# nianticlabs/simplerecon

Hardware: AMD Instinct MI355X
Metric: depth frames/sec (640x480, 7 src views, 64 planes) (higher is better)
Workload: dtype f32

## Files before the change

include/simplerecon_hip.h:

```cpp
#ifndef SIMPLERECON_HIP_H_
#define SIMPLERECON_HIP_H_

#include <stddef.h>
#include <stdint.h>

#ifdef __cplusplus
extern "C" {
#endif

#define SR_OK 0
#define SR_ERR_INVALID_ARGUMENT 1
#define SR_ERR_UNSUPPORTED 2
#define SR_ERR_WORKSPACE_TOO_SMALL 3
#define SR_ERR_HIP_BASE 1000

enum {
  SR_OPT_MLP_SPLIT = 0, SR_OPT_WINO_SPLIT, SR_OPT_WINO_XCD, SR_OPT_WINO_NT, SR_OPT_WINO_KSPLIT, SR_OPT_CONV_WINO,
  SR_OPT_CONV_TILE, SR_OPT_CONV_KSPLIT, SR_OPT_PW_NT, SR_OPT_PW_KS, SR_OPT_PT_CFG, SR_OPT_PT_KS, SR_OPT_DOT_LDS,
  SR_OPT_DOT_LDS_G, SR_OPT_DOT_LDS_CULL, SR_OPT_DOT_LDS_CAP, SR_OPT_UPSAMPLE_QUAD, SR_OPT_POOL_STREAM,
  SR_OPT_MLP_TILE,
  SR_OPT_COUNT
};
int sr_option_count(void);
const char* sr_option_name(int id);
int sr_option_id(const char* name);
int sr_option_get(int id, int* value);
int sr_option_set(int id, int value, int* previous );
int sr_option_default(int id, int* value);

int sr_abi_version(void);

const char* sr_target_arch(void);


size_t sr_volume_workspace_bytes(int B, int K, int C, int h, int w);

int sr_volume_prepare(const float* src, const float* K_src, const float* T_src_cur,
                      const float* T_cur_src, int B, int K, int C, int h, int w, void* workspace,
                      size_t workspace_bytes, void* stream);

int sr_dot_volume_sweep(const float* cur, const float* invK_cur, const float* planes, int64_t ps_b,
                        int64_t ps_d, int64_t ps_y, int64_t ps_x, int B, int K, int C, int h, int w,
                        int D, float* out_cv, int64_t cv_sb, int64_t cv_sd, int64_t cv_sp,
                        float* out_lowest, uint8_t* out_mask, void* workspace,
                        size_t workspace_bytes, void* stream);

int sr_conv3x3_wino_io_nhwc_fwd(const void* in, int64_t in_batch_stride, int in_pix_stride, const float* packed_u,
                                const float* bias, const void* residual, int64_t res_batch_stride, int res_pix_stride,
                                void* out, int64_t out_batch_stride, int out_pix_stride, int B, int H, int W, int Cin,
                                int Cout, float leaky_slope, int io_dtype, void* stream);
int sr_pw_conv_io_nhwc_fwd(const void* in, int64_t in_batch_stride, int in_pix_stride, const float* packed_w,
                           const float* bias, const void* residual, int64_t res_batch_stride, int res_pix_stride, void* out,
                           int64_t out_batch_stride, int out_pix_stride, int B, int HW, int Cin, int Cout, float act_code,
                           int io_dtype, void* stream);

size_t sr_pw_conv_tiled_workspace_bytes(int M, int Cin, int Cout);
int sr_pw_conv_tiled_plan(int M, int Cin, int Cout, int can_split, int* cfg, int* ks);
int sr_pw_conv_tiled_nhwc_fwd(const float* in, int in_pix_stride, const float* packed_w, const float* bias,
                              const float* gate, const float* residual, int res_pix_stride, float* out,
                              int out_pix_stride, int M, int HW, int Cin, int Cout, float act_code, void* workspace,
                              size_t workspace_bytes, void* stream);
int sr_pw_conv_supported(int Cin, int Cout);
int sr_pw_conv_plan(int B, int HW, int Cin, int Cout, int* nt, int* ks);
int sr_pw_conv_nhwc_fwd(const float* in, int64_t in_batch_stride, int in_pix_stride, const float* packed_w,
                        const float* bias, const float* gate, const float* residual, int64_t res_batch_stride,
                        int res_pix_stride, float* out, int64_t out_batch_stride, int out_pix_stride, int B, int HW,
                        int Cin, int Cout, float act_code, void* stream);

int sr_backproject_fwd(const float* depth, const float* invK, float* out_points, int B, int h, int w, void* stream);
int sr_project3d_fwd(const float* points, const float* K, const float* T, float* out, int B, int N, float eps,
                     void* stream);
int sr_backproject_bwd(const float* grad_points, const float* invK, float* grad_depth, int B, int h, int w, void* stream);
int sr_project3d_bwd(const float* grad_out, const float* points, const float* K, const float* T, float* grad_points, int B,
                     int N, float eps, void* stream);
int sr_pose_distance_fwd(const float* T, float* out, int n, void* stream);
int sr_camera_rays_fwd(const float* points, const float* T, float* out, int B, int N, int in_camera_frame, void* stream);

int sr_selftest_rcp(const float* x, float* out_fast, float* out_div, int n, void* stream);

int sr_dot_volume_fwd(const float* cur, const float* src, const float* K_src,
                      const float* T_src_cur, const float* invK_cur, const float* planes,
                      int64_t ps_b, int64_t ps_d, int64_t ps_y, int64_t ps_x, int B, int K, int C,
                      int h, int w, int D, float* out_cv, int64_t cv_sb, int64_t cv_sd,
                      int64_t cv_sp, float* out_lowest, uint8_t* out_mask, void* workspace,
                      size_t workspace_bytes, void* stream);

int sr_warp_features_fwd(const float* src, const float* K_src, const float* T_src_cur,
                         const float* invK_cur, const float* planes, int64_t ps_b, int64_t ps_d,
                         int64_t ps_y, int64_t ps_x, int B, int K, int C, int h, int w, int Dp,
                         float* out_world, float* out_depths, float* out_warped, float* out_mask,
                         float* out_pix, void* workspace, size_t workspace_bytes, void* stream);

size_t sr_mlp_volume_workspace_bytes(int B, int K, int C, int h, int w, int hidden);

int sr_mlp_pack_weights(const float* W1, const float* b1, const float* W2, const float* b2,
                        const float* W3, const float* b3, int hidden, int B, int K, int C, int h, int w,
                        void* workspace, size_t workspace_bytes, void* stream);

int sr_mlp_volume_sweep(const float* cur, const float* invK_cur, const float* planes, int64_t ps_b,
                        int64_t ps_d, int64_t ps_y, int64_t ps_x, float leaky_slope, int B, int K,
                        int C, int h, int w, int D, float* out_cv, int64_t cv_sb, int64_t cv_sd,
                        int64_t cv_sp, float* out_lowest, uint8_t* out_mask, void* workspace,
                        size_t workspace_bytes, void* stream);

int sr_mlp_volume_tile_shape(int h, int w, int* th, int* tw);

int sr_mlp_volume_fwd(const float* cur, const float* src, const float* K_src, const float* T_src_cur,
                      const float* T_cur_src, const float* invK_cur, const float* planes, int64_t ps_b,
                      int64_t ps_d, int64_t ps_y, int64_t ps_x, const float* W1, const float* b1,
                      const float* W2, const float* b2, const float* W3, const float* b3, int hidden,
                      float leaky_slope, int B, int K, int C, int h, int w, int D, float* out_cv,
                      int64_t cv_sb, int64_t cv_sd, int64_t cv_sp, float* out_lowest, uint8_t* out_mask,
                      int reserve_cus, void* workspace, size_t workspace_bytes, void* stream);

int sr_mlp_volume_fwd_nhwc(const float* cur, const float* src, const float* K_src, const float* T_src_cur,
                           const float* T_cur_src, const float* invK_cur, const float* planes, int64_t ps_b,
                           int64_t ps_d, int64_t ps_y, int64_t ps_x, const float* W1, const float* b1,
                           const float* W2, const float* b2, const float* W3, const float* b3, int hidden,
                           float leaky_slope, int B, int K, int C, int h, int w, int D, float* out_cv,
                           int64_t cv_sb, int64_t cv_sd, int64_t cv_sp, float* out_lowest, uint8_t* out_mask,
                           int reserve_cus, void* workspace, size_t workspace_bytes, void* stream);


size_t sr_conv_packed_weight_floats(int Cout, int Cin, int ksize);

int sr_conv_pack_weights(const float* weight, int Cout, int Cin, int ksize, float* packed, void* stream);

int sr_conv2d_nhwc_fwd(const float* in, int64_t in_batch_stride, int in_pix_stride,
                       const float* packed_weight, const float* bias, const float* residual,
                       int64_t res_batch_stride, int res_pix_stride, float* out,
                       int64_t out_batch_stride, int out_pix_stride, int B, int H, int W, int Cin,
                       int Cout, int ksize, int stride, float leaky_slope, void* stream);

int sr_conv2d_replicate_nhwc_fwd(const float* in, int64_t in_batch_stride, int in_pix_stride,
                                 const float* packed_weight, const float* bias, const float* residual,
                                 int64_t res_batch_stride, int res_pix_stride, float* out,
                                 int64_t out_batch_stride, int out_pix_stride, int B, int H, int W, int Cin,
                                 int Cout, int ksize, int stride, float leaky_slope, void* stream);

#define SR_ACT_NONE (-1.0f)
#define SR_ACT_SILU (-2.0f)
int sr_conv2d_padded_nhwc_fwd(const float* in, int64_t in_batch_stride, int in_pix_stride,
                              const float* packed_weight, const float* bias, const float* residual,
                              int64_t res_batch_stride, int res_pix_stride, float* out,
                              int64_t out_batch_stride, int out_pix_stride, int B, int H, int W, int Cin,
                              int Cout, int ksize, int stride, int pad_top, int pad_left, int pad_bottom,
                              int pad_right, float leaky_slope, void* stream);

size_t sr_conv_splitk_workspace_bytes(int B, int H, int W, int Cin, int Cout, int ksize, int stride);
int sr_conv2d_splitk_nhwc_fwd(const float* in, int64_t in_batch_stride, int in_pix_stride,
                              const float* packed_weight, const float* bias, const float* residual,
                              int64_t res_batch_stride, int res_pix_stride, float* out,
                              int64_t out_batch_stride, int out_pix_stride, int B, int H, int W, int Cin,
                              int Cout, int ksize, int stride, float leaky_slope, void* workspace,
                              size_t workspace_bytes, void* stream);

size_t sr_wino_packed_weight_floats(int Cout, int Cin);
int sr_wino_pack_weights(const float* weight, int Cout, int Cin, float* packed, void* stream);
int sr_conv_prefers_wino(int B, int H, int W, int Cin, int Cout, int ksize, int stride);
int sr_conv3x3_wino_nhwc_fwd(const float* in, int64_t in_batch_stride, int in_pix_stride,
                             const float* packed_u, const float* bias, const float* residual,
                             int64_t res_batch_stride, int res_pix_stride, float* out,
                             int64_t out_batch_stride, int out_pix_stride, int B, int H, int W, int Cin,
                             int Cout, float leaky_slope, void* stream);

size_t sr_wino4_packed_weight_floats(int Cout, int Cin);
int sr_wino4_pack_weights(const float* weight, int Cout, int Cin, float* packed, void* stream);
int sr_conv_prefers_wino4(int B, int H, int W, int Cin, int Cout, int mode);
int sr_conv3x3_wino4_nhwc_fwd(const float* in, int64_t in_batch_stride, int in_pix_stride, const float* packed_u,
                              const float* bias, const float* residual, int64_t res_batch_stride, int res_pix_stride,
                              float* out, int64_t out_batch_stride, int out_pix_stride, int B, int H, int W, int Cin,
                              int Cout, float leaky_slope, void* stream);

int sr_conv3x3_wino4_variant_nhwc_fwd(const float* in, int64_t in_batch_stride, int in_pix_stride, const float* packed_u,
                                      const float* bias, const float* residual, int64_t res_batch_stride,
                                      int res_pix_stride, float* out, int64_t out_batch_stride, int out_pix_stride, int B,
                                      int H, int W, int Cin, int Cout, float leaky_slope, int variant, void* stream);

int sr_wino_splitk_factor(int B, int H, int W, int Cin, int Cout);
size_t sr_wino_splitk_workspace_bytes(int B, int H, int W, int Cin, int Cout);
int sr_conv3x3_wino_splitk_nhwc_fwd(const float* in, int64_t in_batch_stride, int in_pix_stride,
                                    const float* packed_u, const float* bias, const float* residual,
                                    int64_t res_batch_stride, int res_pix_stride, float* out,
                                    int64_t out_batch_stride, int out_pix_stride, int B, int H, int W, int Cin,
                                    int Cout, float leaky_slope, void* workspace, size_t workspace_bytes,
                                    void* stream);

const char* sr_wino_kernel_name(int B, int H, int W, int Cin, int Cout, int aligned_in, int aligned_out);

const char* sr_conv_kernel_name(int B, int H, int W, int Cin, int Cout, int ksize, int stride, int aligned16);

int sr_upsample2x_nhwc_fwd(const float* in, int64_t in_batch_stride, int in_pix_stride, float* out,
                           int64_t out_batch_stride, int out_pix_stride, int B, int H, int W, int C,
                           void* stream);

int sr_exp_fwd(const float* in, float* out, int64_t n, void* stream);


size_t sr_stem_packed_weight_floats(int Cout);
int sr_stem_pack_weights(const float* weight, int Cout, float* packed, void* stream);

int sr_stem7x7_fwd(const float* in, int64_t in_batch_stride, int64_t in_chan_stride, int64_t in_row_stride,
                   int64_t in_col_stride, const float* packed_weight, const float* scale, const float* shift,
                   float leaky_slope, float* out, int64_t out_batch_stride, int out_pix_stride, int B, int H, int W,
                   int Cout, void* stream);

int sr_maxblurpool_nhwc_fwd(const float* in, int64_t in_batch_stride, int in_pix_stride, float* out,
                            int64_t out_batch_stride, int out_pix_stride, int B, int H, int W, int C, void* stream);

size_t sr_instance_norm_workspace_bytes(int B, int H, int W, int C);
int sr_instance_norm_nhwc_fwd(const float* in, int64_t in_batch_stride, int in_pix_stride, float* out,
                              int64_t out_batch_stride, int out_pix_stride, int B, int H, int W, int C, float eps,
                              float leaky_slope, void* workspace, size_t workspace_bytes, void* stream);

int sr_instance_norm_stats_nhwc(const float* in, int64_t in_batch_stride, int in_pix_stride, int B, int H, int W, int C,
                                float eps, float* stats, void* workspace, size_t workspace_bytes, void* stream);

size_t sr_conv1x1_stats_workspace_bytes(int B, int H, int W, int Cout);
int sr_conv1x1_stats_nhwc_fwd(const float* in, int64_t in_batch_stride, int in_pix_stride, const float* weight,
                              const float* bias, float* out, int64_t out_batch_stride, int out_pix_stride, int B, int H,
                              int W, int Cin, int Cout, float eps, float* stats, void* workspace, size_t workspace_bytes,
                              void* stream);

size_t sr_conv3x3_c16_packed_weight_floats(int Cout, int Cin);
// ... 351 lines not shown
```

simplerecon_amd/_lib.py:

```python
import contextlib
import ctypes as C
import os

import torch

_HERE = os.path.dirname(os.path.abspath(__file__))
LIB_PATH = os.environ.get("SR_HIP_LIBRARY") or os.path.join(_HERE, "libsimplerecon_hip.so")
ABI_VERSION = 3

_lib = None

_p = C.c_void_p
_i = C.c_int
_i64 = C.c_int64
_f = C.c_float
_sz = C.c_size_t

SIGNATURES = {
    "sr_abi_version": (_i, []),
    "sr_option_count": (_i, []),
    "sr_option_name": (C.c_char_p, [_i]),
    "sr_option_id": (_i, [C.c_char_p]),
    "sr_option_get": (_i, [_i, C.POINTER(C.c_int)]),
    "sr_option_set": (_i, [_i, _i, C.POINTER(C.c_int)]),
    "sr_option_default": (_i, [_i, C.POINTER(C.c_int)]),
    "sr_target_arch": (C.c_char_p, []),
    "sr_volume_workspace_bytes": (_sz, [_i, _i, _i, _i, _i]),
    "sr_volume_prepare": (_i, [_p, _p, _p, _p, _i, _i, _i, _i, _i, _p, _sz, _p]),
    "sr_dot_volume_sweep": (_i, [_p, _p, _p, _i64, _i64, _i64, _i64, _i, _i, _i, _i, _i, _i,
                                 _p, _i64, _i64, _i64, _p, _p, _p, _sz, _p]),
    "sr_dot_volume_fwd": (_i, [_p, _p, _p, _p, _p, _p, _i64, _i64, _i64, _i64, _i, _i, _i, _i, _i, _i,
                               _p, _i64, _i64, _i64, _p, _p, _p, _sz, _p]),
    "sr_rgb_stem3x3s2_fwd": (_i, [_p, _i64, _i64, _i64, _i64, _p, _p, _p, _i64, _i, _i, _i, _i, _i, _i, _i, _i, _i, _f, _p]),
    "sr_se_gate2_fwd": (_i, [_p, _i, _i, _p, _p, _p, _p, _p, _p, _i, _i, _i, _p]),
    "sr_conv3x3_wino_io_nhwc_fwd": (_i, [_p, _i64, _i, _p, _p, _p, _i64, _i, _p, _i64, _i, _i, _i, _i, _i, _i, _f, _i, _p]),
    "sr_pw_conv_io_nhwc_fwd": (_i, [_p, _i64, _i, _p, _p, _p, _i64, _i, _p, _i64, _i, _i, _i, _i, _i, _f, _i, _p]),
    "sr_conv16_packed_weight_bytes": (_sz, [_i, _i, _i]),
    "sr_conv16_pack_weights": (_i, [_p, _i, _i, _i, _i, _p, _p]),
    "sr_conv16_supported": (_i, [_i, _i, _i, _i, _i, _i, _i]),
    "sr_conv16_prefers": (_i, [_i, _i, _i, _i, _i, _i, _i]),
    "sr_conv16_nhwc_fwd": (_i, [_p, _i64, _i, _p, _p, _p, _i64, _i, _p, _i64, _i, _i, _i, _i, _i, _i, _i, _i, _f, _i, _i, _p]),
    "sr_conv16_wgrad_supported": (_i, [_i, _i, _i, _i, _i, _i, _i]),
    "sr_conv16_wgrad_prefers": (_i, [_i, _i, _i, _i, _i, _i, _i]),
    "sr_conv16_wgrad_workspace_bytes": (_sz, [_i, _i, _i, _i, _i, _i, _i]),
    "sr_conv16_wgrad_nhwc": (_i, [_p, _i64, _i, _p, _i64, _i, _p, _i, _i, _i, _i, _i, _i, _i, _i, _p, _sz, _p]),
    "sr_act_bwd_bias16_workspace_bytes": (_sz, [_i64, _i]),
    "sr_act_bwd_bias16_nhwc": (_i, [_p, _i, _p, _p, _p, _i64, _i, _f, _i, _p, _sz, _p]),
    "sr_pw_conv_tiled_workspace_bytes": (_sz, [_i, _i, _i]),
    "sr_pw_conv_tiled_plan": (_i, [_i, _i, _i, _i, _p, _p]),
    "sr_pw_conv_tiled_nhwc_fwd": (_i, [_p, _i, _p, _p, _p, _p, _i, _p, _i, _i, _i, _i, _i, _f, _p, _sz, _p]),
    "sr_pw_conv_supported": (_i, [_i, _i]),
    "sr_pw_conv_plan": (_i, [_i, _i, _i, _i, _p, _p]),
    "sr_pw_conv_nhwc_fwd": (_i, [_p, _i64, _i, _p, _p, _p, _p, _i64, _i, _p, _i64, _i, _i, _i, _i, _i, _f, _p]),
    "sr_backproject_fwd": (_i, [_p, _p, _p, _i, _i, _i, _p]),
    "sr_project3d_fwd": (_i, [_p, _p, _p, _p, _i, _i, _f, _p]),
    "sr_backproject_bwd": (_i, [_p, _p, _p, _i, _i, _i, _p]),
    "sr_project3d_bwd": (_i, [_p, _p, _p, _p, _p, _i, _i, _f, _p]),
    "sr_pose_distance_fwd": (_i, [_p, _p, _i, _p]),
    "sr_camera_rays_fwd": (_i, [_p, _p, _p, _i, _i, _i, _p]),
    "sr_selftest_rcp": (_i, [_p, _p, _p, _i, _p]),
    "sr_warp_features_fwd": (_i, [_p, _p, _p, _p, _p, _i64, _i64, _i64, _i64, _i, _i, _i, _i, _i, _i,
                                  _p, _p, _p, _p, _p, _p, _sz, _p]),
    "sr_mlp_volume_workspace_bytes": (_sz, [_i, _i, _i, _i, _i, _i]),
    "sr_mlp_pack_weights": (_i, [_p, _p, _p, _p, _p, _p, _i, _i, _i, _i, _i, _i, _p, _sz, _p]),
    "sr_mlp_volume_sweep": (_i, [_p, _p, _p, _i64, _i64, _i64, _i64, _f, _i, _i, _i, _i, _i, _i,
                                 _p, _i64, _i64, _i64, _p, _p, _p, _sz, _p]),
    "sr_mlp_volume_tile_shape": (_i, [_i, _i, C.POINTER(C.c_int), C.POINTER(C.c_int)]),
    "sr_mlp_volume_fwd": (_i, [_p, _p, _p, _p, _p, _p, _p, _i64, _i64, _i64, _i64, _p, _p, _p, _p, _p, _p, _i,
                               _f, _i, _i, _i, _i, _i, _i, _p, _i64, _i64, _i64, _p, _p, _i, _p, _sz, _p]),
    "sr_mlp_volume_fwd_nhwc": (_i, [_p, _p, _p, _p, _p, _p, _p, _i64, _i64, _i64, _i64, _p, _p, _p, _p, _p, _p, _i,
                                    _f, _i, _i, _i, _i, _i, _i, _p, _i64, _i64, _i64, _p, _p, _i, _p, _sz, _p]),
    "sr_conv_packed_weight_floats": (_sz, [_i, _i, _i]),
    "sr_conv_pack_weights": (_i, [_p, _i, _i, _i, _p, _p]),
    "sr_conv2d_nhwc_fwd": (_i, [_p, _i64, _i, _p, _p, _p, _i64, _i, _p, _i64, _i, _i, _i, _i, _i, _i, _i, _i, _f, _p]),
    "sr_conv2d_replicate_nhwc_fwd": (_i, [_p, _i64, _i, _p, _p, _p, _i64, _i, _p, _i64, _i, _i, _i, _i, _i, _i, _i, _i,
                                          _f, _p]),
    "sr_conv2d_padded_nhwc_fwd": (_i, [_p, _i64, _i, _p, _p, _p, _i64, _i, _p, _i64, _i, _i, _i, _i, _i, _i, _i, _i,
                                       _i, _i, _i, _i, _f, _p]),
    "sr_dwconv3x3_pool_bands": (_i, [_i]),
    "sr_dwconv3x3_nhwc_fwd": (_i, [_p, _i64, _i, _p, _p, _p, _i64, _i, _p, _i, _i, _i, _i, _i, _i, _i, _i, _i, _f,
                                   _p]),
    "sr_add_nhwc_fwd": (_i, [_p, _i64, _i, _p, _i64, _i, _p, _i64, _i, _i, _i, _i, _i, _p]),
    "sr_se_scale_nhwc_fwd": (_i, [_p, _i, _p, _p, _p, _p, _p, _p, _i64, _i, _p, _i64, _i, _p, _i, _i, _i, _i, _i,
                                  _p]),
    "sr_se_gate_fwd": (_i, [_p, _i, _i, _p, _p, _p, _p, _p, _i, _i, _i, _p]),
    "sr_scale_channels_nhwc_fwd": (_i, [_p, _i64, _i, _p, _p, _i64, _i, _i, _i, _i, _i, _p]),
    "sr_dot_volume_bwd_scratch_bytes": (_sz, [_i, _i, _i, _i, _i]),
    "sr_dot_volume_bwd": (_i, [_p, _i64, _i64, _i64, _p, _p, _p, _i64, _i64, _i64, _i64, _i, _i, _i, _i, _i, _i, _p, _p,
                               _p, _sz, _p, _sz, _p]),
    "sr_mlp_volume_bwd_scratch_bytes": (_sz, [_i, _i, _i, _i, _i, _i]),
    "sr_mlp_volume_bwd": (_i, [_p, _i64, _i64, _i64, _p, _p, _p, _i64, _i64, _i64, _i64, _p, _p, _p, _p, _p, _f, _i, _i,
                               _i, _i, _i, _i, _i, _p, _p, _p, _p, _p, _p, _p, _p, _p, _sz, _p, _sz, _p]),
    "sr_conv_wgrad_workspace_bytes": (_sz, [_i, _i, _i, _i, _i, _i, _i]),
    "sr_conv_wgrad_nhwc": (_i, [_p, _i64, _i, _p, _i64, _i, _p, _i, _i, _i, _i, _i, _i, _i, _p, _sz, _p]),
    "sr_bias_grad_nhwc": (_i, [_p, _i64, _i, _p, _i, _i, _i, _i, _p]),
    "sr_act_bwd": (_i, [_p, _p, _p, _i64, _f, _p]),
    "sr_act_bwd_bias_workspace_bytes": (_sz, [_i64, _i]),
    "sr_act_bwd_bias_nhwc": (_i, [_p, _p, _p, _p, _i64, _i, _f, _p, _sz, _p]),
    "sr_zero_stuff2x_nhwc": (_i, [_p, _i64, _i, _p, _i, _i, _i, _i, _i, _i, _p]),
    "sr_upsample2x_bwd_nhwc": (_i, [_p, _i64, _i, _p, _i64, _i, _i, _i, _i, _i, _p]),
    "sr_conv_flip_transpose_weights": (_i, [_p, _i, _i, _i, _p, _p]),
    "sr_mul_fwd": (_i, [_p, _p, _p, _i64, _p]),
    "sr_norm_workspace_bytes": (_sz, [_i, _i, _i, _i]),
    "sr_norm_stats_nhwc": (_i, [_p, _i64, _i, _i, _i, _i, _i, _p, _p, _p, _sz, _p]),
    "sr_norm_act_fwd_nhwc": (_i, [_p, _i64, _i, _p, _p, _f, _p, _p, _f, _i, _p, _i64, _i, _i, _i, _i, _p]),
    "sr_norm_act_bwd_nhwc": (_i, [_p, _i64, _i, _p, _i64, _i, _p, _p, _f, _p, _p, _f, _i, _i, _p, _i64, _i, _p, _p,
                                  _i, _i, _i, _p, _sz, _p]),
    "sr_rowsum_nhwc": (_i, [_p, _i64, _i, _p, _i64, _i, _i, _i, _i, _f, _p, _p, _sz, _p]),
    "sr_maxblurpool_bwd_workspace_bytes": (_sz, [_i, _i, _i, _i]),
    "sr_maxblurpool_bwd_nhwc": (_i, [_p, _i64, _i, _p, _i64, _i, _p, _i64, _i, _i, _i, _i, _i, _p, _sz, _p]),
    "sr_replicate_pad_nhwc_fwd": (_i, [_p, _i64, _i, _p, _i, _i, _i, _i, _i, _p]),
    "sr_replicate_pad_nhwc_bwd": (_i, [_p, _p, _i, _i, _i, _i, _i, _p]),
    "sr_im2col7x7s2_nhwc": (_i, [_p, _i64, _i64, _i64, _i64, _p, _i, _i, _i, _i, _p]),
    "sr_dwconv3x3_bwd_workspace_bytes": (_sz, [_i, _i, _i, _i]),
    "sr_dwconv3x3_bwd_nhwc": (_i, [_p, _i64, _i, _p, _i64, _i, _p, _p, _p, _i, _i, _i, _i, _i, _i, _i, _i, _i, _p, _sz,
                                   _p]),
    "sr_scale_bwd_nhwc": (_i, [_p, _i64, _i, _p, _p, _f, _p, _i, _i, _i, _p]),
    "sr_small_linear_fwd": (_i, [_p, _p, _p, _p, _p, _i, _i, _i, _f, _p]),
    "sr_small_linear_bwd": (_i, [_p, _p, _p, _p, _p, _p, _p, _i, _i, _i, _f, _p]),
    "sr_act_in_bwd": (_i, [_p, _p, _p, _i64, _f, _p]),
    "sr_add_act_fwd": (_i, [_p, _p, _p, _p, _i64, _f, _p]),
    "sr_conv_wgrad_padded_workspace_bytes": (_sz, [_i, _i, _i, _i, _i, _i]),
    "sr_conv_wgrad_padded_nhwc": (_i, [_p, _i64, _i, _p, _i64, _i, _p, _i, _i, _i, _i, _i, _i, _i, _i, _i, _i, _i, _p,
                                       _sz, _p]),
    "sr_conv_splitk_workspace_bytes": (_sz, [_i, _i, _i, _i, _i, _i, _i]),
    "sr_conv2d_splitk_nhwc_fwd": (_i, [_p, _i64, _i, _p, _p, _p, _i64, _i, _p, _i64, _i, _i, _i, _i, _i, _i, _i, _i,
                                       _f, _p, _sz, _p]),
    "sr_wino_packed_weight_floats": (_sz, [_i, _i]),
    "sr_wino_pack_weights": (_i, [_p, _i, _i, _p, _p]),
    "sr_conv_prefers_wino": (_i, [_i, _i, _i, _i, _i, _i, _i]),
    "sr_wino_splitk_factor": (_i, [_i, _i, _i, _i, _i]),
    "sr_wino_splitk_workspace_bytes": (_sz, [_i, _i, _i, _i, _i]),
    "sr_conv3x3_wino_splitk_nhwc_fwd": (_i, [_p, _i64, _i, _p, _p, _p, _i64, _i, _p, _i64, _i, _i, _i, _i, _i, _i, _f,
                                             _p, _sz, _p]),
# ... 47 lines not shown
    "sr_depth_terms_bwd": (_i, [_p, _p, _p, _p, _p, _p, _p, _i, _i, _p, _i, _i, _p, _i, _i, _i, _i, _i, _f, _i, _p, _p,
                                _p, _p, _p, _p]),
    "sr_depth_metrics_workspace_bytes": (_sz, [_i, _i, _i]),
    "sr_depth_metrics": (_i, [_p, _p, _p, _f, _i, _i, _i, _i, _i, _i, _i, _p, _p, _p, _p, _sz, _p]),
    "sr_depth_metrics_gather": (_i, [_p, _i, _i, _i, _i, _i, _i, _p, _p]),
    "sr_nn_grid_plan": (_i, [_i64, _p, _i64, _p, _p, _p]),
    "sr_nn_keys": (_i, [_p, _i64, C.c_double, C.c_double, C.c_double, C.c_double, _i, _i, _i, _p, _p]),
    "sr_nn_build": (_i, [_p, _i64, _p, _p, _i64, _p, _p, _p]),
    "sr_nn_query": (_i, [_p, _i64, _p, _p, _i64, _p, _i64, C.c_double, C.c_double, C.c_double, C.c_double, _i, _i, _i,
                         _p, _p, _p, _p]),
    "sr_sample_surface_workspace_bytes": (_sz, [_i64]),
    "sr_sample_surface_cdf": (_i, [_p, _i64, _p, _i64, _p, _p, _sz, _p]),
    "sr_sample_surface": (_i, [_p, _i64, _p, _i64, _p, _i64, C.c_uint64, _p, _p, _p]),
    "sr_mesh_metrics_workspace_bytes": (_sz, [_i64, _i64]),
    "sr_mesh_metrics": (_i, [_p, _i64, _p, _i64, _f, _p, _p, _sz, _p]),
    "sr_stsdf_touch": (_i, [_p, _i, _i, _i, _p, C.c_double, C.c_double, _p, _p]),
    "sr_stsdf_block_masks": (_i, [_p, _p, _i64, _i64, _p, _p]),
    "sr_stsdf_integrate": (_i, [_p, _i64, _p, _p, _p, _i64, _p, _p, _p, _i, _i, _i, _f, _f, _p]),
    "sr_stsdf_mesh_count": (_i, [_p, _i64, _p, _p, _i64, _p, _p]),
    "sr_stsdf_mesh_emit": (_i, [_p, _i64, _p, _p, _i64, _f, _p, _i64, _i64, _p, _p, _p, _p, _p]),
    "sr_raster_small": (_i, [_p, _i64, _p, _i64, _p, _p, _i, _i, _i, _f, _f, _i, _p, _p, _p]),
    "sr_raster_large_setup": (_i, [_p, _i64, _p, _i64, _p, _p, _i, _i, _i, _f, _f, _i, _i64, _p, _p, _p, _p]),
    "sr_raster_large": (_i, [_p, _p, _i64, _i64, _p, _i, _i, _i, _f, _f, _p, _p]),
    "sr_raster_resolve": (_i, [_p, _i64, _p, _p, _p]),
    "sr_raster_visibility_mask": (_i, [_p, _i, _i64, _i64, _p, _p]),
    "sr_raster_visibility_count": (_i, [_p, _i64, _p, _i, _p, _p]),
    "sr_mesh_vertex_normals": (_i, [_p, _i64, _p, _i64, _p, _p, _p, _p]),
    "sr_raster_shade": (_i, [_p, _i64, _p, _i64, _p, _p, _i, _i, _i, _f, _p, _p, _p, _p, _p, _f, _p, _i, _i, _i, _p, _p,
                             _p, _p]),
    "sr_frames_resize_fits_lds": (_i, [_i, _i, _i, _i]),
    "sr_frames_resize": (_i, [_p, _i, _i, _i, _i, _p, _i, _p, _i, _i, _p, _p, _i, _i, _i, _i, _p, _p]),
    "sr_frames_depth": (_i, [_p, _i, _i, _i, _i, _p, _p, _i, _i, _f, _f, _f, _i, _p, _p, _p, _p]),
    "sr_frames_jitter_scratch_bytes": (_sz, [_i, _i, _i]),
    "sr_frames_jitter_check_params": (_i, [_p, _i]),
    "sr_frames_jitter": (_i, [_p, _i, _i, _i, _p, _p, _i, _i, _p, _sz, _p]),
    "sr_viz_range_workspace_bytes": (_sz, [_i, _i64]),
    "sr_viz_range": (_i, [_p, _p, _i, _i, _i64, _i, _p, _p, _sz, _p]),
    "sr_viz_colormap": (_i, [_p, _p, _i, _i, _i64, _p, _p, _i64, _p, _i64, _f, _f, _f, _f, _f, _p, _p, _p]),
    "sr_viz_unit": (_i, [_p, _i, _i64, _i, _p, _p, _p]),
    "sr_adamw_step": (_i, [_p, _p, _p, _p, _p, _p, _p, _p, _p, _i, _i, _p, _i, _p, _p, _p]),
    "sr_adamw_step_clipped": (_i, [_p, _p, _p, _p, _p, _p, _p, _p, _p, _i, _i, _p, _i, _p, _p, _p, _p]),
    "sr_grad_stats_workspace_bytes": (_sz, [_i, _i]),
    "sr_grad_stats": (_i, [_p, _p, _p, _i, _i, _p, _f, _p, _p, _p, _p, C.c_double, C.c_double, _i, _p, _sz, _p]),
    "sr_grad_scale_inplace": (_i, [_p, _p, _p, _i, _i, _p, _p]),
}


class HipLibraryError(RuntimeError):
    pass


def lib():
    global _lib
    if _lib is None:
        if not os.path.exists(LIB_PATH):
            raise HipLibraryError(
                f"{LIB_PATH} not found: build it with `python -m simplerecon_amd.build` "
                "(hipcc --offload-arch=gfx950).  simplerecon_amd has no CPU/torch fallback.")
        l = C.CDLL(LIB_PATH)
        for name, (res, args) in SIGNATURES.items():
            fn = getattr(l, name)
            fn.restype = res
            fn.argtypes = args
        if l.sr_abi_version() != ABI_VERSION:
            raise HipLibraryError(f"ABI mismatch: library {l.sr_abi_version()} vs binding {ABI_VERSION}")
        _lib = l
    return _lib


ERR_UNSUPPORTED = 2
_ERRORS = {1: "invalid argument", ERR_UNSUPPORTED: "unsupported configuration", 3: "workspace too small"}


def check(rc, what):
    if rc != 0:
        msg = _ERRORS.get(rc, f"hipError {rc - 1000}" if rc >= 1000 else f"error {rc}")
        raise HipLibraryError(f"{what} failed: {msg}")


SPLIT_MODES = {"": 0, "0": 0, "off": 0, "fp32": 0, "bf16": 1, "f16": 2, "fp16": 2}
_SPLIT_NAMES = {0: "", 1: "bf16", 2: "f16"}
SPLIT_OPTION_NAMES = ("SR_MLP_SPLIT", "SR_WINO_SPLIT")
TILE_MODES = {"auto": 0, "flat": 1, "2x32": 2, "4x16": 3, "8x8": 4}
_NAMED_VALUES = {"SR_MLP_SPLIT": SPLIT_MODES, "SR_WINO_SPLIT": SPLIT_MODES, "SR_MLP_TILE": TILE_MODES}
import threading
SPLIT_GUARD = threading.RLock()


OPTION_LISTENERS = []


def _option_id(name):
    oid = lib().sr_option_id(name.encode())
    if oid < 0:
        raise KeyError(f"libsimplerecon_hip.so has no option {name!r}")
    return oid


_OPTION_MIRROR = {}


def get_option(name):
    v = _OPTION_MIRROR.get(name)
    if v is None:
        c = C.c_int(0)
        check(lib().sr_option_get(_option_id(name), C.byref(c)), "sr_option_get")
        v = _OPTION_MIRROR[name] = c.value
    return v


def refresh_options():
    _OPTION_MIRROR.clear()


def set_option(name, value):
    if isinstance(value, str):
        if name not in _NAMED_VALUES:
            raise ValueError(f"option {name} takes an integer, got {value!r}")
        value = _NAMED_VALUES[name].get(value, -1)
    prev = C.c_int(0)
    with SPLIT_GUARD if name in SPLIT_OPTION_NAMES else _NULL_CONTEXT:
        check(lib().sr_option_set(_option_id(name), int(value), C.byref(prev)), "sr_option_set")
        _OPTION_MIRROR[name] = int(value)
        for fn in OPTION_LISTENERS:
            fn(name, int(value))
    return prev.value


@contextlib.contextmanager
def option(name, value):
    prev = set_option(name, value)
    try:
        yield
    finally:
        set_option(name, prev)


def split_mode_name(option_name):
    v = get_option(option_name)
    return _SPLIT_NAMES.get(v, str(v))


def require_device_f32(name, t, allow_none=False):
    if t is None:
        if allow_none:
            return
        raise ValueError(f"{name} is None")
    if not isinstance(t, torch.Tensor):
        raise TypeError(f"{name} must be a torch.Tensor, got {type(t)}")
    if not t.is_cuda:
        raise HipLibraryError(f"{name} lives on {t.device}: the HIP path needs device tensors (no CPU fallback)")
    if t.dtype != torch.float32:
        raise TypeError(f"{name} must be float32 (the reference runs inference in fp32), got {t.dtype}")


def device_f32(name, t, why=None):
    if why is not None and isinstance(t, torch.Tensor) and t.dtype != torch.float32:
        raise TypeError(f"{name} must be float32 ({why}), got {t.dtype}")
    require_device_f32(name, t)
    return t.contiguous()


def data_f32(name, t, role, why=None):
    t = device_f32(name, t, why)
    if torch.is_grad_enabled() and t.requires_grad:
        raise HipLibraryError(f"{name} requires a gradient: {role}")
    return t.detach()
# ... 66 lines not shown
```

simplerecon_amd/csrc/sr_common.h:

```cpp
#pragma once
#include <hip/hip_runtime.h>
#include <stdint.h>

#include "simplerecon_hip.h"

#define SR_GEOM_STRIDE 20

#define SR_WAVE 64

int sr_opt(int id);

int sr_device_cus();

hipError_t sr_allow_lds(const void* kernel, size_t bytes);

int sr_wgrad_reduce_launch(const float* part, float* d_weight, int Cout, int Cin, int taps, int ci_blocks, int per, int blocks,
                           hipStream_t stream);
int sr_bias_partial_reduce_launch(const float* partial, int blocks, int C, float* d_bias, hipStream_t stream);

static inline int sr_hip_rc(hipError_t e) { return e == hipSuccess ? SR_OK : SR_ERR_HIP_BASE + (int)e; }

static inline size_t sr_align_up(size_t v, size_t a) { return (v + a - 1) / a * a; }

struct SrPlanes {
// ... 37 lines not shown
  w_nw = (vx0 & vy0) ? wtop.x : 0.0f;
  w_ne = (vx1 & vy0) ? wtop.y : 0.0f;
  w_sw = (vx0 & vy1) ? wbot.x : 0.0f;
  w_se = (vx1 & vy1) ? wbot.y : 0.0f;
  any_tap = (vx0 | vx1) & (vy0 | vy1);
}
__device__ __forceinline__ void sr_bilinear_taps(float ix, float iy, int h, int w, float& fx0, float& fy0, float& w_nw,
                                                 float& w_ne, float& w_sw, float& w_se) {
  bool any_tap;
  sr_bilinear_taps(ix, iy, h, w, fx0, fy0, w_nw, w_ne, w_sw, w_se, any_tap);
}

struct SrSampleXY {
  float zp, pix_x, pix_y;
  float ix, iy;
  float fx0, fy0;
  float w_nw, w_ne, w_sw, w_se;
  bool any_tap;
};

__device__ __forceinline__ void sr_project_sample_xy(const float* __restrict__ g ,
                                                     float X0, float X1, float X2, int h, int w,
                                                     float inv_w, float inv_h, SrSampleXY& s) {
#pragma clang fp contract(off)
  const float eps = 1e-8f;
  const sr_f2v q01 = sr_f2v{g[0], g[4]} * X0 + sr_f2v{g[1], g[5]} * X1 + sr_f2v{g[2], g[6]} * X2 + sr_f2v{g[3], g[7]};
  const float q2 = g[8] * X0 + g[9] * X1 + g[10] * X2 + g[11];
  s.zp = q2 + eps;
  const float sc = (fabsf(q2) > eps) ? 1.0f / s.zp : 1.0f;
  const sr_f2v pix = q01 * sc;
  s.pix_x = pix.x;
  s.pix_y = pix.y;
  const sr_f2v uv = 2.0f * pix * sr_f2v{inv_w, inv_h} - 1.0f;
  const sr_f2v size = {(float)w, (float)h};
  const sr_f2v ixy = ((uv + 1.0f) * size - 1.0f) / 2.0f;
  s.ix = ixy.x;
  s.iy = ixy.y;
  sr_bilinear_taps(s.ix, s.iy, h, w, s.fx0, s.fy0, s.w_nw, s.w_ne, s.w_sw, s.w_se, s.any_tap);
}

__device__ __forceinline__ void sr_project_sample(const float* __restrict__ g ,
                                                  float X0, float X1, float X2, int h, int w,
                                                  float inv_w, float inv_h, SrSample& s) {
  SrSampleXY c;
  sr_project_sample_xy(g, X0, X1, X2, h, w, inv_w, inv_h, c);
  s.zp = c.zp; s.pix_x = c.pix_x; s.pix_y = c.pix_y;
  s.w_nw = c.w_nw; s.w_ne = c.w_ne; s.w_sw = c.w_sw; s.w_se = c.w_se;
  s.any_tap = c.any_tap;
  const float wm = (float)(w - 1), hm = (float)(h - 1);
  const float fx1 = c.fx0 + 1.0f, fy1 = c.fy0 + 1.0f;
  const int x0 = (int)fminf(fmaxf(c.fx0, 0.0f), wm), x1 = (int)fminf(fmaxf(fx1, 0.0f), wm);
  const int y0 = (int)fminf(fmaxf(c.fy0, 0.0f), hm), y1 = (int)fminf(fmaxf(fy1, 0.0f), hm);
  s.o_nw = y0 * w + x0;
  s.o_ne = y0 * w + x1;
  s.o_sw = y1 * w + x0;
  s.o_se = y1 * w + x1;
}

__device__ __forceinline__ bool sr_in_bounds(const SrSample& s, int h, int w) {
  return (s.pix_x > 2.0f) & (s.pix_x < (float)(w - 2)) & (s.pix_y > 2.0f) & (s.pix_y < (float)(h - 2));
}

#ifdef __HIPCC__
__device__ __forceinline__ float sr_vmax(float a, float b) {
  float r;
  asm("v_max_f32 %0, %1, %2" : "=v"(r) : "v"(a), "v"(b));
  return r;
}
__device__ __forceinline__ float sr_vmin(float a, float b) {
  float r;
  asm("v_min_f32 %0, %1, %2" : "=v"(r) : "v"(a), "v"(b));
  return r;
}
__device__ __forceinline__ float sr_vmax_mfma(float a, float b) {
  float r;
  asm("v_max_f32 %0, %1, %2\n\ts_nop 1" : "=v"(r) : "v"(a), "v"(b));
  return r;
}
__device__ __forceinline__ float sr_activate(float v, float slope) {
  if (slope >= 0.0f) return fmaxf(v, 0.0f) + slope * fminf(v, 0.0f);
  if (slope < -1.5f) return v / (1.0f + __expf(-v));
  return v;
}
__device__ __forceinline__ float sr_uniform(float x) {
  return __builtin_bit_cast(float, __builtin_amdgcn_readfirstlane(__builtin_bit_cast(int, x)));
}
template <int N>
__device__ __forceinline__ void sr_activate_group(float (&v)[N], float slope) {
  if (slope >= 0.0f) {
    if (slope <= 1.0f) {
#pragma unroll
      for (int i = 0; i < N; ++i) v[i] = sr_vmax(v[i], slope * v[i]);
    } else {
#pragma unroll
      for (int i = 0; i < N; ++i) v[i] = sr_vmax(v[i], 0.0f) + slope * sr_vmin(v[i], 0.0f);
    }
  } else if (slope < -1.5f) {
#pragma unroll
    for (int i = 0; i < N; ++i) v[i] = v[i] / (1.0f + __expf(-v[i]));
  }
}
#endif

struct SrDotParams {
  const float* cur;
  const float* src_nhwc;
  const float* invK;
  const float* geom;
  SrPlanes planes;
  SrVolumeOut out;
  int B, K, h, w, D;
  float inv_w, inv_h;
};

static inline float* sr_ws_geom(void* workspace) { return (float*)sr_align_up((size_t)workspace, 256); }
static inline float* sr_ws_src_nhwc(void* workspace, int B, int K) {
  return (float*)((char*)sr_ws_geom(workspace) + sr_align_up((size_t)B * K * SR_GEOM_STRIDE * sizeof(float), 256));
}

static inline size_t sr_ws_nhwc_bytes(int B, int K, int C, int h, int w) {
  return sr_align_up((size_t)B * K * h * w * C * sizeof(float), 256);
}
static inline unsigned long long* sr_ws_keys(void* workspace, int B, int K, int C, int h, int w) {
  return (unsigned long long*)((char*)sr_ws_src_nhwc(workspace, B, K) + sr_ws_nhwc_bytes(B, K, C, h, w));
}

int sr_launch_dot_volume_lds(const SrDotParams& p, unsigned long long* keys, hipStream_t stream);
int sr_launch_geom(const float* K_src, const float* T_src_cur, const float* T_cur_src, float* geom,
                   int n, hipStream_t stream);
int sr_launch_argmax_planes(const float* cv, int64_t sb, int64_t sd, int64_t sp, SrPlanes planes, int B, int h, int w,
                            int D, float* lowest, hipStream_t stream);
int sr_launch_splitk_reduce(const float* part, int ksplit, int64_t part_stride, const float* bias, const float* res,
                            int64_t res_sb, int res_sp, float* out, int64_t out_sb, int out_sp, int B, int HW, int Cout,
                            float slope, hipStream_t stream);
int sr_launch_unpack_nhwc(const float* src_nhwc, float* dst_nchw, int images, int C, int npix, hipStream_t stream);
int sr_launch_pack_nhwc(const float* src_nchw, float* dst_nhwc, int images, int C, int npix,
                        hipStream_t stream);
```

simplerecon_amd/csrc/sr_conv.hip:

```cpp
#include <stdio.h>
#include <stdlib.h>

#include "sr_common.h"
#include "sr_view.h"

#ifndef SR_NB1
#define SR_NB1 6
#endif
#ifndef SR_RES_PF
#define SR_RES_PF 0
#endif

#ifndef SR_CK1
#define SR_CK1 64
#endif
#ifndef SR_CONV_BLOCKS_PER_CU
#define SR_CONV_BLOCKS_PER_CU 2
#endif
__host__ __device__ constexpr int sr_ck(int ks, int stride = 1) { return (ks == 1 && stride == 1) ? SR_CK1 : 16; }

struct SrConvParams {
  const float* in; int64_t in_sb; int in_sp;
  const float* wp;
  const float* bias;
// ... 15 lines not shown
  static constexpr int HH = (TH - 1) * S + KS;
  static constexpr int HW = (CM - 1) * S + KS;
  static constexpr int CK = sr_ck(KS, S);
  static constexpr int ROW = CK + 4;
  static constexpr int Q = CK / 4;
  static constexpr int ELEMS = HH * HW * Q;
  static constexpr int PER_THREAD = (ELEMS + 255) / 256;
  static constexpr int TILE_FLOATS = HH * HW * ROW;
};

template <int KS, int S, int MT, int CM>
__device__ __forceinline__ void sr_conv_stage_setup(const SrConvParams& p, int iy0, int ix0,
                                                    int (&offs)[SrConvGeom<KS, S, MT, CM>::PER_THREAD]) {
  using G = SrConvGeom<KS, S, MT, CM>;
#pragma unroll
  for (int it = 0; it < G::PER_THREAD; ++it) {
    const int e = threadIdx.x + it * 256;
    const int px = e / G::Q, q = e % G::Q;
    const int hy = px / G::HW, hx = px - hy * G::HW;
    int iy = iy0 + hy, ix = ix0 + hx;
    if (p.replicate) {
      iy = min(max(iy, 0), p.H - 1);
      ix = min(max(ix, 0), p.W - 1);
    }
    const bool ok = (e < G::ELEMS) && (iy >= 0) && (iy < p.H) && (ix >= 0) && (ix < p.W);
    offs[it] = ok ? (iy * p.W + ix) * p.in_sp + 4 * q : -1;
  }
}

template <int KS, int S, int MT, int CM, bool VEC4>
__device__ __forceinline__ void sr_conv_stage_load(const SrConvParams& p, const float* __restrict__ in_b, int c0,
                                                   const int (&offs)[SrConvGeom<KS, S, MT, CM>::PER_THREAD],
                                                   float4 (&stg)[SrConvGeom<KS, S, MT, CM>::PER_THREAD]) {
  using G = SrConvGeom<KS, S, MT, CM>;
#pragma unroll
  for (int it = 0; it < G::PER_THREAD; ++it) {
    const int c = c0 + 4 * ((threadIdx.x + it * 256) % G::Q);
    const bool ok = (offs[it] >= 0) && (c < p.Cin);
    const float* src = in_b + (ok ? offs[it] + c0 : 0);
    if (VEC4) {
      const float4 v = *reinterpret_cast<const float4*>(src);
      stg[it] = ok ? v : make_float4(0.f, 0.f, 0.f, 0.f);
    } else {
      float4 v = make_float4(0.f, 0.f, 0.f, 0.f);
      if (ok) {
        v.x = src[0];
        if (c + 1 < p.Cin) v.y = src[1];
        if (c + 2 < p.Cin) v.z = src[2];
        if (c + 3 < p.Cin) v.w = src[3];
      }
      stg[it] = v;
    }
  }
}

template <int KS, int S, int MT, int CM>
__device__ __forceinline__ void sr_conv_stage_store(float* __restrict__ tile,
                                                    const float4 (&stg)[SrConvGeom<KS, S, MT, CM>::PER_THREAD]) {
  using G = SrConvGeom<KS, S, MT, CM>;
#pragma unroll
  for (int it = 0; it < G::PER_THREAD; ++it) {
    const int e = threadIdx.x + it * 256;
    if (e < G::ELEMS) *reinterpret_cast<float4*>(&tile[(e / G::Q) * G::ROW + 4 * (e % G::Q)]) = stg[it];
  }
}

struct SrTileCoord { int b, co0, oy0, ox0, ks; };

template <int TH, int NT, int CM>
__device__ __forceinline__ SrTileCoord sr_conv_tile(const SrConvParams& p, int work) {
  SrTileCoord t;
  t.ks = 0;
  if (p.ksplit > 1) { t.ks = work % p.ksplit; work /= p.ksplit; }
  const int cb = work % p.co_blocks; work /= p.co_blocks;
  const int tx = work % p.tiles_x; work /= p.tiles_x;
  const int ty = work % p.tiles_y;
  t.b = work / p.tiles_y;
  t.co0 = cb * (32 * NT);
  t.oy0 = ty * TH;
  t.ox0 = tx * CM;
  return t;
}

template <int KS, int S, int MT, int NT, int CM, bool VEC4>
__global__ __launch_bounds__(256) void sr_conv_kernel(SrConvParams p) {
  using G = SrConvGeom<KS, S, MT, CM>;
  constexpr int TH = G::TH, HW = G::HW, RM = G::RM;
  constexpr int GPS = G::CK / 8;
  constexpr int STEPS = KS * KS * GPS;
  constexpr int ROW = G::ROW;
  __shared__ __attribute__((aligned(16))) float tiles[2][G::TILE_FLOATS];

  const int lane = threadIdx.x & 63;
  const int wave = threadIdx.x >> 6;
  const int i = lane & 31, kk = lane >> 5;

  int a_off[MT];
#pragma unroll
  for (int m = 0; m < MT; ++m)
    a_off[m] = ((((wave * MT + m) * RM + i / CM) * S) * HW + (i % CM) * S) * ROW + 4 * kk;
  const int64_t rec = (int64_t)2 * p.Co_pad;
  const int chunks = p.G / GPS;

  constexpr int NB = (NT == 1) ? (STEPS % 6 == 0 ? SR_NB1 : STEPS % 4 == 0 ? 4 : STEPS % 3 == 0 ? 3 : 2)
                               : (STEPS % 3 == 0 ? 3 : 2);
  constexpr int PD = NB - 1;
  static_assert(STEPS % NB == 0 && PD < STEPS + 1, "rotating buffers must line up across slabs");
  constexpr bool RES_PF = (MT * NT <= 2) && SR_RES_PF;
  float4 b_f[NB][NT], a_f[2][MT], stg[G::PER_THREAD];
  int offs[G::PER_THREAD];

  int work = blockIdx.x;
  if (work >= p.total_tiles) return;
  SrTileCoord t = sr_conv_tile<TH, NT, CM>(p, work);
  const float4* wp4 = reinterpret_cast<const float4*>(p.wp) + (kk * p.Co_pad + t.co0 + i);
  auto load_b = [&](const float4* base, int ch, int s, float4 (&dst)[NT]) {
    const int tap = s / GPS, g = s % GPS;
    const float4* wrec = base + (int64_t)(tap * p.G + GPS * ch + g) * rec;
#pragma unroll
    for (int n = 0; n < NT; ++n) dst[n] = wrec[32 * n];
  };

  int c_beg = t.ks * chunks / p.ksplit, c_end = (t.ks + 1) * chunks / p.ksplit;
  sr_conv_stage_setup<KS, S, MT, CM>(p, t.oy0 * S - p.pad_y, t.ox0 * S - p.pad_x, offs);
  sr_conv_stage_load<KS, S, MT, CM, VEC4>(p, p.in + (int64_t)t.b * p.in_sb, c_beg * G::CK, offs, stg);
  sr_conv_stage_store<KS, S, MT, CM>(tiles[0], stg);
#pragma unroll
  for (int s = 0; s < PD; ++s) load_b(wp4, c_beg, s, b_f[s]);
  __syncthreads();
  int buf = 0;
  const bool partial = p.ksplit > 1;

  while (true) {
    const int next_work = work + gridDim.x;
    const bool have_next = next_work < p.total_tiles;
    SrTileCoord tn = t;
    if (have_next) tn = sr_conv_tile<TH, NT, CM>(p, next_work);
    const float4* wp4n = reinterpret_cast<const float4*>(p.wp) + (kk * p.Co_pad + tn.co0 + i);
    const int cn_beg = tn.ks * chunks / p.ksplit, cn_end = (tn.ks + 1) * chunks / p.ksplit;

    f32x16 acc[MT][NT];
#pragma unroll
    for (int m = 0; m < MT; ++m)
#pragma unroll
      for (int n = 0; n < NT; ++n)
#pragma unroll
        for (int r = 0; r < 16; ++r) acc[m][n][r] = 0.0f;
    float rpf[RES_PF ? MT : 1][RES_PF ? NT : 1][16];
    const float* __restrict__ resp = (p.res && !partial) ? p.res + (int64_t)t.b * p.res_sb : nullptr;

    for (int ch = c_beg; ch < c_end; ++ch) {
      const float* tile = tiles[buf];
      const bool last = ch + 1 == c_end;
      const bool more = !last || have_next;
      if (more) {
        if (last) sr_conv_stage_setup<KS, S, MT, CM>(p, tn.oy0 * S - p.pad_y, tn.ox0 * S - p.pad_x, offs);
        sr_conv_stage_load<KS, S, MT, CM, VEC4>(p, p.in + (int64_t)(last ? tn.b : t.b) * p.in_sb,
                                            (last ? cn_beg : ch + 1) * G::CK, offs, stg);
      }
      const float4* wnext = last ? wp4n : wp4;
      const int chn = last ? cn_beg : ch + 1;
      if (RES_PF && last) {
#pragma unroll
        for (int m = 0; m < (RES_PF ? MT : 0); ++m) {
          const int oyb = t.oy0 + (wave * MT + m) * RM;
          const int pixb = oyb * p.Wo + t.ox0 + 4 * kk;
#pragma unroll
          for (int n = 0; n < NT; ++n) {
            const int co = t.co0 + 32 * n + i;
            const unsigned rb = (unsigned)(pixb * p.res_sp + co);
#pragma unroll
            for (int r = 0; r < 16; ++r) {
              const int row = (8 * (r >> 2)) / CM, colc = (8 * (r >> 2)) % CM + (r & 3);
              const bool ok = (resp != nullptr) & (co < p.Cout) & (oyb + row < p.Ho) & (t.ox0 + colc + 4 * kk < p.Wo);
              const float v = (resp ? resp : p.in)[ok ? rb + (unsigned)((row * p.Wo + colc) * p.res_sp) : 0u];
              rpf[m][n][r] = ok ? v : 0.0f;
            }
          }
        }
      }
#pragma unroll
      for (int m = 0; m < MT; ++m) a_f[0][m] = *reinterpret_cast<const float4*>(&tile[a_off[m]]);
#pragma unroll
      for (int s = 0; s < STEPS; ++s) {
        const int cb = s % NB, ca = s & 1;
        if (s + PD < STEPS) load_b(wp4, ch, s + PD, b_f[(s + PD) % NB]);
        else if (more) load_b(wnext, chn, s + PD - STEPS, b_f[(s + PD) % NB]);
        if (s + 1 < STEPS) {
          const int tap = (s + 1) / GPS, g = (s + 1) % GPS;
          const int ky = tap / KS, kx = tap - ky * KS;
#pragma unroll
          for (int m = 0; m < MT; ++m)
            a_f[ca ^ 1][m] = *reinterpret_cast<const float4*>(&tile[a_off[m] + (ky * HW + kx) * ROW + 8 * g]);
        }
        __builtin_amdgcn_sched_barrier(0);
#define SR_CONV_KSTEP(E)                                                                                       \
        _Pragma("unroll") for (int m = 0; m < MT; ++m)                                                         \
          _Pragma("unroll") for (int n = 0; n < NT; ++n)                                                       \
            acc[m][n] = __builtin_amdgcn_mfma_f32_32x32x2f32(a_f[ca][m].E, b_f[cb][n].E, acc[m][n], 0, 0, 0);
        SR_CONV_KSTEP(x) SR_CONV_KSTEP(y) SR_CONV_KSTEP(z) SR_CONV_KSTEP(w)
#undef SR_CONV_KSTEP
        __builtin_amdgcn_sched_barrier(0);
      }
      if (more) sr_conv_stage_store<KS, S, MT, CM>(tiles[buf ^ 1], stg);
      __syncthreads();
      buf ^= 1;
    }

    {
      float* __restrict__ outp = partial ? p.part + t.ks * p.part_stride + (int64_t)t.b * p.Ho * p.Wo * p.Cout
                                         : p.out + (int64_t)t.b * p.out_sb;
      const int osp = partial ? p.Cout : p.out_sp, rsp = p.res_sp;
      const float slope = sr_uniform(partial ? SR_ACT_NONE : p.slope);
      const bool no_res = (resp == nullptr);
      const bool full = (t.oy0 + TH <= p.Ho) && (t.ox0 + CM <= p.Wo) && (t.co0 + 32 * NT <= p.Cout);
#pragma unroll
      for (int m = 0; m < MT; ++m) {
        const int oyb = t.oy0 + (wave * MT + m) * RM;
        const int pixb = oyb * p.Wo + t.ox0 + 4 * kk;
#pragma unroll
        for (int n = 0; n < NT; ++n) {
          const int co = t.co0 + 32 * n + i;
          const bool okc = co < p.Cout;
          const float bv = (p.bias && okc && !partial) ? p.bias[co] : 0.0f;
          const unsigned ob = (unsigned)(pixb * osp + co), rb = (unsigned)(pixb * rsp + co);
          float rv[16];
          if (RES_PF) {
#pragma unroll
            for (int r = 0; r < 16; ++r) rv[r] = rpf[RES_PF ? m : 0][RES_PF ? n : 0][r];
          }
          if (full) {
            if (RES_PF) {
            } else if (!no_res) {
#pragma unroll
              for (int r = 0; r < 16; ++r) {
                const int row = (8 * (r >> 2)) / CM, colc = (8 * (r >> 2)) % CM + (r & 3);
                rv[r] = resp[rb + (unsigned)((row * p.Wo + colc) * rsp)];
              }
            } else {
#pragma unroll
              for (int r = 0; r < 16; ++r) rv[r] = 0.0f;
            }
            float o16[16];
#pragma unroll
            for (int r = 0; r < 16; ++r) o16[r] = acc[m][n][r] + bv + rv[r];
            sr_activate_group(o16, slope);
#pragma unroll
            for (int r = 0; r < 16; ++r) {
              const int row = (8 * (r >> 2)) / CM, colc = (8 * (r >> 2)) % CM + (r & 3);
              outp[ob + (unsigned)((row * p.Wo + colc) * osp)] = o16[r];
            }
          } else {
            bool ok[16];
#pragma unroll
            for (int r = 0; r < 16; ++r) {
              const int row = (8 * (r >> 2)) / CM, colc = (8 * (r >> 2)) % CM + (r & 3);
              ok[r] = okc && (oyb + row < p.Ho) && (t.ox0 + colc + 4 * kk < p.Wo);
              if (!RES_PF) rv[r] = (!no_res && ok[r]) ? resp[rb + (unsigned)((row * p.Wo + colc) * rsp)] : 0.0f;
            }
            float o16[16];
#pragma unroll
            for (int r = 0; r < 16; ++r) o16[r] = acc[m][n][r] + bv + rv[r];
            sr_activate_group(o16, slope);
#pragma unroll
            for (int r = 0; r < 16; ++r) {
              const int row = (8 * (r >> 2)) / CM, colc = (8 * (r >> 2)) % CM + (r & 3);
              if (ok[r]) outp[ob + (unsigned)((row * p.Wo + colc) * osp)] = o16[r];
            }
          }
        }
      }
    }
    if (!have_next) break;
    work = next_work;
    t = tn;
    c_beg = cn_beg; c_end = cn_end;
    wp4 = wp4n;
  }
}

__global__ void sr_conv_pack_kernel(const float* __restrict__ w, float* __restrict__ wp, int Co, int Ci, int taps,
                                    int G, int Co_pad) {
  const int64_t total = (int64_t)taps * G * 2 * Co_pad * 4;
  for (int64_t e = blockIdx.x * (int64_t)blockDim.x + threadIdx.x; e < total; e += (int64_t)gridDim.x * blockDim.x) {
    const int el = (int)(e & 3);
    int64_t r = e >> 2;
    const int co = (int)(r % Co_pad); r /= Co_pad;
    const int kk = (int)(r & 1); r >>= 1;
    const int g = (int)(r % G);
    const int tap = (int)(r / G);
    const int ci = 8 * g + 4 * kk + el;
    wp[e] = (co < Co && ci < Ci) ? w[((int64_t)co * Ci + ci) * taps + tap] : 0.0f;
  }
}

__global__ void sr_upsample2x_kernel(const float* __restrict__ in, int64_t in_sb, int in_sp, float* __restrict__ out,
                                     int64_t out_sb, int out_sp, int H, int W, int C, int vec4) {
  const int Ho = 2 * H, Wo = 2 * W;
  const int cq = (C + 3) >> 2;
  const int64_t total = (int64_t)Ho * Wo * cq;
  const int b = blockIdx.y;
  for (int64_t e = blockIdx.x * (int64_t)blockDim.x + threadIdx.x; e < total; e += (int64_t)gridDim.x * blockDim.x) {
    const int q = (int)(e % cq);
    const int64_t opix = e / cq;
    const int oy = (int)(opix / Wo), ox = (int)(opix - (int64_t)oy * Wo);
    const float sy = fmaxf(((float)oy + 0.5f) * 0.5f - 0.5f, 0.0f);
    const float sx = fmaxf(((float)ox + 0.5f) * 0.5f - 0.5f, 0.0f);
    const int y0 = (int)sy, x0 = (int)sx;
    const int y1 = y0 + (y0 < H - 1 ? 1 : 0), x1 = x0 + (x0 < W - 1 ? 1 : 0);
    const float ly = sy - (float)y0, lx = sx - (float)x0;
    const float hy = 1.0f - ly, hx = 1.0f - lx;
    const float* ib = in + (int64_t)b * in_sb + 4 * q;
    const float* p00 = ib + ((int64_t)y0 * W + x0) * in_sp;
    const float* p01 = ib + ((int64_t)y0 * W + x1) * in_sp;
    const float* p10 = ib + ((int64_t)y1 * W + x0) * in_sp;
    const float* p11 = ib + ((int64_t)y1 * W + x1) * in_sp;
    float* o = out + (int64_t)b * out_sb + opix * out_sp + 4 * q;
    const int nc = min(4, C - 4 * q);
    if (vec4 && nc == 4) {
      const float4 a = *reinterpret_cast<const float4*>(p00), bq = *reinterpret_cast<const float4*>(p01);
      const float4 c = *reinterpret_cast<const float4*>(p10), d = *reinterpret_cast<const float4*>(p11);
      float4 r;
      r.x = hy * (hx * a.x + lx * bq.x) + ly * (hx * c.x + lx * d.x);
      r.y = hy * (hx * a.y + lx * bq.y) + ly * (hx * c.y + lx * d.y);
      r.z = hy * (hx * a.z + lx * bq.z) + ly * (hx * c.z + lx * d.z);
      r.w = hy * (hx * a.w + lx * bq.w) + ly * (hx * c.w + lx * d.w);
      *reinterpret_cast<float4*>(o) = r;
    } else {
      for (int k = 0; k < nc; ++k)
        o[k] = hy * (hx * p00[k] + lx * p01[k]) + ly * (hx * p10[k] + lx * p11[k]);
    }
  }
}

__global__ __launch_bounds__(256) void sr_upsample2x_quad_kernel(const float* __restrict__ in, int64_t in_sb, int in_sp,
                                                                 float* __restrict__ out, int64_t out_sb, int out_sp, int B,
                                                                 int H, int W, int cq) {
  const int Ho = 2 * H, Wo = 2 * W;
  const int t = blockIdx.x * blockDim.x + threadIdx.x;
  if (t >= (W + 1) * cq) return;
  const int q = t % cq, bx = t / cq - 1;
  const int xa = min(max(bx, 0), W - 1), xb = min(xa + 1, W - 1);
  float lx[2], hx[2];
#pragma unroll
  for (int r = 0; r < 2; ++r) {
    const float sx = fmaxf(((float)(2 * bx + 1 + r) + 0.5f) * 0.5f - 0.5f, 0.0f);
// ... 2 lines not shown
  }
  for (int row = blockIdx.y; row < B * (H + 1); row += gridDim.y) {
    const int b = row / (H + 1), by = row - b * (H + 1) - 1;
    const int ya = min(max(by, 0), H - 1), yb = min(ya + 1, H - 1);
    const float* ib = in + (int64_t)b * in_sb + 4 * q;
    const float4 a = *reinterpret_cast<const float4*>(ib + ((int64_t)ya * W + xa) * in_sp);
    const float4 bq = *reinterpret_cast<const float4*>(ib + ((int64_t)ya * W + xb) * in_sp);
    const float4 c = *reinterpret_cast<const float4*>(ib + ((int64_t)yb * W + xa) * in_sp);
    const float4 d = *reinterpret_cast<const float4*>(ib + ((int64_t)yb * W + xb) * in_sp);
    float* ob = out + (int64_t)b * out_sb + 4 * q;
#pragma unroll
    for (int ry = 0; ry < 2; ++ry) {
      const int oy = 2 * by + 1 + ry;
      if (oy < 0 || oy >= Ho) continue;
      const float sy = fmaxf(((float)oy + 0.5f) * 0.5f - 0.5f, 0.0f);
      const float ly = sy - (float)ya, hy = 1.0f - ly;
#pragma unroll
      for (int rx = 0; rx < 2; ++rx) {
        const int ox = 2 * bx + 1 + rx;
        if (ox < 0 || ox >= Wo) continue;
        float4 r;
        r.x = hy * (hx[rx] * a.x + lx[rx] * bq.x) + ly * (hx[rx] * c.x + lx[rx] * d.x);
        r.y = hy * (hx[rx] * a.y + lx[rx] * bq.y) + ly * (hx[rx] * c.y + lx[rx] * d.y);
        r.z = hy * (hx[rx] * a.z + lx[rx] * bq.z) + ly * (hx[rx] * c.z + lx[rx] * d.z);
        r.w = hy * (hx[rx] * a.w + lx[rx] * bq.w) + ly * (hx[rx] * c.w + lx[rx] * d.w);
        *reinterpret_cast<float4*>(ob + ((int64_t)oy * Wo + ox) * out_sp) = r;
      }
    }
  }
}

__global__ __launch_bounds__(256) void sr_exp_kernel(const float* __restrict__ in, float* __restrict__ out, int64_t n) {
  for (int64_t i = (int64_t)blockIdx.x * blockDim.x + threadIdx.x; i < n; i += (int64_t)gridDim.x * blockDim.x)
    out[i] = expf(in[i]);
}


extern "C" int sr_exp_fwd(const float* in, float* out, int64_t n, void* stream_) {
  if (n < 0) return SR_ERR_INVALID_ARGUMENT;
  if (n == 0) return SR_OK;
  if (!in || !out) return SR_ERR_INVALID_ARGUMENT;
  const int64_t blocks = (n + 255) / 256 < 2048 ? (n + 255) / 256 : 2048;
  hipLaunchKernelGGL(sr_exp_kernel, dim3((unsigned)blocks), dim3(256), 0, (hipStream_t)stream_, in, out, n);
  return sr_hip_rc(hipGetLastError());
}

extern "C" size_t sr_conv_packed_weight_floats(int Cout, int Cin, int ksize) {
  if (Cout <= 0 || Cin <= 0 || (ksize != 1 && ksize != 3)) return 0;
  const int ck = sr_ck(ksize);
  const size_t G = (size_t)((Cin + ck - 1) / ck) * (ck / 8), Co_pad = (size_t)((Cout + 31) / 32) * 32;
  return (size_t)ksize * ksize * G * 2 * Co_pad * 4;
}

extern "C" int sr_conv_pack_weights(const float* weight, int Cout, int Cin, int ksize, float* packed, void* stream_) {
  if (!weight || !packed || Cout <= 0 || Cin <= 0) return SR_ERR_INVALID_ARGUMENT;
  if (ksize != 1 && ksize != 3) return SR_ERR_UNSUPPORTED;
  const int ck = sr_ck(ksize);
  const int G = ((Cin + ck - 1) / ck) * (ck / 8), Co_pad = ((Cout + 31) / 32) * 32;
  hipLaunchKernelGGL(sr_conv_pack_kernel, dim3(256), dim3(256), 0, (hipStream_t)stream_, weight, packed, Cout, Cin,
                     ksize * ksize, G, Co_pad);
  return sr_hip_rc(hipGetLastError());
}

template <int KS, int S, int MT, int CM>
static int sr_conv_launch(SrConvParams& p, int B, int nt, hipStream_t stream) {
  using G = SrConvGeom<KS, S, MT, CM>;
  p.tiles_x = (p.Wo + CM - 1) / CM;
  p.tiles_y = (p.Ho + G::TH - 1) / G::TH;
  p.co_blocks = (p.Co_pad + 32 * nt - 1) / (32 * nt);
  p.total_tiles = p.tiles_x * p.tiles_y * p.co_blocks * B;
  if (p.ksplit > 1) {
    const int chunks = p.G / (G::CK / 8);
    int ks = (2 * sr_device_cus()) / p.total_tiles;
    if (KS == 3 && 2 * p.total_tiles > sr_device_cus()) ks = 1;
    if (ks > chunks / 2) ks = chunks / 2;
    if (ks > p.ksplit) ks = p.ksplit;
    p.ksplit = ks < 2 ? 1 : ks;
    p.total_tiles *= p.ksplit;
  }
  int blocks = sr_device_cus() * (KS == 1 ? SR_CONV_BLOCKS_PER_CU : 2);
  if (blocks > p.total_tiles) blocks = p.total_tiles;
  dim3 grid(blocks), block(256);
  const bool v4 = p.vec4 && (p.Cin % 4 == 0);
  if (nt == 2 && v4) hipLaunchKernelGGL((sr_conv_kernel<KS, S, MT, 2, CM, true>), grid, block, 0, stream, p);
  else if (nt == 2) hipLaunchKernelGGL((sr_conv_kernel<KS, S, MT, 2, CM, false>), grid, block, 0, stream, p);
  else if (v4) hipLaunchKernelGGL((sr_conv_kernel<KS, S, MT, 1, CM, true>), grid, block, 0, stream, p);
  else hipLaunchKernelGGL((sr_conv_kernel<KS, S, MT, 1, CM, false>), grid, block, 0, stream, p);
  return sr_hip_rc(hipGetLastError());
}

struct SrConvCfg { int shape, nt; };
static SrConvCfg sr_conv_pick(const SrConvParams& p, int B, int stride, int ksize) {
  const int cus = sr_device_cus();
  const double stage_w = ksize == 1 ? 0.6 : 0.0;
  const int th[3] = {8, 4, 16}, tw[3] = {32, 32, 8}, mt[3] = {2, 1, 1};
  SrConvCfg best = {1, 1};
  double best_cost = -1;
  for (int c = 0; c < 3; ++c) {
    if (stride == 2 && c == 0) continue;
    for (int nt = 2; nt >= 1; --nt) {
      if (nt == 2 && p.Co_pad % 64 != 0) continue;
      const long tiles = (long)((p.Wo + tw[c] - 1) / tw[c]) * ((p.Ho + th[c] - 1) / th[c]) *
                         ((p.Co_pad + 32 * nt - 1) / (32 * nt)) * B;
      double rounds = (double)((tiles + cus - 1) / cus);
      if (ksize == 1 && mt[c] * nt == 1 && tiles > cus && tiles <= 2 * cus)
        rounds = 1.0 + 0.35 * (double)(tiles - cus) / cus;
      const double cost = rounds * (mt[c] * nt + 0.12 + 0.04 * nt + stage_w * mt[c]);
      if (best_cost < 0 || cost < best_cost) { best = {c, nt}; best_cost = cost; }
    }
  }
  return best;
}

static SrConvCfg sr_conv_cfg(const SrConvParams& p, int B, int stride, int ksize) {
  SrConvCfg cfg = sr_conv_pick(p, B, stride, ksize);
  const int v = sr_opt(SR_OPT_CONV_TILE);
  if (v > 0) {
    const int shape = v % 10, nt = v / 10;
    if (shape >= 0 && shape <= 2 && !(stride == 2 && shape == 0)) cfg.shape = shape;
    if (nt == 1 || (nt == 2 && p.Co_pad % 64 == 0)) cfg.nt = nt;
  }
  return cfg;
}

#define SR_CONV_KSPLIT_MAX 8
static bool sr_conv_splitk_eligible(const float* out, int64_t out_sb, int out_sp, const float* bias, const float* res,
                                    int64_t res_sb, int res_sp, int Cin, int Cout, int ksize, int stride) {
  const int on = sr_opt(SR_OPT_CONV_KSPLIT);
  const bool pw = ksize == 1 && stride == 1 && Cin >= 4 * SR_CK1;
  const bool s2 = ksize == 3 && stride == 2 && Cin >= 8 * sr_ck(3);
  if (!on || !(pw || s2) || Cout % 4 != 0) return false;
  if (!sr_rows_aligned(out, out_sb, out_sp, 15, 4) || (bias && !sr_ptr_aligned(bias, 15))) return false;
  return !res || sr_rows_aligned(res, res_sb, res_sp, 15, 4);
}

static int sr_conv2d_dispatch(const float* in, int64_t in_batch_stride, int in_pix_stride,
                             const float* packed_weight, const float* bias, const float* residual,
                             int64_t res_batch_stride, int res_pix_stride, float* out, int64_t out_batch_stride,
                             int out_pix_stride, int B, int H, int W, int Cin, int Cout, int ksize, int stride,
                             float leaky_slope, int replicate, void* stream_, const int* pads = nullptr,
                             void* workspace = nullptr, size_t workspace_bytes = 0) {
  if (B < 0 || H <= 0 || W <= 0 || Cin <= 0 || Cout <= 0) return SR_ERR_INVALID_ARGUMENT;
  if (B == 0) return SR_OK;
  if (!in || !packed_weight || !out) return SR_ERR_INVALID_ARGUMENT;
  if ((ksize != 1 && ksize != 3) || (stride != 1 && stride != 2)) return SR_ERR_UNSUPPORTED;
  const int pad = ksize / 2;
  const int pt = pads ? pads[0] : pad, pl = pads ? pads[1] : pad, pb = pads ? pads[2] : pad, pr = pads ? pads[3] : pad;
  if (pt < 0 || pl < 0 || pb < 0 || pr < 0 || pt >= ksize || pl >= ksize || pb >= ksize || pr >= ksize ||
      H + pt + pb < ksize || W + pl + pr < ksize)
    return SR_ERR_INVALID_ARGUMENT;
  SrConvParams p;
  p.in = in; p.in_sb = in_batch_stride; p.in_sp = in_pix_stride;
  p.wp = packed_weight; p.bias = bias;
  p.res = residual; p.res_sb = res_batch_stride; p.res_sp = res_pix_stride;
  p.out = out; p.out_sb = out_batch_stride; p.out_sp = out_pix_stride;
  p.H = H; p.W = W; p.Cin = Cin; p.Cout = Cout;
  p.Ho = (H + pt + pb - ksize) / stride + 1;
  p.Wo = (W + pl + pr - ksize) / stride + 1;
  p.pad_y = pt; p.pad_x = pl;
  p.Co_pad = ((Cout + 31) / 32) * 32;
  p.G = ((Cin + sr_ck(ksize) - 1) / sr_ck(ksize)) * (sr_ck(ksize) / 8);
  p.slope = leaky_slope;
  p.replicate = replicate;
  p.ksplit = 1; p.part = nullptr; p.part_stride = 0;
  if (workspace && sr_conv_splitk_eligible(out, out_batch_stride, out_pix_stride, bias, residual, res_batch_stride,
                                           res_pix_stride, Cin, Cout, ksize, stride)) {
    p.part_stride = (int64_t)B * p.Ho * p.Wo * Cout;
    const size_t fit = workspace_bytes / ((size_t)p.part_stride * sizeof(float));
    p.ksplit = fit < 2 ? 1 : (fit < SR_CONV_KSPLIT_MAX ? (int)fit : SR_CONV_KSPLIT_MAX);
    p.part = (float*)workspace;
  }
  p.vec4 = sr_rows_aligned(in, in_batch_stride, in_pix_stride, 15, 4);
  hipStream_t stream = (hipStream_t)stream_;
  const SrConvCfg cfg = sr_conv_cfg(p, B, stride, ksize);
  const int c = cfg.shape, nt = cfg.nt;
  int rc;
  if (ksize == 3 && stride == 1) {
    if (c == 0) rc = sr_conv_launch<3, 1, 2, 32>(p, B, nt, stream);
    else if (c == 1) rc = sr_conv_launch<3, 1, 1, 32>(p, B, nt, stream);
    else rc = sr_conv_launch<3, 1, 1, 8>(p, B, nt, stream);
  } else if (ksize == 3 && stride == 2) {
    if (c == 1) rc = sr_conv_launch<3, 2, 1, 32>(p, B, nt, stream);
    else rc = sr_conv_launch<3, 2, 1, 8>(p, B, nt, stream);
  } else if (ksize == 1 && stride == 1) {
    if (c == 0) rc = sr_conv_launch<1, 1, 2, 32>(p, B, nt, stream);
    else if (c == 1) rc = sr_conv_launch<1, 1, 1, 32>(p, B, nt, stream);
    else rc = sr_conv_launch<1, 1, 1, 8>(p, B, nt, stream);
  } else {
    if (c == 1) rc = sr_conv_launch<1, 2, 1, 32>(p, B, nt, stream);
    else rc = sr_conv_launch<1, 2, 1, 8>(p, B, nt, stream);
  }
  if (rc == SR_OK && p.ksplit > 1)
    rc = sr_launch_splitk_reduce(p.part, p.ksplit, p.part_stride, bias, residual, res_batch_stride, res_pix_stride, out,
                                 out_batch_stride, out_pix_stride, B, p.Ho * p.Wo, Cout, leaky_slope, stream);
  return rc;
}

extern "C" int sr_conv2d_nhwc_fwd(const float* in, int64_t in_batch_stride, int in_pix_stride,
                                  const float* packed_weight, const float* bias, const float* residual,
                                  int64_t res_batch_stride, int res_pix_stride, float* out,
                                  int64_t out_batch_stride, int out_pix_stride, int B, int H, int W, int Cin,
                                  int Cout, int ksize, int stride, float leaky_slope, void* stream_) {
  return sr_conv2d_dispatch(in, in_batch_stride, in_pix_stride, packed_weight, bias, residual, res_batch_stride,
                            res_pix_stride, out, out_batch_stride, out_pix_stride, B, H, W, Cin, Cout, ksize, stride,
                            leaky_slope, 0, stream_);
}

extern "C" int sr_conv2d_replicate_nhwc_fwd(const float* in, int64_t in_batch_stride, int in_pix_stride,
                                            const float* packed_weight, const float* bias, const float* residual,
                                            int64_t res_batch_stride, int res_pix_stride, float* out,
                                            int64_t out_batch_stride, int out_pix_stride, int B, int H, int W,
                                            int Cin, int Cout, int ksize, int stride, float leaky_slope,
                                            void* stream_) {
  return sr_conv2d_dispatch(in, in_batch_stride, in_pix_stride, packed_weight, bias, residual, res_batch_stride,
                            res_pix_stride, out, out_batch_stride, out_pix_stride, B, H, W, Cin, Cout, ksize, stride,
                            leaky_slope, 1, stream_);
}

extern "C" int sr_conv2d_padded_nhwc_fwd(const float* in, int64_t in_batch_stride, int in_pix_stride,
                                         const float* packed_weight, const float* bias, const float* residual,
                                         int64_t res_batch_stride, int res_pix_stride, float* out,
                                         int64_t out_batch_stride, int out_pix_stride, int B, int H, int W, int Cin,
                                         int Cout, int ksize, int stride, int pad_top, int pad_left, int pad_bottom,
                                         int pad_right, float leaky_slope, void* stream_) {
  const int pads[4] = {pad_top, pad_left, pad_bottom, pad_right};
  return sr_conv2d_dispatch(in, in_batch_stride, in_pix_stride, packed_weight, bias, residual, res_batch_stride,
                            res_pix_stride, out, out_batch_stride, out_pix_stride, B, H, W, Cin, Cout, ksize, stride,
                            leaky_slope, 0, stream_, pads);
}

extern "C" size_t sr_conv_splitk_workspace_bytes(int B, int H, int W, int Cin, int Cout, int ksize, int stride) {
  if (B <= 0 || H <= 0 || W <= 0 || Cout % 4 != 0) return 0;
  const bool pw = ksize == 1 && stride == 1 && Cin >= 4 * SR_CK1;
  const bool s2 = ksize == 3 && stride == 2 && Cin >= 8 * sr_ck(3);
  if (!pw && !s2) return 0;
  const int64_t px = s2 ? (int64_t)B * ((H - 1) / 2 + 1) * ((W - 1) / 2 + 1) : (int64_t)B * H * W;
  const int64_t tiles = ((px + 127) / 128) * ((Cout + 31) / 32);
  if (s2 ? 2 * tiles > sr_device_cus() : tiles >= 2 * sr_device_cus()) return 0;
  return (size_t)SR_CONV_KSPLIT_MAX * px * Cout * sizeof(float);
}

extern "C" int sr_conv2d_splitk_nhwc_fwd(const float* in, int64_t in_batch_stride, int in_pix_stride,
                                         const float* packed_weight, const float* bias, const float* residual,
                                         int64_t res_batch_stride, int res_pix_stride, float* out,
                                         int64_t out_batch_stride, int out_pix_stride, int B, int H, int W, int Cin,
                                         int Cout, int ksize, int stride, float leaky_slope, void* workspace,
                                         size_t workspace_bytes, void* stream_) {
  return sr_conv2d_dispatch(in, in_batch_stride, in_pix_stride, packed_weight, bias, residual, res_batch_stride,
                            res_pix_stride, out, out_batch_stride, out_pix_stride, B, H, W, Cin, Cout, ksize, stride,
                            leaky_slope, 0, stream_, nullptr, workspace, workspace_bytes);
}

extern "C" const char* sr_conv_kernel_name(int B, int H, int W, int Cin, int Cout, int ksize, int stride,
                                           int aligned16) {
  static thread_local char buf[96];
  SrConvParams p;
  const int pad = ksize / 2;
  p.Ho = (H + 2 * pad - ksize) / stride + 1;
  p.Wo = (W + 2 * pad - ksize) / stride + 1;
  p.Co_pad = ((Cout + 31) / 32) * 32;
  const SrConvCfg cfg = sr_conv_cfg(p, B, stride, ksize);
  const int mt = cfg.shape == 0 ? 2 : 1, cm = cfg.shape == 2 ? 8 : 32, nt = cfg.nt;
  snprintf(buf, sizeof(buf), "sr_conv_kernel<%d, %d, %d, %d, %d, %s>", ksize, stride, mt, nt, cm,
           (aligned16 && Cin % 4 == 0) ? "true" : "false");
  return buf;
}

extern "C" int sr_upsample2x_nhwc_fwd(const float* in, int64_t in_batch_stride, int in_pix_stride, float* out,
                                      int64_t out_batch_stride, int out_pix_stride, int B, int H, int W, int C,
                                      void* stream_) {
  if (B < 0 || H <= 0 || W <= 0 || C <= 0) return SR_ERR_INVALID_ARGUMENT;
  if (B == 0) return SR_OK;
  if (!in || !out) return SR_ERR_INVALID_ARGUMENT;
  const int vec4 = sr_rows_aligned(in, in_batch_stride, in_pix_stride, 15, 4) &&
                   sr_rows_aligned(out, out_batch_stride, out_pix_stride, 15, 4);
  if (vec4 && C % 4 == 0 && sr_opt(SR_OPT_UPSAMPLE_QUAD)) {
    const int cq = C / 4;
    const int64_t rows = (int64_t)B * (H + 1);
    hipLaunchKernelGGL(sr_upsample2x_quad_kernel, dim3(((W + 1) * cq + 255) / 256, (unsigned)(rows < 65535 ? rows : 65535)),
                       dim3(256), 0, (hipStream_t)stream_, in, in_batch_stride, in_pix_stride, out, out_batch_stride,
                       out_pix_stride, B, H, W, cq);
    return sr_hip_rc(hipGetLastError());
  }
  const int64_t total = (int64_t)4 * H * W * ((C + 3) / 4);
  const int blocks = (int)((total + 255) / 256 < 4096 ? (total + 255) / 256 : 4096);
  hipLaunchKernelGGL(sr_upsample2x_kernel, dim3(blocks, B), dim3(256), 0, (hipStream_t)stream_, in, in_batch_stride,
                     in_pix_stride, out, out_batch_stride, out_pix_stride, H, W, C, vec4);
  return sr_hip_rc(hipGetLastError());
}
```

simplerecon_amd/csrc/sr_mbconv.hip:

```cpp
#include "sr_common.h"

namespace {

constexpr int DW_CH = 64;
constexpr int DW_XL = 16;

struct SrDwParams {
  const float* in; int64_t in_sb; int in_sp;
  const float* w;
  const float* bias;
  float* out; int64_t out_sb; int out_sp;
  float* pool;
  int H, W, C, Ho, Wo, stride, pad_y, pad_x, rows, bands;
  float slope;
};

__device__ __forceinline__ float4 f4fma(float4 a, float4 b, float4 c) {
  return make_float4(fmaf(a.x, b.x, c.x), fmaf(a.y, b.y, c.y), fmaf(a.z, b.z, c.z), fmaf(a.w, b.w, c.w));
}

__global__ __launch_bounds__(256) void sr_dwconv3x3_kernel(SrDwParams p) {
  __shared__ float4 red[DW_XL][DW_CH / 4];
  const int c4 = threadIdx.x & 15, xl = threadIdx.x >> 4;
  const int c = blockIdx.x * DW_CH + 4 * c4;
  const int band = blockIdx.y, b = blockIdx.z;
  const bool live = c < p.C;
  float4 wt[9], bv = make_float4(0.f, 0.f, 0.f, 0.f), sum = make_float4(0.f, 0.f, 0.f, 0.f);
#pragma unroll
  for (int t = 0; t < 9; ++t)
    wt[t] = live ? *reinterpret_cast<const float4*>(p.w + (int64_t)t * p.C + c) : make_float4(0.f, 0.f, 0.f, 0.f);
  if (live && p.bias) bv = *reinterpret_cast<const float4*>(p.bias + c);
  const float* __restrict__ inb = p.in + (int64_t)b * p.in_sb + c;
  float* __restrict__ outb = p.out + (int64_t)b * p.out_sb + c;
  const int oy0 = band * p.rows;
  const int npx = (min(p.Ho, oy0 + p.rows) - oy0) * p.Wo;
  if (live) {
    for (int q0 = xl; q0 < npx; q0 += 2 * DW_XL) {
      float4 v[2][9];
      int opix[2];
#pragma unroll
      for (int u = 0; u < 2; ++u) {
        const int q = q0 + u * DW_XL;
        const bool have = q < npx;
        const int oy = oy0 + (have ? q / p.Wo : 0), ox = have ? q % p.Wo : 0;
        opix[u] = have ? oy * p.Wo + ox : -1;
        const int iy0 = oy * p.stride - p.pad_y, ix0 = ox * p.stride - p.pad_x;
#pragma unroll
        for (int ky = 0; ky < 3; ++ky) {
#pragma unroll
          for (int kx = 0; kx < 3; ++kx) {
            const int iy = iy0 + ky, ix = ix0 + kx;
            const bool ok = have && (iy >= 0) && (iy < p.H) && (ix >= 0) && (ix < p.W);
            const float4 t = *reinterpret_cast<const float4*>(inb + (int64_t)(ok ? iy * p.W + ix : 0) * p.in_sp);
            v[u][ky * 3 + kx] = ok ? t : make_float4(0.f, 0.f, 0.f, 0.f);
          }
        }
      }
#pragma unroll
      for (int u = 0; u < 2; ++u) {
        if (opix[u] < 0) continue;
        float4 acc = bv;
#pragma unroll
        for (int t = 0; t < 9; ++t) acc = f4fma(v[u][t], wt[t], acc);
        {
          float a4[4] = {acc.x, acc.y, acc.z, acc.w};
          sr_activate_group(a4, sr_uniform(p.slope));
          acc = make_float4(a4[0], a4[1], a4[2], a4[3]);
        }
        *reinterpret_cast<float4*>(outb + (int64_t)opix[u] * p.out_sp) = acc;
        sum.x += acc.x; sum.y += acc.y; sum.z += acc.z; sum.w += acc.w;
      }
    }
  }
  if (p.pool) {
    red[xl][c4] = sum;
    __syncthreads();
    for (int s = DW_XL / 2; s > 0; s >>= 1) {
      if (xl < s) {
        const float4 a = red[xl][c4], o = red[xl + s][c4];
        red[xl][c4] = make_float4(a.x + o.x, a.y + o.y, a.z + o.z, a.w + o.w);
      }
      __syncthreads();
    }
    if (xl == 0 && live)
      *reinterpret_cast<float4*>(p.pool + ((int64_t)b * p.bands + band) * p.C + c) = red[0][c4];
  }
}

struct SrSeParams {
  const float* pool; int bands; float inv_count;
  const float* w1; const float* b1;
  const float* w2; const float* b2;
  float* gate;
  int C, rd;
};

__global__ __launch_bounds__(256) void sr_se_gate_kernel(SrSeParams p) {
  extern __shared__ float sm[];
  float* mean = sm;
  float* hid = sm + p.C;
  const int b = blockIdx.x;
  for (int c = threadIdx.x; c < p.C; c += 256) {
    float s = 0.f;
    for (int k = 0; k < p.bands; ++k) s += p.pool[((int64_t)b * p.bands + k) * p.C + c];
    mean[c] = s * p.inv_count;
  }
  __syncthreads();
  const int lane = threadIdx.x & 63, wave = threadIdx.x >> 6;
  for (int j = wave; j < p.rd; j += 4) {
    float s = 0.f;
    for (int c = lane; c < p.C; c += 64) s = fmaf(p.w1[(int64_t)j * p.C + c], mean[c], s);
#pragma unroll
    for (int o = 32; o > 0; o >>= 1) s += __shfl_xor(s, o);
    if (lane == 0) hid[j] = sr_activate(s + (p.b1 ? p.b1[j] : 0.f), SR_ACT_SILU);
  }
  __syncthreads();
  for (int c = threadIdx.x; c < p.C; c += 256) {
    float s = p.b2 ? p.b2[c] : 0.f;
    for (int j = 0; j < p.rd; ++j) s = fmaf(p.w2[(int64_t)c * p.rd + j], hid[j], s);
    p.gate[(int64_t)b * p.C + c] = 1.0f / (1.0f + __expf(-s));
  }
}

__global__ __launch_bounds__(256) void sr_se_hidden_kernel(SrSeParams p, float* __restrict__ hidden) {
  extern __shared__ float mean[];
  const int lane = threadIdx.x & 63, wave = threadIdx.x >> 6;
  const int j = blockIdx.x * 4 + wave, b = blockIdx.y;
  const float* __restrict__ pool = p.pool + (int64_t)b * p.bands * p.C;
  for (int c = threadIdx.x; c < p.C; c += 256) {
    float m = 0.f;
    for (int k0 = 0; k0 < p.bands; k0 += 16) {
      float v[16];
#pragma unroll
      for (int k = 0; k < 16; ++k) v[k] = (k0 + k < p.bands) ? pool[(int64_t)(k0 + k) * p.C + c] : 0.f;
#pragma unroll
      for (int k = 0; k < 16; ++k) m += v[k];
    }
    mean[c] = m * p.inv_count;
  }
  __syncthreads();
  if (j >= p.rd) return;
  const float* __restrict__ w = p.w1 + (int64_t)j * p.C;
  float s = 0.f;
  for (int c0 = 0; c0 < p.C; c0 += 64 * 8) {
    float v[8];
#pragma unroll
    for (int u = 0; u < 8; ++u) { const int c = c0 + 64 * u + lane; v[u] = c < p.C ? w[c] : 0.f; }
#pragma unroll
    for (int u = 0; u < 8; ++u) { const int c = c0 + 64 * u + lane; s = fmaf(v[u], c < p.C ? mean[c] : 0.f, s); }
  }
#pragma unroll
  for (int o = 32; o > 0; o >>= 1) s += __shfl_xor(s, o);
  if (lane == 0) hidden[(int64_t)b * p.rd + j] = sr_activate(s + (p.b1 ? p.b1[j] : 0.f), SR_ACT_SILU);
// ... 43 lines not shown
#pragma unroll
    for (int u = 0; u < 8; ++u) {
      const int px = px0 + 16 * u;
      v[u] = px < HW ? *reinterpret_cast<const float4*>(inb + (int64_t)px * in_sp) : make_float4(0.f, 0.f, 0.f, 0.f);
    }
#pragma unroll
    for (int u = 0; u < 8; ++u) {
      const int px = px0 + 16 * u;
      if (px < HW)
        *reinterpret_cast<float4*>(outb + (int64_t)px * out_sp) =
            make_float4(v[u].x * gv.x, v[u].y * gv.y, v[u].z * gv.z, v[u].w * gv.w);
    }
  }
}

__global__ __launch_bounds__(256) void sr_scale_channels_kernel(const float* __restrict__ in, int64_t in_sb, int in_sp,
                                                                const float* __restrict__ gate,
                                                                float* __restrict__ out, int64_t out_sb, int out_sp,
                                                                int HW, int C4) {
  const int b = blockIdx.y;
  const int64_t n = (int64_t)HW * C4;
  for (int64_t e = blockIdx.x * 256 + threadIdx.x; e < n; e += (int64_t)gridDim.x * 256) {
    const int px = (int)(e / C4), c4 = (int)(e - (int64_t)px * C4);
    const float4 g = *reinterpret_cast<const float4*>(gate + ((int64_t)b * C4 + c4) * 4);
    float4 v = *reinterpret_cast<const float4*>(in + (int64_t)b * in_sb + (int64_t)px * in_sp + 4 * c4);
    v.x *= g.x; v.y *= g.y; v.z *= g.z; v.w *= g.w;
    *reinterpret_cast<float4*>(out + (int64_t)b * out_sb + (int64_t)px * out_sp + 4 * c4) = v;
  }
}

__global__ __launch_bounds__(256) void sr_add_kernel(const float* __restrict__ a, int64_t a_sb, int a_sp,
                                                     const float* __restrict__ b_, int64_t b_sb, int b_sp,
                                                     float* __restrict__ out, int64_t out_sb, int out_sp, int HW,
                                                     int C4) {
  const int b = blockIdx.y;
  const int64_t n = (int64_t)HW * C4;
  for (int64_t e = blockIdx.x * 256 + threadIdx.x; e < n; e += (int64_t)gridDim.x * 256) {
    const int px = (int)(e / C4), c4 = (int)(e - (int64_t)px * C4);
    const float4 u = *reinterpret_cast<const float4*>(a + (int64_t)b * a_sb + (int64_t)px * a_sp + 4 * c4);
    const float4 v = *reinterpret_cast<const float4*>(b_ + (int64_t)b * b_sb + (int64_t)px * b_sp + 4 * c4);
    *reinterpret_cast<float4*>(out + (int64_t)b * out_sb + (int64_t)px * out_sp + 4 * c4) =
        make_float4(u.x + v.x, u.y + v.y, u.z + v.z, u.w + v.w);
  }
}

template <int COUT>
__global__ __launch_bounds__(256) void sr_rgb_stem3x3s2_kernel(const float* __restrict__ img, int64_t sb, int64_t sc, int64_t sy,
                                                               int64_t sx, const float* __restrict__ w ,
                                                               const float* __restrict__ bias, float* __restrict__ out,
                                                               int64_t out_sb, int out_sp, int H, int W, int Ho, int Wo,
                                                               int pad_y, int pad_x, float slope) {
  const int b = blockIdx.y;
  const int64_t npix = (int64_t)Ho * Wo;
  for (int64_t pix = blockIdx.x * (int64_t)blockDim.x + threadIdx.x; pix < npix; pix += (int64_t)gridDim.x * blockDim.x) {
    const int oy = (int)(pix / Wo), ox = (int)(pix - (int64_t)oy * Wo);
    float acc[COUT];
#pragma unroll
    for (int c = 0; c < COUT; ++c) acc[c] = bias ? bias[c] : 0.0f;
#pragma unroll
    for (int ky = 0; ky < 3; ++ky) {
      const int iy = 2 * oy - pad_y + ky;
#pragma unroll
      for (int kx = 0; kx < 3; ++kx) {
        const int ix = 2 * ox - pad_x + kx;
        const bool ok = (iy >= 0) & (iy < H) & (ix >= 0) & (ix < W);
        const float* q = img + b * sb + (ok ? iy * sy + ix * sx : 0);
#pragma unroll
        for (int ci = 0; ci < 3; ++ci) {
          const float v = ok ? q[ci * sc] : 0.0f;
          const float* wr = w + ((ky * 3 + kx) * 3 + ci) * COUT;
#pragma unroll
          for (int c = 0; c < COUT; ++c) acc[c] = fmaf(v, wr[c], acc[c]);
        }
      }
    }
    sr_activate_group(acc, sr_uniform(slope));
    float* o = out + b * out_sb + pix * out_sp;
#pragma unroll
    for (int c = 0; c < COUT; c += 4) *reinterpret_cast<float4*>(o + c) = make_float4(acc[c], acc[c + 1], acc[c + 2], acc[c + 3]);
  }
}

inline bool aligned16(const void* ptr) { return (((uintptr_t)ptr) & 15) == 0; }

}

extern "C" int sr_dwconv3x3_pool_bands(int Ho) {
  if (Ho <= 0) return 0;
  const int rows = Ho > 64 ? 4 : 2;
  return (Ho + rows - 1) / rows;
}

extern "C" int sr_dwconv3x3_nhwc_fwd(const float* in, int64_t in_batch_stride, int in_pix_stride, const float* weight9c,
                                     const float* bias, float* out, int64_t out_batch_stride, int out_pix_stride,
                                     float* pool_partial, int B, int H, int W, int C, int stride, int pad_top,
                                     int pad_left, int pad_bottom, int pad_right, float leaky_slope, void* stream_) {
  if (B < 0 || H <= 0 || W <= 0 || C <= 0) return SR_ERR_INVALID_ARGUMENT;
  if (stride != 1 && stride != 2) return SR_ERR_UNSUPPORTED;
  if (pad_top < 0 || pad_left < 0 || pad_bottom < 0 || pad_right < 0 || pad_top > 2 || pad_left > 2 ||
      pad_bottom > 2 || pad_right > 2 || H + pad_top + pad_bottom < 3 || W + pad_left + pad_right < 3)
    return SR_ERR_INVALID_ARGUMENT;
  if (B == 0) return SR_OK;
  if (!in || !weight9c || !out) return SR_ERR_INVALID_ARGUMENT;
  if (C % 4 != 0 || in_pix_stride % 4 != 0 || out_pix_stride % 4 != 0 || in_batch_stride % 4 != 0 ||
      out_batch_stride % 4 != 0 || !aligned16(in) || !aligned16(out) || !aligned16(weight9c) ||
      (bias && !aligned16(bias)) || (pool_partial && !aligned16(pool_partial)))
    return SR_ERR_UNSUPPORTED;
  SrDwParams p;
  p.in = in; p.in_sb = in_batch_stride; p.in_sp = in_pix_stride;
  p.w = weight9c; p.bias = bias;
  p.out = out; p.out_sb = out_batch_stride; p.out_sp = out_pix_stride;
  p.pool = pool_partial;
  p.H = H; p.W = W; p.C = C; p.stride = stride; p.pad_y = pad_top; p.pad_x = pad_left;
  p.Ho = (H + pad_top + pad_bottom - 3) / stride + 1;
  p.Wo = (W + pad_left + pad_right - 3) / stride + 1;
  p.bands = sr_dwconv3x3_pool_bands(p.Ho);
  p.rows = (p.Ho + p.bands - 1) / p.bands;
  p.slope = leaky_slope;
  if ((int64_t)H * W * in_pix_stride >= (1ll << 31) || (int64_t)p.Ho * p.Wo * out_pix_stride >= (1ll << 31))
    return SR_ERR_UNSUPPORTED;
  dim3 grid((C + DW_CH - 1) / DW_CH, p.bands, B);
  hipLaunchKernelGGL(sr_dwconv3x3_kernel, grid, dim3(256), 0, (hipStream_t)stream_, p);
  return sr_hip_rc(hipGetLastError());
}

extern "C" int sr_se_gate_fwd(const float* pool_partial, int bands, int pixels, const float* w_reduce,
                              const float* b_reduce, const float* w_expand, const float* b_expand, float* gate, int B,
                              int C, int rd, void* stream_) {
  if (B < 0 || C <= 0 || rd <= 0 || bands <= 0 || pixels <= 0) return SR_ERR_INVALID_ARGUMENT;
  if (B == 0) return SR_OK;
  if (!pool_partial || !w_reduce || !w_expand || !gate) return SR_ERR_INVALID_ARGUMENT;
  const size_t lds = (size_t)(C + rd) * sizeof(float);
  if (lds > 64 * 1024) return SR_ERR_UNSUPPORTED;
  SrSeParams p;
  p.pool = pool_partial; p.bands = bands; p.inv_count = 1.0f / (float)pixels;
  p.w1 = w_reduce; p.b1 = b_reduce; p.w2 = w_expand; p.b2 = b_expand; p.gate = gate; p.C = C; p.rd = rd;
  hipLaunchKernelGGL(sr_se_gate_kernel, dim3(B), dim3(256), lds, (hipStream_t)stream_, p);
  return sr_hip_rc(hipGetLastError());
}

extern "C" int sr_scale_channels_nhwc_fwd(const float* in, int64_t in_batch_stride, int in_pix_stride,
                                          const float* gate, float* out, int64_t out_batch_stride, int out_pix_stride,
                                          int B, int H, int W, int C, void* stream_) {
  if (B < 0 || H <= 0 || W <= 0 || C <= 0) return SR_ERR_INVALID_ARGUMENT;
  if (B == 0) return SR_OK;
  if (!in || !gate || !out) return SR_ERR_INVALID_ARGUMENT;
  if (C % 4 != 0 || in_pix_stride % 4 != 0 || out_pix_stride % 4 != 0 || in_batch_stride % 4 != 0 ||
      out_batch_stride % 4 != 0 || !aligned16(in) || !aligned16(out) || !aligned16(gate))
    return SR_ERR_UNSUPPORTED;
  const int64_t n = (int64_t)H * W * (C / 4);
  const int blocks = (int)((n + 256 * 4 - 1) / (256 * 4));
  dim3 grid(blocks < 1 ? 1 : (blocks > 2048 ? 2048 : blocks), B);
  hipLaunchKernelGGL(sr_scale_channels_kernel, grid, dim3(256), 0, (hipStream_t)stream_, in, in_batch_stride,
                     in_pix_stride, gate, out, out_batch_stride, out_pix_stride, H * W, C / 4);
  return sr_hip_rc(hipGetLastError());
}

extern "C" int sr_add_nhwc_fwd(const float* a, int64_t a_batch_stride, int a_pix_stride, const float* b,
                               int64_t b_batch_stride, int b_pix_stride, float* out, int64_t out_batch_stride,
                               int out_pix_stride, int B, int H, int W, int C, void* stream_) {
  if (B < 0 || H <= 0 || W <= 0 || C <= 0) return SR_ERR_INVALID_ARGUMENT;
  if (B == 0) return SR_OK;
  if (!a || !b || !out) return SR_ERR_INVALID_ARGUMENT;
  if (C % 4 != 0 || a_pix_stride % 4 != 0 || b_pix_stride % 4 != 0 || out_pix_stride % 4 != 0 ||
      a_batch_stride % 4 != 0 || b_batch_stride % 4 != 0 || out_batch_stride % 4 != 0 || !aligned16(a) ||
      !aligned16(b) || !aligned16(out))
    return SR_ERR_UNSUPPORTED;
  const int64_t n = (int64_t)H * W * (C / 4);
  const int blocks = (int)((n + 256 * 4 - 1) / (256 * 4));
  dim3 grid(blocks < 1 ? 1 : (blocks > 2048 ? 2048 : blocks), B);
  hipLaunchKernelGGL(sr_add_kernel, grid, dim3(256), 0, (hipStream_t)stream_, a, a_batch_stride, a_pix_stride, b,
                     b_batch_stride, b_pix_stride, out, out_batch_stride, out_pix_stride, H * W, C / 4);
  return sr_hip_rc(hipGetLastError());
}

extern "C" int sr_rgb_stem3x3s2_fwd(const float* image, int64_t sb, int64_t sc, int64_t sy, int64_t sx, const float* weight27c,
                                    const float* bias, float* out, int64_t out_batch_stride, int out_pix_stride, int B, int H,
                                    int W, int Cout, int pad_top, int pad_left, int Ho, int Wo, float act_code, void* stream_) {
  if (B < 0 || H <= 0 || W <= 0 || Ho <= 0 || Wo <= 0 || pad_top < 0 || pad_left < 0) return SR_ERR_INVALID_ARGUMENT;
  if (B == 0) return SR_OK;
  if (!image || !weight27c || !out) return SR_ERR_INVALID_ARGUMENT;
  if (Cout != 24 || out_pix_stride % 4 != 0 || out_batch_stride % 4 != 0 || !aligned16(out)) return SR_ERR_UNSUPPORTED;
  if (2 * (Ho - 1) - pad_top >= H || 2 * (Wo - 1) - pad_left >= W) return SR_ERR_INVALID_ARGUMENT;
  const int64_t npix = (int64_t)Ho * Wo;
  const int blocks = (int)((npix + 255) / 256 < 4096 ? (npix + 255) / 256 : 4096);
  hipLaunchKernelGGL((sr_rgb_stem3x3s2_kernel<24>), dim3(blocks, B), dim3(256), 0, (hipStream_t)stream_, image, sb, sc, sy, sx,
                     weight27c, bias, out, out_batch_stride, out_pix_stride, H, W, Ho, Wo, pad_top, pad_left, act_code);
  return sr_hip_rc(hipGetLastError());
}

extern "C" int sr_se_gate2_fwd(const float* pool_partial, int bands, int pixels, const float* w_reduce,
                               const float* b_reduce, const float* w_expand, const float* b_expand, float* hidden,
                               float* gate, int B, int C, int rd, void* stream_) {
  if (B < 0 || C <= 0 || rd <= 0 || bands <= 0 || pixels <= 0) return SR_ERR_INVALID_ARGUMENT;
  if (B == 0) return SR_OK;
  if (!pool_partial || !w_reduce || !w_expand || !hidden || !gate) return SR_ERR_INVALID_ARGUMENT;
  if (rd > 256 || C > 16384) return SR_ERR_UNSUPPORTED;
  SrSeParams p;
  p.pool = pool_partial; p.bands = bands; p.inv_count = 1.0f / (float)pixels;
  p.w1 = w_reduce; p.b1 = b_reduce; p.w2 = w_expand; p.b2 = b_expand; p.gate = gate; p.C = C; p.rd = rd;
  hipStream_t stream = (hipStream_t)stream_;
  hipLaunchKernelGGL(sr_se_hidden_kernel, dim3((rd + 3) / 4, B), dim3(256), (size_t)C * sizeof(float), stream, p, hidden);
  hipLaunchKernelGGL(sr_se_scale_kernel, dim3((C + DW_CH - 1) / DW_CH, B), dim3(256), 0, stream, p, (const float*)hidden,
                     (const float*)nullptr, (int64_t)0, 0, (float*)nullptr, (int64_t)0, 0, 0);
  return sr_hip_rc(hipGetLastError());
// ... 24 lines not shown
```

simplerecon_amd/csrc/sr_options.hip:

```cpp
#include <atomic>
#include <map>
#include <mutex>
#include <utility>
#include <stdlib.h>
#include <string.h>

#include "sr_common.h"

namespace {

struct OptDef { const char* name; int dflt; int kind; };
const OptDef kDefs[SR_OPT_COUNT] = {
    {"SR_MLP_SPLIT", 0, 1},       {"SR_WINO_SPLIT", 0, 1},     {"SR_WINO_XCD", 1, 0},        {"SR_WINO_NT", 0, 0},
    {"SR_WINO_KSPLIT", 0, 0},     {"SR_CONV_WINO", 1, 0},      {"SR_CONV_TILE", 0, 0},       {"SR_CONV_KSPLIT", 1, 0},
    {"SR_PW_NT", 0, 0},           {"SR_PW_KS", 0, 0},          {"SR_PT_CFG", -1, 0},         {"SR_PT_KS", 0, 0},
    {"SR_DOT_LDS", 1, 0},         {"SR_DOT_LDS_G", 0, 0},      {"SR_DOT_LDS_CULL", 1, 0},    {"SR_DOT_LDS_CAP", 634, 0},
    {"SR_UPSAMPLE_QUAD", 1, 0},   {"SR_POOL_STREAM", 1, 0},    {"SR_MLP_TILE", 0, 2},
};
std::atomic<int> g_val[SR_OPT_COUNT];
std::once_flag g_once;

int parse(const OptDef& d, const char* e) {
  if (d.kind == 1) {
    if (!e || !*e || !strcmp(e, "0") || !strcmp(e, "off") || !strcmp(e, "fp32")) return 0;
    if (!strcmp(e, "bf16")) return 1;
    if (!strcmp(e, "f16") || !strcmp(e, "fp16")) return 2;
    return -1;
  }
  if (d.kind == 2) {
    static const char* const names[] = {"auto", "flat", "2x32", "4x16", "8x8"};
    if (!e || !*e) return d.dflt;
    for (int i = 0; i < 5; ++i)
      if (!strcmp(e, names[i])) return i;
    return -1;
  }
  return (e && *e) ? atoi(e) : d.dflt;
}

void init() {
  for (int i = 0; i < SR_OPT_COUNT; ++i) {
    const char* e = getenv(kDefs[i].name);
    g_val[i].store(e ? parse(kDefs[i], e) : kDefs[i].dflt, std::memory_order_relaxed);
  }
}

}

int sr_opt(int id) {
  std::call_once(g_once, init);
  return g_val[id].load(std::memory_order_relaxed);
}

extern "C" int sr_option_count(void) { return SR_OPT_COUNT; }

extern "C" const char* sr_option_name(int id) { return (id >= 0 && id < SR_OPT_COUNT) ? kDefs[id].name : nullptr; }

extern "C" int sr_option_id(const char* name) {
  if (!name) return -1;
  for (int i = 0; i < SR_OPT_COUNT; ++i)
    if (!strcmp(kDefs[i].name, name)) return i;
  return -1;
}

extern "C" int sr_option_get(int id, int* value) {
  if (id < 0 || id >= SR_OPT_COUNT || !value) return SR_ERR_INVALID_ARGUMENT;
  *value = sr_opt(id);
  return SR_OK;
}

extern "C" int sr_option_set(int id, int value, int* previous) {
  if (id < 0 || id >= SR_OPT_COUNT) return SR_ERR_INVALID_ARGUMENT;
  std::call_once(g_once, init);
  const int old = g_val[id].exchange(value, std::memory_order_relaxed);
  if (previous) *previous = old;
  return SR_OK;
}

extern "C" int sr_option_default(int id, int* value) {
  if (id < 0 || id >= SR_OPT_COUNT || !value) return SR_ERR_INVALID_ARGUMENT;
  *value = kDefs[id].dflt;
  return SR_OK;
}

int sr_device_cus() {
  constexpr int kMaxDevices = 64;
  static std::atomic<int> cus[kMaxDevices];
  int dev = 0;
  if (hipGetDevice(&dev) != hipSuccess || dev < 0 || dev >= kMaxDevices) return 256;
  int v = cus[dev].load(std::memory_order_relaxed);
  if (v == 0) {
    if (hipDeviceGetAttribute(&v, hipDeviceAttributeMultiprocessorCount, dev) != hipSuccess || v <= 0) v = 256;
    cus[dev].store(v, std::memory_order_relaxed);
  }
  return v;
}

hipError_t sr_allow_lds(const void* kernel, size_t bytes) {
  static std::mutex mu;
  static std::map<std::pair<const void*, int>, size_t> granted;
  int dev = 0;
  if (hipError_t e = hipGetDevice(&dev)) return e;
  std::lock_guard<std::mutex> lock(mu);
  size_t& have = granted[{kernel, dev}];
  if (bytes <= have) return hipSuccess;
  if (hipError_t e = hipFuncSetAttribute(kernel, hipFuncAttributeMaxDynamicSharedMemorySize, (int)bytes)) return e;
  have = bytes;
  return hipSuccess;
}
```

simplerecon_amd/csrc/sr_pw.hip:

```cpp
#include <stdlib.h>

#include "sr_buffer.h"
#include "sr_view.h"

namespace {

template <int IO>
__device__ __forceinline__ float pw_load_elem(__amdgpu_buffer_rsrc_t r, unsigned voff, unsigned soff) {
  if (IO == 0) return __builtin_bit_cast(float, __builtin_amdgcn_raw_buffer_load_b32(r, (int)voff, (int)soff, 0));
  return sr_widen<IO>(__builtin_amdgcn_raw_buffer_load_b16(r, (int)voff, (int)soff, 0));
}
template <int IO>
__device__ __forceinline__ void pw_store_elem(float v, __amdgpu_buffer_rsrc_t r, unsigned voff, unsigned soff) {
  if (IO == 0) __builtin_amdgcn_raw_buffer_store_b32(__builtin_bit_cast(unsigned, v), r, (int)voff, (int)soff, 0);
  else __builtin_amdgcn_raw_buffer_store_b16(sr_narrow<IO>(v), r, (int)voff, (int)soff, 0);
}
struct SrPwParams {
  const float* in; int64_t in_sb; int in_sp;
  const float* wp;
  const float* bias;
  const float* gate;
  const float* res; int64_t res_sb; int res_sp;
  float* out; int64_t out_sb; int out_sp;
  int B, HW, Cin, Cout, Co_pad, G, G8;
// ... 115 lines not shown
      float rv[16];
#pragma unroll
      for (int r = 0; r < 16; ++r) {
        const int dr = (r & 3) + 8 * (r >> 2);
        const bool ok = full || (okc && row0 + 4 * kk + dr < p.HW);
        rv[r] = pw_load_elem<IO>(rs_res, ok ? r_base : SR_OOB, (unsigned)dr * (unsigned)p.res_sp * ES);
      }
#pragma unroll
      for (int r = 0; r < 16; ++r) v[r] += rv[r];
    }
    sr_activate_group(v, slope);
#pragma unroll
    for (int r = 0; r < 16; ++r) {
      const int dr = (r & 3) + 8 * (r >> 2);
      const bool ok = full || (okc && row0 + 4 * kk + dr < p.HW);
      pw_store_elem<IO>(v[r], rs_out, ok ? o_base : SR_OOB, (unsigned)dr * (unsigned)p.out_sp * ES);
    }
  }
}

struct PwPlan { int nt, ks; };

PwPlan pw_plan(int B, int HW, int Cin, int Cout) {
  const int f_nt = sr_opt(SR_OPT_PW_NT), f_ks = sr_opt(SR_OPT_PW_KS);
  const long mt = (long)B * ((HW + 31) / 32);
  const int n32 = (Cout + 31) / 32;
  const int g8 = (Cin + 7) / 8;
  const long want = (long)sr_device_cus() * 4 * 3 / 2;
  PwPlan best = {1, 1};
  double best_cost = -1.0;
  const int nts[4] = {4, 2, 1, 5};
  for (int a = 0; a < 4; ++a) {
    const int nt = nts[a];
    if (nt == 5 && n32 % 5 != 0) continue;
    if (f_nt > 0 && nt != f_nt) continue;
    for (int ks = 1; ks <= 4; ks *= 2) {
      if (f_ks > 0 && ks != f_ks) continue;
      if (ks > 1 && g8 / ks < 8) continue;
      if (ks > 1 && nt > 2) continue;
      if (nt == 5 && ks > 1) continue;
      const int nblocks = (n32 + nt - 1) / nt;
      const long waves = mt * nblocks * ks;
      const double pad = (double)(nblocks * nt) / n32;
      const double fill = waves >= want ? 1.0 : (double)want / (double)waves;
      const double cost = pad * fill * (1.0 + 0.25 / nt) * (1.0 + (ks > 1 ? 1.5 * ks / g8 : 0.0));
      if (best_cost < 0 || cost < best_cost) { best = {nt, ks}; best_cost = cost; }
    }
  }
  return best;
}

template <int NT, int KS>
int pw_launch(const SrPwParams& p, hipStream_t stream, int io) {
  const int mt_per_wg = 4 / KS;
  const long wgs = ((long)p.total_mt + mt_per_wg - 1) / mt_per_wg * p.n_blocks;
  const size_t lds = KS > 1 ? (size_t)mt_per_wg * (KS - 1) * NT * 16 * 64 * sizeof(float) : 0;
  if (io == 1) hipLaunchKernelGGL((sr_pw_kernel<NT, KS, false, 1>), dim3((unsigned)wgs), dim3(256), lds, stream, p);
  else if (io == 2) hipLaunchKernelGGL((sr_pw_kernel<NT, KS, false, 2>), dim3((unsigned)wgs), dim3(256), lds, stream, p);
  else if (p.gate) hipLaunchKernelGGL((sr_pw_kernel<NT, KS, true>), dim3((unsigned)wgs), dim3(256), lds, stream, p);
  else hipLaunchKernelGGL((sr_pw_kernel<NT, KS, false>), dim3((unsigned)wgs), dim3(256), lds, stream, p);
  return sr_hip_rc(hipGetLastError());
}

}

extern "C" int sr_pw_conv_supported(int Cin, int Cout) { return (Cin > 0 && Cout > 0 && Cin % 4 == 0) ? 1 : 0; }

extern "C" int sr_pw_conv_plan(int B, int HW, int Cin, int Cout, int* nt, int* ks) {
  if (B <= 0 || HW <= 0 || Cin <= 0 || Cout <= 0) return SR_ERR_INVALID_ARGUMENT;
  const PwPlan pl = pw_plan(B, HW, Cin, Cout);
  if (nt) *nt = pl.nt;
  if (ks) *ks = pl.ks;
  return SR_OK;
}

static int pw_run(const float* in, int64_t in_batch_stride, int in_pix_stride, const float* packed_w,
                  const float* bias, const float* gate, const float* residual, int64_t res_batch_stride,
                  int res_pix_stride, float* out, int64_t out_batch_stride, int out_pix_stride, int B,
                  int HW, int Cin, int Cout, float act_code, void* stream_, int io) {
  if (B < 0 || HW <= 0 || Cin <= 0 || Cout <= 0 || io < 0 || io > 2) return SR_ERR_INVALID_ARGUMENT;
  if (B == 0) return SR_OK;
  if (!in || !packed_w || !out) return SR_ERR_INVALID_ARGUMENT;
  if (io && gate) return SR_ERR_UNSUPPORTED;
  if (Cin % 4 != 0 || !sr_rows_aligned(in, in_batch_stride, in_pix_stride, io ? 7 : 15, 4) || (gate && !sr_ptr_aligned(gate, 15)))
    return SR_ERR_UNSUPPORTED;
  if (!sr_view_fits32(HW, in_pix_stride, Cin, 4) || !sr_view_fits32(HW, out_pix_stride, Cout, 4) ||
      (residual && !sr_view_fits32(HW, res_pix_stride, Cout, 4)))
    return SR_ERR_UNSUPPORTED;
  SrPwParams p;
  p.in = in; p.in_sb = in_batch_stride; p.in_sp = in_pix_stride;
  p.wp = packed_w; p.bias = bias; p.gate = gate;
  p.res = residual; p.res_sb = res_batch_stride; p.res_sp = res_pix_stride;
  p.out = out; p.out_sb = out_batch_stride; p.out_sp = out_pix_stride;
  p.B = B; p.HW = HW; p.Cin = Cin; p.Cout = Cout;
  p.Co_pad = ((Cout + 31) / 32) * 32;
  p.G = ((Cin + 63) / 64) * 8;
  p.G8 = (Cin + 7) / 8;
  p.m_tiles = (HW + 31) / 32;
  p.total_mt = B * p.m_tiles;
  p.slope = act_code;
  const PwPlan pl = pw_plan(B, HW, Cin, Cout);
  p.n_blocks = (p.Co_pad / 32 + pl.nt - 1) / pl.nt;
  hipStream_t stream = (hipStream_t)stream_;
  switch (pl.nt * 10 + pl.ks) {
    case 11: return pw_launch<1, 1>(p, stream, io);
    case 12: return pw_launch<1, 2>(p, stream, io);
    case 14: return pw_launch<1, 4>(p, stream, io);
    case 21: return pw_launch<2, 1>(p, stream, io);
    case 22: return pw_launch<2, 2>(p, stream, io);
    case 24: return pw_launch<2, 4>(p, stream, io);
    case 41: return pw_launch<4, 1>(p, stream, io);
    case 51: return pw_launch<5, 1>(p, stream, io);
    default: return SR_ERR_UNSUPPORTED;
  }
}

extern "C" int sr_pw_conv_nhwc_fwd(const float* in, int64_t in_batch_stride, int in_pix_stride, const float* packed_w,
                                   const float* bias, const float* gate, const float* residual, int64_t res_batch_stride,
                                   int res_pix_stride, float* out, int64_t out_batch_stride, int out_pix_stride, int B,
                                   int HW, int Cin, int Cout, float act_code, void* stream_) {
  return pw_run(in, in_batch_stride, in_pix_stride, packed_w, bias, gate, residual, res_batch_stride, res_pix_stride, out,
                out_batch_stride, out_pix_stride, B, HW, Cin, Cout, act_code, stream_, 0);
}

extern "C" int sr_pw_conv_io_nhwc_fwd(const void* in, int64_t in_batch_stride, int in_pix_stride, const float* packed_w,
                                      const float* bias, const void* residual, int64_t res_batch_stride, int res_pix_stride,
                                      void* out, int64_t out_batch_stride, int out_pix_stride, int B, int HW, int Cin, int Cout,
                                      float act_code, int io_dtype, void* stream_) {
  return pw_run((const float*)in, in_batch_stride, in_pix_stride, packed_w, bias, nullptr, (const float*)residual,
                res_batch_stride, res_pix_stride, (float*)out, out_batch_stride, out_pix_stride, B, HW, Cin, Cout, act_code,
                stream_, io_dtype);
}
```

simplerecon_amd/csrc/sr_pw_tiled.hip:

```cpp
#include <stdlib.h>

#include "sr_buffer.h"
#include "sr_view.h"

namespace {

constexpr int PT_KS = 32;
constexpr int PT_AROW = PT_KS + 4;

struct SrPtParams {
  const float* in; int in_sp;
  const float* wp;
  const float* bias; const float* gate;
  const float* res; int res_sp;
  float* out; int out_sp;
  int64_t part_stride;
  int M, HW, Cin, Cout, Co_pad, G;
  int slabs, slabs_per_part, ksplit, tiles_n;
  float slope;
};

template <int WM, int WN, int NTW, bool GATE>
__global__ __launch_bounds__(256, 2) void sr_pw_tiled_kernel(SrPtParams p) {
  constexpr int BM = 32 * WM, BN = 32 * WN * NTW;
// ... 99 lines not shown
    const float bv = (!partial && p.bias && okc) ? p.bias[col] : 0.0f;
    float v[16];
#pragma unroll
    for (int r = 0; r < 16; ++r) v[r] = acc[n][r] + bv;
    if (!partial && p.res) {
      float rv[16];
#pragma unroll
      for (int r = 0; r < 16; ++r) {
        const int m = rbase + (r & 3) + 8 * (r >> 2);
        rv[r] = (okc && m < p.M) ? p.res[(int64_t)m * p.res_sp + col] : 0.0f;
      }
#pragma unroll
      for (int r = 0; r < 16; ++r) v[r] += rv[r];
    }
    sr_activate_group(v, slope);
#pragma unroll
    for (int r = 0; r < 16; ++r) {
      const int m = rbase + (r & 3) + 8 * (r >> 2);
      if (okc && m < p.M) outp[(int64_t)m * p.out_sp + col] = v[r];
    }
  }
}

struct PtPlan { int cfg, ks; };
constexpr int PT_BM[4] = {64, 128, 128, 64}, PT_BN[4] = {128, 160, 64, 64};

PtPlan pt_plan(int M, int Cin, int Cout, bool can_split) {
  const int f_cfg = sr_opt(SR_OPT_PT_CFG), f_ks = sr_opt(SR_OPT_PT_KS);
  const int slabs = (Cin + PT_KS - 1) / PT_KS;
  const long want = (long)sr_device_cus() * 3 / 2;
  PtPlan best = {0, 1};
  double best_cost = -1.0;
  for (int cfg = 0; cfg < 4; ++cfg) {
    if (f_cfg >= 0 && cfg != f_cfg) continue;
    const long tm = (M + PT_BM[cfg] - 1) / PT_BM[cfg], tn = (Cout + PT_BN[cfg] - 1) / PT_BN[cfg];
    const double pad = (double)(tm * PT_BM[cfg]) * (double)(tn * PT_BN[cfg]) / ((double)M * Cout);
    for (int ks = 1; ks <= 8; ks *= 2) {
      if (f_ks > 0 && ks != f_ks) continue;
      if (ks > 1 && (!can_split || slabs / ks < 4)) continue;
      const long wgs = tm * tn * ks;
      const double fill = wgs >= want ? 1.0 : (double)want / (double)wgs;
      const double reuse = 1.0 + 24.0 / (PT_BM[cfg] * PT_BN[cfg] / (double)(PT_BM[cfg] + PT_BN[cfg]));
      const double cost = pad * fill * reuse * (1.0 + (ks > 1 ? 0.10 + 2.0 * ks / slabs : 0.0));
      if (best_cost < 0 || cost < best_cost) { best = {cfg, ks}; best_cost = cost; }
    }
  }
  return best;
}

template <int WM, int WN, int NTW>
int pt_launch(const SrPtParams& p, int tiles_m, hipStream_t stream) {
  constexpr int BM = 32 * WM, BN = 32 * WN * NTW;
  const size_t lds = (size_t)2 * (BM * PT_AROW + (PT_KS / 8) * 2 * BN * 4) * sizeof(float);
  const dim3 grid((unsigned)(tiles_m * p.tiles_n), (unsigned)p.ksplit);
  auto kernel = p.gate ? sr_pw_tiled_kernel<WM, WN, NTW, true> : sr_pw_tiled_kernel<WM, WN, NTW, false>;
  if (hipError_t e = sr_allow_lds((const void*)kernel, lds)) return sr_hip_rc(e);
  hipLaunchKernelGGL(kernel, grid, dim3(256), lds, stream, p);
  return sr_hip_rc(hipGetLastError());
}

}

extern "C" size_t sr_pw_conv_tiled_workspace_bytes(int M, int Cin, int Cout) {
  if (M <= 0 || Cin <= 0 || Cout <= 0 || Cout % 4 != 0) return 0;
  const PtPlan pl = pt_plan(M, Cin, Cout, true);
  return pl.ks > 1 ? (size_t)pl.ks * M * Cout * sizeof(float) : 0;
}

extern "C" int sr_pw_conv_tiled_plan(int M, int Cin, int Cout, int can_split, int* cfg, int* ks) {
  if (M <= 0 || Cin <= 0 || Cout <= 0) return SR_ERR_INVALID_ARGUMENT;
  const PtPlan pl = pt_plan(M, Cin, Cout, can_split != 0 && Cout % 4 == 0);
  if (cfg) *cfg = pl.cfg;
  if (ks) *ks = pl.ks;
  return SR_OK;
}

extern "C" int sr_pw_conv_tiled_nhwc_fwd(const float* in, int in_pix_stride, const float* packed_w, const float* bias,
                                         const float* gate, const float* residual, int res_pix_stride, float* out,
                                         int out_pix_stride, int M, int HW, int Cin, int Cout, float act_code,
                                         void* workspace, size_t workspace_bytes, void* stream_) {
  if (M < 0 || HW <= 0 || Cin <= 0 || Cout <= 0) return SR_ERR_INVALID_ARGUMENT;
  if (M == 0) return SR_OK;
  if (!in || !packed_w || !out) return SR_ERR_INVALID_ARGUMENT;
  if (Cin % 4 != 0 || !sr_rows_aligned(in, 0, in_pix_stride, 15, 4) || (gate && !sr_ptr_aligned(gate, 15)))
    return SR_ERR_UNSUPPORTED;
  const bool can_split = workspace && sr_ptr_aligned(workspace, 15) && Cout % 4 == 0 &&
                         (!residual || sr_rows_aligned(residual, 0, res_pix_stride, 15, 4)) &&
                         sr_rows_aligned(out, 0, out_pix_stride, 15, 4) && (!bias || sr_ptr_aligned(bias, 15));
  PtPlan pl = pt_plan(M, Cin, Cout, can_split);
  if (pl.ks > 1 && workspace_bytes < (size_t)pl.ks * M * Cout * sizeof(float)) pl = pt_plan(M, Cin, Cout, false);
  SrPtParams p;
  p.in = in; p.in_sp = in_pix_stride; p.wp = packed_w; p.bias = bias; p.gate = gate;
  p.res = residual; p.res_sp = res_pix_stride;
  p.M = M; p.HW = HW; p.Cin = Cin; p.Cout = Cout;
  p.Co_pad = ((Cout + 31) / 32) * 32;
  p.G = ((Cin + 63) / 64) * 8;
  p.slabs = (Cin + PT_KS - 1) / PT_KS;
  p.ksplit = pl.ks;
  p.slabs_per_part = (p.slabs + pl.ks - 1) / pl.ks;
  p.slope = act_code;
  p.part_stride = (int64_t)M * Cout;
  if (pl.ks > 1) { p.out = (float*)workspace; p.out_sp = Cout; }
  else { p.out = out; p.out_sp = out_pix_stride; }
  const int tiles_m = (M + PT_BM[pl.cfg] - 1) / PT_BM[pl.cfg];
  p.tiles_n = (Cout + PT_BN[pl.cfg] - 1) / PT_BN[pl.cfg];
  hipStream_t stream = (hipStream_t)stream_;
  int rc;
  switch (pl.cfg) {
    case 0: rc = pt_launch<2, 2, 2>(p, tiles_m, stream); break;
    case 1: rc = pt_launch<4, 1, 5>(p, tiles_m, stream); break;
    case 2: rc = pt_launch<4, 1, 2>(p, tiles_m, stream); break;
    default: rc = pt_launch<2, 2, 1>(p, tiles_m, stream); break;
  }
  if (rc == SR_OK && pl.ks > 1)
    rc = sr_launch_splitk_reduce((const float*)workspace, pl.ks, p.part_stride, bias, residual, (int64_t)0, res_pix_stride,
                                 out, (int64_t)0, out_pix_stride, 1, M, Cout, act_code, stream);
  return rc;
}
```

simplerecon_amd/csrc/sr_wino.hip:

```cpp
#include <type_traits>

#include "sr_view.h"
#include "sr_wino.h"

__global__ void sr_wino_pack_kernel(const float* __restrict__ w, float* __restrict__ wu, int Co, int Ci, int G,
                                    int Co_pad) {
  const int64_t total = (int64_t)16 * G * 2 * Co_pad * 4;
  for (int64_t e = blockIdx.x * (int64_t)blockDim.x + threadIdx.x; e < total; e += (int64_t)gridDim.x * blockDim.x) {
    const int el = (int)(e & 3);
    int64_t r = e >> 2;
    const int co = (int)(r % Co_pad); r /= Co_pad;
    const int kk = (int)(r & 1); r >>= 1;
    const int g8 = (int)(r % G);
    const int xi = (int)(r / G);
    const int ci = 8 * g8 + 4 * kk + el;
    float v = 0.0f;
    if (co < Co && ci < Ci) {
      const float* g = w + ((int64_t)co * Ci + ci) * 9;
      const int ur = xi >> 2, uc = xi & 3;
      float rowv[3];
#pragma unroll
      for (int c = 0; c < 3; ++c) {
        const float g0 = g[c], g1 = g[3 + c], g2 = g[6 + c];
        rowv[c] = ur == 0 ? g0 : (ur == 1 ? (g0 + g1 + g2) * 0.5f : (ur == 2 ? (g0 - g1 + g2) * 0.5f : g2));
      }
      v = uc == 0 ? rowv[0]
                  : (uc == 1 ? (rowv[0] + rowv[1] + rowv[2]) * 0.5f
                             : (uc == 2 ? (rowv[0] - rowv[1] + rowv[2]) * 0.5f : rowv[2]));
    }
    wu[e] = v;
  }
}

template <int NT, bool VEC4, bool VOUT, int IO = 0>
__global__ __launch_bounds__(256, NT == 1 ? SR_WINO_NT1_WAVES : SR_WINO_WAVES) void sr_wino_kernel(SrWinoParams p) {
  static_assert(IO == 0 || (VEC4 && VOUT), "16-bit I/O exists for the vector staging / epilogue instantiation only");
  constexpr unsigned ES = SR_IO_ES(IO);
  extern __shared__ __attribute__((aligned(16))) float lds[];
  float* O = lds;
  float* rawA = lds + WN_V_FLOATS(NT);
  float* rawB = lds + WN_O_FLOATS(NT);
  const int tid = threadIdx.x;
  const int lane = tid & 63, wave = __builtin_amdgcn_readfirstlane(tid >> 6);
  const int i = lane & 31, kk = lane >> 5;
  const int chunks = (p.G >> 1) / p.ksplit;
  const int64_t rec = (int64_t)2 * p.Co_pad;
  constexpr int STEPS = 8;
  static_assert(8 % SR_WINO_NB == 0 && SR_WINO_PD < SR_WINO_NB, "the register rotation must line up across slabs");
  constexpr int NB = SR_WINO_NB, PD = SR_WINO_PD;

  const int t_ra = wave == 0 ? 0 : (wave == 2 ? 2 : 1), t_rb = wave == 0 ? 2 : (wave == 1 ? 2 : (wave == 2 ? 1 : 3));
  const float t_sign = wave == 1 ? 1.0f : -1.0f;
  const int rv_base = ((2 * (i >> 3)) * WN_PW + 2 * (i & 7)) * WN_ROW + 4 * kk;
  int rv_a = rv_base + t_ra * WN_PW * WN_ROW, rv_b = rv_base + t_rb * WN_PW * WN_ROW;
#define SR_WN_PIN(...) asm volatile("" : __VA_ARGS__)

#ifdef SR_WINO_TRACE
  int tr_region = -1;
  if (tid == 0) {
    p.trace[((size_t)blockIdx.x * SR_TR_REGIONS) * SR_TR_EVENTS + 15] =
        ((unsigned long long)__builtin_amdgcn_s_getreg(20 | (0 << 6) | (3 << 11)) << 32) |
        (unsigned long long)__builtin_amdgcn_s_getreg(4 | (0 << 6) | (31 << 11));
  }
#endif
  struct Region { int b, oy0, ox0, co0, ks; };
  const int xcd_g = (int)gridDim.x;
  auto decode = [&](int wk) {
    if (p.xcd_order && (xcd_g & 7) == 0) {
      const int r0 = wk / xcd_g * xcd_g;
      if (r0 + xcd_g <= p.total) { const int bb = wk - r0; wk = r0 + (bb & 7) * (xcd_g >> 3) + (bb >> 3); }
    }
    Region r;
    r.ks = wk % p.ksplit; wk /= p.ksplit;
    const int cb = wk % p.co_blocks; wk /= p.co_blocks;
    const int rx = wk % p.regions_x; wk /= p.regions_x;
    const int ry = wk % p.regions_y;
    r.b = wk / p.regions_y;
    r.oy0 = ry * (2 * WN_TR); r.ox0 = rx * (2 * WN_TC); r.co0 = cb * (32 * NT);
    return r;
  };
  int offs[WN_STAGE_PER_THREAD];
  unsigned s_org = 0;
  const float* in_b = p.in;
  __amdgpu_buffer_rsrc_t rs_in = sr_rsrc(p.in, 0);
  const int64_t in_img_bytes = ((int64_t)(p.H * p.W - 1) * p.in_sp + p.Cin) * ES;
  const int c_quad = 4 * (tid & 3);
  auto aim = [&](const Region& r) {
    in_b = reinterpret_cast<const float*>(reinterpret_cast<const char*>(p.in) + (int64_t)r.b * p.in_sb * ES);
    if (VEC4) {
      rs_in = sr_rsrc(in_b, in_img_bytes);
      const bool interior = (r.oy0 >= 1) & (r.oy0 + 2 * WN_TR + 1 <= p.H) & (r.ox0 >= 1) & (r.ox0 + 2 * WN_TC + 1 <= p.W);
      if (interior) {
        s_org = (unsigned)(((r.oy0 - 1) * p.W + (r.ox0 - 1)) * p.in_sp) * ES;
#pragma unroll
        for (int it = 0; it < WN_STAGE_PER_THREAD; ++it) {
          const int e = tid + it * 256;
          const int px = e >> 2;
          const int py = px / WN_PW, pxx = px - py * WN_PW;
          offs[it] = (it < WN_STAGE_PER_THREAD - 1 || e < WN_STAGE_ELEMS) ? (int)(((py * p.W + pxx) * p.in_sp + c_quad) * ES)
                                                                          : (int)SR_OOB;
        }
      } else {
        s_org = 0;
#pragma unroll
        for (int it = 0; it < WN_STAGE_PER_THREAD; ++it) {
          const int e = tid + it * 256;
          const int px = e >> 2;
          const int py = px / WN_PW, pxx = px - py * WN_PW;
          const int iy = r.oy0 - 1 + py, ix = r.ox0 - 1 + pxx;
          const bool ok = (e < WN_STAGE_ELEMS) & (iy >= 0) & (iy < p.H) & (ix >= 0) & (ix < p.W);
          offs[it] = ok ? (int)(((iy * p.W + ix) * p.in_sp + c_quad) * ES) : (int)SR_OOB;
        }
      }
    } else {
#pragma unroll
      for (int it = 0; it < WN_STAGE_PER_THREAD; ++it) {
        const int e = tid + it * 256;
        const int px = e >> 2, q = e & 3;
        const int py = px / WN_PW, pxx = px - py * WN_PW;
// ... 186 lines not shown
      constexpr int TILE_ROWS_PER_UNIT = (256 / CG) / 8;
      const int cg = tid % CG;
      const int tile0 = tid / CG;
      const int tr0 = tile0 >> 3, tc0 = tile0 & 7;
      const __amdgpu_buffer_rsrc_t rs_out = sr_rsrc(outp, ((int64_t)(p.H * p.W - 1) * out_sp + p.Cout) * ES);
      const __amdgpu_buffer_rsrc_t rs_res =
          sr_rsrc(resp ? (const void*)resp : (const void*)p.wu,
                  resp ? ((int64_t)(p.H * p.W - 1) * p.res_sp + p.Cout) * ES : (int64_t)0);
      const __amdgpu_buffer_rsrc_t rs_bias = sr_rsrc(bias_p ? (const void*)bias_p : (const void*)p.wu,
                                                     bias_p ? (int64_t)p.Cout * 4 : (int64_t)0);
      const bool okc = co0 + 4 * cg < p.Cout;
      const bool full = (oy0 + 2 * WN_TR <= p.H) & (ox0 + 2 * WN_TC <= p.W) & (co0 + CO <= p.Cout);
      const unsigned pix0 = (unsigned)((2 * tr0) * p.W + 2 * tc0);
      const unsigned v_out = (pix0 * out_sp + 4u * cg) * ES, v_res = (pix0 * (unsigned)p.res_sp + 4u * cg) * ES;
      const unsigned s_out0 = ((unsigned)(oy0 * p.W + ox0) * out_sp + (unsigned)co0) * ES;
      const unsigned s_res0 = ((unsigned)(oy0 * p.W + ox0) * (unsigned)p.res_sp + (unsigned)co0) * ES;
      auto d_pix = [&](int it, int q) {
        return (unsigned)((2 * TILE_ROWS_PER_UNIT * it + (q >> 1)) * p.W + (q & 1));
      };
      int o_wr = (wave * 2 * 32 + 4 * kk) * CO + i, o_rd = tile0 * CO + 4 * cg;
      asm volatile("" : "+v"(o_wr), "+v"(o_rd));
      float neg1s = -1.0f;
      asm volatile("" : "+s"(neg1s));
      const wn_f2 neg1 = {neg1s, neg1s};
      unsigned rsp4 = (unsigned)p.res_sp * ES, osp4 = out_sp * ES;
      SR_WN_PIN("+s"(rsp4), "+s"(osp4));
      const bool fast_leaky = slope >= 0.0f && slope <= 1.0f;
      const wn_f2 slope2 = {slope, slope};
      auto epilogue = [&](auto full_tag, auto res_tag) {
        constexpr bool FULL = decltype(full_tag)::value, RES = decltype(res_tag)::value;
        unsigned okm = 0;
        if (!FULL) {
#pragma unroll
          for (int it = 0; it < UNITS; ++it)
#pragma unroll
            for (int q = 0; q < 4; ++q) {
              const int oy = oy0 + 2 * (tr0 + TILE_ROWS_PER_UNIT * it) + (q >> 1), ox = ox0 + 2 * tc0 + (q & 1);
              okm |= (unsigned)(okc & (oy < p.H) & (ox < p.W)) << (4 * it + q);
            }
        }
        auto lane_off = [&](unsigned v, int it, int q) { return (FULL || ((okm >> (4 * it + q)) & 1u)) ? v : SR_OOB; };
        float4 rv[UNITS][4];
        if (RES) {
#pragma unroll
          for (int it = 0; it < UNITS; ++it)
#pragma unroll
            for (int q = 0; q < 4; ++q)
              rv[it][q] = wn_io_load<IO>(rs_res, lane_off(v_res, it, q), s_res0 + d_pix(it, q) * rsp4);
        }
        const float4 bv = wn_io_load<0>(rs_bias, (FULL || okc) ? 16u * cg : SR_OOB, (unsigned)co0 * 4u);
        SR_TR(10);
#pragma unroll
        for (int n = 0; n < NT; ++n) {
#pragma unroll
          for (int r = 0; r < 16; r += 2) {
            const wn_f2 m0 = {acc[0][n][r], acc[0][n][r + 1]}, m1 = {acc[1][n][r], acc[1][n][r + 1]};
            const wn_f2 m2 = {acc[2][n][r], acc[2][n][r + 1]}, m3 = {acc[3][n][r], acc[3][n][r + 1]};
            const wn_f2 c0 = (m0 + m1) + m2;
            const wn_f2 c1 = __builtin_elementwise_fma(neg1, m3, __builtin_elementwise_fma(neg1, m2, m1));
            float* o0 = &O[o_wr + ((r & 3) + 8 * (r >> 2)) * CO + 32 * n];
            float* o1 = o0 + 32 * CO;
            o0[0] = c0.x; o0[CO] = c0.y;
            o1[0] = c1.x; o1[CO] = c1.y;
          }
        }
        SR_TR(11);
        __syncthreads();
        SR_TR(13);
        __builtin_amdgcn_sched_barrier(0);
#pragma unroll
        for (int it = 0; it < UNITS; ++it) {
          float4 t[4][2];
#pragma unroll
          for (int ur = 0; ur < 4; ++ur)
#pragma unroll
            for (int bb = 0; bb < 2; ++bb)
              t[ur][bb] = *reinterpret_cast<const float4*>(&O[o_rd + ((ur * 2 + bb) * 32 + (256 / CG) * it) * CO]);
          const float4 y[4] = {f4add(f4add(t[0][0], t[1][0]), t[2][0]), f4add(f4add(t[0][1], t[1][1]), t[2][1]),
                               f4sub(f4sub(t[1][0], t[2][0]), t[3][0]), f4sub(f4sub(t[1][1], t[2][1]), t[3][1])};
          float o16[16];
#pragma unroll
          for (int q = 0; q < 4; ++q) {
            float4 v = f4add(y[q], bv);
            if (RES) v = f4add(v, rv[it][q]);
            if (fast_leaky) {
              const wn_f2 lo = wn_f2{v.x, v.y} * slope2, hi = wn_f2{v.z, v.w} * slope2;
              v = make_float4(sr_vmax(v.x, lo.x), sr_vmax(v.y, lo.y), sr_vmax(v.z, hi.x), sr_vmax(v.w, hi.y));
            }
            o16[4 * q + 0] = v.x; o16[4 * q + 1] = v.y; o16[4 * q + 2] = v.z; o16[4 * q + 3] = v.w;
          }
          if (!fast_leaky) sr_activate_group(o16, slope);
#pragma unroll
          for (int q = 0; q < 4; ++q) {
            sr_io_store<IO>(sr_f4{o16[4 * q], o16[4 * q + 1], o16[4 * q + 2], o16[4 * q + 3]}, rs_out,
                            lane_off(v_out, it, q), s_out0 + d_pix(it, q) * osp4);
          }
        }
      };
      if (full) { if (resp) epilogue(std::true_type{}, std::true_type{}); else epilogue(std::true_type{}, std::false_type{}); }
      else { if (resp) epilogue(std::false_type{}, std::true_type{}); else epilogue(std::false_type{}, std::false_type{}); }
#ifdef SR_WINO_TRACE
      if (tr_region > 0) SR_TR(15);
#endif
      __syncthreads();
      SR_TR(14);
    } else {
      constexpr int UNITS = 32 * CO / 256;
      float rv[UNITS][4];
      bool ok[UNITS][4];
      unsigned opix[UNITS][4];
      const int co = tid & (CO - 1);
      const int cog = co0 + co;
      const bool okc = cog < p.Cout;
#pragma unroll
      for (int it = 0; it < UNITS; ++it) {
        const int tile = tid / CO + (256 / CO) * it;
        const int tr = tile >> 3, tc = tile & 7;
#pragma unroll
        for (int q = 0; q < 4; ++q) {
          const int oy = oy0 + 2 * tr + (q >> 1), ox = ox0 + 2 * tc + (q & 1);
          ok[it][q] = okc & (oy < p.H) & (ox < p.W);
          opix[it][q] = (unsigned)(oy * p.W + ox);
          const bool ld = ok[it][q] & (resp != nullptr);
          const float v = (resp ? resp : p.in)[ld ? opix[it][q] * (unsigned)p.res_sp + cog : 0u];
          rv[it][q] = ld ? v : 0.0f;
        }
      }
#pragma unroll
      for (int n = 0; n < NT; ++n)
#pragma unroll
        for (int r = 0; r < 16; ++r) {
          const int tile = (r & 3) + 8 * (r >> 2) + 4 * kk;
          const float m0 = acc[0][n][r], m1 = acc[1][n][r], m2 = acc[2][n][r], m3 = acc[3][n][r];
          O[((wave * 2 + 0) * 32 + tile) * CO + 32 * n + i] = (m0 + m1) + m2;
          O[((wave * 2 + 1) * 32 + tile) * CO + 32 * n + i] = (m1 - m2) - m3;
        }
      __syncthreads();
      const float bv = (bias_p && okc) ? bias_p[cog] : 0.0f;
#pragma unroll
      for (int it = 0; it < UNITS; ++it) {
        const int tile = tid / CO + (256 / CO) * it;
        float t[4][2];
#pragma unroll
        for (int ur = 0; ur < 4; ++ur)
#pragma unroll
          for (int bb = 0; bb < 2; ++bb) t[ur][bb] = O[((ur * 2 + bb) * 32 + tile) * CO + co];
        const float y[4] = {(t[0][0] + t[1][0]) + t[2][0], (t[0][1] + t[1][1]) + t[2][1],
                            (t[1][0] - t[2][0]) - t[3][0], (t[1][1] - t[2][1]) - t[3][1]};
        float o4[4];
#pragma unroll
        for (int q = 0; q < 4; ++q) o4[q] = y[q] + bv + rv[it][q];
        sr_activate_group(o4, slope);
#pragma unroll
        for (int q = 0; q < 4; ++q)
          if (ok[it][q]) outp[opix[it][q] * out_sp + cog] = o4[q];
      }
      __syncthreads();
    }
    reg = has_next ? nxt : decode(work + (int)gridDim.x < p.total ? work + (int)gridDim.x : work);
  }
}

__global__ __launch_bounds__(256) void sr_wino_reduce_kernel(const float* __restrict__ part, int ksplit,
                                                             int64_t part_stride, const float* __restrict__ bias,
                                                             const float* __restrict__ res, int64_t res_sb, int res_sp,
                                                             float* __restrict__ out, int64_t out_sb, int out_sp,
                                                             int HW, int C4, float slope) {
  const int b = blockIdx.y;
  const int64_t total = (int64_t)HW * C4;
  for (int64_t idx = (int64_t)blockIdx.x * blockDim.x + threadIdx.x; idx < total; idx += (int64_t)gridDim.x * blockDim.x) {
    const int c4 = (int)(idx % C4);
    const int64_t px = idx / C4;
    const float* q = part + ((int64_t)b * HW + px) * (4 * C4) + 4 * c4;
    float4 v = *reinterpret_cast<const float4*>(q);
// ... 42 lines not shown
  const long regions = (long)((H + 7) / 8) * ((W + 15) / 16);
  const double util = (double)H * W / (double)(regions * 128);
  return (util >= 0.4 && Cin >= 16) ? 1 : 0;
}

struct SrWinoPlan { int nt, ks; };
static SrWinoPlan sr_wino_plan(int B, int H, int W, int Cin, int Cout, bool allow_split) {
  const int co_pad = ((Cout + 31) / 32) * 32;
  const int slabs = (Cin + 15) / 16;
  const int forced_nt = sr_opt(SR_OPT_WINO_NT), forced_ks = sr_opt(SR_OPT_WINO_KSPLIT);
  const long regions = (long)((H + 2 * WN_TR - 1) / (2 * WN_TR)) * ((W + 2 * WN_TC - 1) / (2 * WN_TC)) * B;
  const long cus = sr_device_cus(), slots = 2 * cus;
  SrWinoPlan best = {co_pad % 64 == 0 ? 2 : 1, 1};
  double best_cost = -1.0;
  for (int nt = 2; nt >= 1; --nt) {
    if (nt == 2 && co_pad % 64 != 0) continue;
    if ((forced_nt == 1 || forced_nt == 2) && nt != forced_nt && !(forced_nt == 2 && co_pad % 64 != 0)) continue;
    for (int ks = 1; ks <= 8; ks *= 2) {
      if (ks > 1 && (!allow_split || slabs % ks != 0 || slabs / ks < 4 || Cout % 4 != 0)) continue;
      if (forced_ks > 0 && ks != forced_ks && allow_split && slabs % forced_ks == 0 && slabs / forced_ks >= 1) continue;
      const long items = regions * (co_pad / (32 * nt)) * ks;
      const double f = ((double)slabs / ks + 2.0) / ((double)slabs + 2.0);
      const double t_lat = nt == 2 ? 1.0 : 0.6, t_thr = nt == 2 ? 0.82 : 0.46;
      const long n1 = (items + slots - 1) / slots, n2 = items / slots + (items % slots > cus ? 1 : 0);
      double cost = ((double)n2 * 2.0 * t_thr + (double)(n1 - n2) * t_lat) * f;
      if (ks > 1) cost += 2.7 / ((double)slabs + 2.0);
      if (nt == 1 || ks > 1) cost *= 1.03;
      if (best_cost < 0 || cost < best_cost) { best = {nt, ks}; best_cost = cost; }
    }
  }
  return best;
}

extern "C" int sr_wino_splitk_factor(int B, int H, int W, int Cin, int Cout) {
  if (B <= 0 || H <= 0 || W <= 0 || Cin <= 0 || Cout <= 0) return 1;
  return sr_wino_plan(B, H, W, Cin, Cout, true).ks;
}

extern "C" size_t sr_wino_splitk_workspace_bytes(int B, int H, int W, int Cin, int Cout) {
  const int ks = sr_wino_splitk_factor(B, H, W, Cin, Cout);
  return ks > 1 ? (size_t)ks * B * H * W * Cout * sizeof(float) : 0;
}

extern "C" const char* sr_wino_kernel_name(int B, int H, int W, int Cin, int Cout, int aligned_in, int aligned_out) {
  static thread_local char buf[64];
  const int vin = aligned_in != 0, vout = vin && aligned_out;
  snprintf(buf, sizeof(buf), "sr_wino_kernel<%d, %s, %s>", sr_wino_plan(B, H, W, Cin, Cout, vout != 0).nt,
           vin ? "true" : "false", vout ? "true" : "false");
  return buf;
}

static int sr_wino_run(const float* in, int64_t in_batch_stride, int in_pix_stride, const float* packed_u,
                       const float* bias, const float* residual, int64_t res_batch_stride, int res_pix_stride,
                       float* out, int64_t out_batch_stride, int out_pix_stride, int B, int H, int W, int Cin, int Cout,
                       float leaky_slope, void* workspace, size_t workspace_bytes, void* stream_, int io = 0) {
  if (io < 0 || io > 2) return SR_ERR_INVALID_ARGUMENT;
  const uintptr_t amask = io ? 7 : 15;
  if (B < 0 || H <= 0 || W <= 0 || Cin <= 0 || Cout <= 0) return SR_ERR_INVALID_ARGUMENT;
  if (B == 0) return SR_OK;
  if (!in || !packed_u || !out) return SR_ERR_INVALID_ARGUMENT;
  SrWinoParams p;
  p.in = in; p.in_sb = in_batch_stride; p.in_sp = in_pix_stride;
  p.wu = packed_u; p.bias = bias;
  p.res = residual; p.res_sb = res_batch_stride; p.res_sp = res_pix_stride;
  p.out = out; p.out_sb = out_batch_stride; p.out_sp = out_pix_stride;
  p.H = H; p.W = W; p.Cin = Cin; p.Cout = Cout;
  p.Co_pad = ((Cout + 31) / 32) * 32;
  p.G = ((Cin + 15) / 16) * 2;
  p.regions_x = (W + 2 * WN_TC - 1) / (2 * WN_TC);
  p.regions_y = (H + 2 * WN_TR - 1) / (2 * WN_TR);
  p.slope = leaky_slope;
  p.vec4 = sr_rows_aligned(in, in_batch_stride, in_pix_stride, amask, 4) && (Cin % 4 == 0);
  const bool vout = p.vec4 && (Cout % 4 == 0) && sr_rows_aligned(out, out_batch_stride, out_pix_stride, amask, 4) &&
                    (!bias || sr_ptr_aligned(bias, 15)) &&
                    (!residual || sr_rows_aligned(residual, res_batch_stride, res_pix_stride, amask, 4));
  if (io && !vout) return SR_ERR_UNSUPPORTED;
  const int split = sr_wino_split_mode();
  if (split < 0) return SR_ERR_INVALID_ARGUMENT;
  if (split && (io || !vout)) return SR_ERR_UNSUPPORTED;
  const int64_t HW = (int64_t)H * W;
  if (p.vec4 && !sr_view_fits32(HW, in_pix_stride, Cin, 4)) return SR_ERR_UNSUPPORTED;
  if (vout && (!sr_view_fits32(HW, out_pix_stride, Cout, 4) || (residual && !sr_view_fits32(HW, res_pix_stride, Cout, 4))))
    return SR_ERR_UNSUPPORTED;
  const bool can_split = !io && vout && workspace && sr_ptr_aligned(workspace, 15);
  SrWinoPlan plan = sr_wino_plan(B, H, W, Cin, Cout, can_split);
  if (plan.ks > 1 && workspace_bytes < (size_t)plan.ks * B * H * W * Cout * sizeof(float))
    plan = sr_wino_plan(B, H, W, Cin, Cout, false);
  const int nt = plan.nt;
  p.ksplit = plan.ks;
  p.part = (float*)workspace;
  p.part_stride = (int64_t)B * H * W * Cout;
  p.co_blocks = p.Co_pad / (32 * nt);
  p.total = p.regions_x * p.regions_y * p.co_blocks * B * p.ksplit;
  p.xcd_order = sr_opt(SR_OPT_WINO_XCD);
  hipStream_t stream = (hipStream_t)stream_;
  int blocks = sr_device_cus() * (nt == 1 ? SR_WINO_NT1_WAVES : SR_WINO_WAVES);
  if (blocks > p.total) blocks = p.total;
  const size_t lds = (size_t)WN_LDS_FLOATS(nt) * sizeof(float);
#ifdef SR_WINO_TRACE
  static unsigned long long* trace_buf = nullptr;
  static int launches = 0;
  const size_t trace_n = (size_t)blocks * SR_TR_REGIONS * SR_TR_EVENTS;
  if (!trace_buf) (void)hipMalloc((void**)&trace_buf, (size_t)1024 * SR_TR_REGIONS * SR_TR_EVENTS * 8);
  (void)hipMemsetAsync(trace_buf, 0, trace_n * 8, stream);
  p.trace = trace_buf;
#endif
#define SR_WINO_LAUNCH_IO(NTV, IOV)                                                                              \
  {                                                                                                               \
    if (hipError_t e = sr_allow_lds((const void*)sr_wino_kernel<NTV, true, true, IOV>, lds)) return sr_hip_rc(e); \
    hipLaunchKernelGGL((sr_wino_kernel<NTV, true, true, IOV>), dim3(blocks), dim3(256), lds, stream, p);          \
  }
#define SR_WINO_LAUNCH(NTV, V4, VO)                                                                               \
  {                                                                                                               \
    if (hipError_t e = sr_allow_lds((const void*)sr_wino_kernel<NTV, V4, VO>, lds)) return sr_hip_rc(e);          \
    hipLaunchKernelGGL((sr_wino_kernel<NTV, V4, VO>), dim3(blocks), dim3(256), lds, stream, p);                   \
  }
  if (split) { const int rc = sr_wino_split_launch(p, nt, blocks, split, stream); if (rc) return rc; }
  else if (io == 1 && nt == 2) SR_WINO_LAUNCH_IO(2, 1)
  else if (io == 1) SR_WINO_LAUNCH_IO(1, 1)
  else if (io == 2 && nt == 2) SR_WINO_LAUNCH_IO(2, 2)
  else if (io == 2) SR_WINO_LAUNCH_IO(1, 2)
  else if (nt == 2 && vout) SR_WINO_LAUNCH(2, true, true)
  else if (nt == 2 && p.vec4) SR_WINO_LAUNCH(2, true, false)
  else if (nt == 2) SR_WINO_LAUNCH(2, false, false)
  else if (vout) SR_WINO_LAUNCH(1, true, true)
  else if (p.vec4) SR_WINO_LAUNCH(1, true, false)
  else SR_WINO_LAUNCH(1, false, false)
#undef SR_WINO_LAUNCH
#undef SR_WINO_LAUNCH_IO
#ifdef SR_WINO_TRACE
  {
    const char* path = getenv("SR_WINO_TRACE_FILE");
    const char* at = getenv("SR_WINO_TRACE_LAUNCH");
    if (path && ++launches == (at ? atoi(at) : 10)) {
      (void)hipStreamSynchronize(stream);
      unsigned long long* host = (unsigned long long*)malloc(trace_n * 8);
      (void)hipMemcpy(host, trace_buf, trace_n * 8, hipMemcpyDeviceToHost);
      FILE* f = fopen(path, "wb");
      if (f) { int hdr[4] = {blocks, SR_TR_REGIONS, SR_TR_EVENTS, p.G / 2}; fwrite(hdr, 4, 4, f); fwrite(host, 8, trace_n, f); fclose(f); }
      free(host);
    }
  }
#endif
  int rc = sr_hip_rc(hipGetLastError());
  if (rc == SR_OK && p.ksplit > 1) {
    rc = sr_launch_splitk_reduce(p.part, p.ksplit, p.part_stride, bias, residual, res_batch_stride, res_pix_stride, out,
                                 out_batch_stride, out_pix_stride, B, H * W, Cout, leaky_slope, stream);
  }
  return rc;
}

extern "C" int sr_conv3x3_wino_nhwc_fwd(const float* in, int64_t in_batch_stride, int in_pix_stride,
                                        const float* packed_u, const float* bias, const float* residual,
                                        int64_t res_batch_stride, int res_pix_stride, float* out,
                                        int64_t out_batch_stride, int out_pix_stride, int B, int H, int W, int Cin,
                                        int Cout, float leaky_slope, void* stream_) {
  return sr_wino_run(in, in_batch_stride, in_pix_stride, packed_u, bias, residual, res_batch_stride, res_pix_stride, out,
                     out_batch_stride, out_pix_stride, B, H, W, Cin, Cout, leaky_slope, nullptr, 0, stream_);
}

extern "C" int sr_conv3x3_wino_io_nhwc_fwd(const void* in, int64_t in_batch_stride, int in_pix_stride, const float* packed_u,
                                           const float* bias, const void* residual, int64_t res_batch_stride,
                                           int res_pix_stride, void* out, int64_t out_batch_stride, int out_pix_stride, int B,
                                           int H, int W, int Cin, int Cout, float leaky_slope, int io_dtype, void* stream_) {
  return sr_wino_run((const float*)in, in_batch_stride, in_pix_stride, packed_u, bias, (const float*)residual,
                     res_batch_stride, res_pix_stride, (float*)out, out_batch_stride, out_pix_stride, B, H, W, Cin, Cout,
                     leaky_slope, nullptr, 0, stream_, io_dtype);
}

extern "C" int sr_conv3x3_wino_splitk_nhwc_fwd(const float* in, int64_t in_batch_stride, int in_pix_stride,
                                               const float* packed_u, const float* bias, const float* residual,
                                               int64_t res_batch_stride, int res_pix_stride, float* out,
                                               int64_t out_batch_stride, int out_pix_stride, int B, int H, int W,
                                               int Cin, int Cout, float leaky_slope, void* workspace,
                                               size_t workspace_bytes, void* stream_) {
  return sr_wino_run(in, in_batch_stride, in_pix_stride, packed_u, bias, residual, res_batch_stride, res_pix_stride, out,
                     out_batch_stride, out_pix_stride, B, H, W, Cin, Cout, leaky_slope, workspace, workspace_bytes,
                     stream_);
}
```

simplerecon_amd/csrc/sr_wino4.hip:

```cpp
#include <stdio.h>
#include <stdlib.h>

#include "sr_buffer.h"
#include "sr_view.h"

namespace {

constexpr int W4_PS = 18;
constexpr int W4_RS = 20;
constexpr int W4_RAW_FLOATS = W4_PS * W4_PS * W4_RS;
constexpr int W4_V_FLOATS = 36 * 16 * 16;
constexpr int W4_LDS_BYTES = (W4_RAW_FLOATS + W4_V_FLOATS) * 4;
constexpr int W4_STAGE = 6;
#ifndef SR_W4_NA
#define SR_W4_NA 3
#define SR_W4_PD 2
#endif
constexpr int W4_NA = SR_W4_NA, W4_PD = SR_W4_PD;
#ifndef SR_W4_PRIO
#define SR_W4_PRIO 2
#endif
__device__ __forceinline__ void w4_prio_other() { if (SR_W4_PRIO) __builtin_amdgcn_s_setprio(SR_W4_PRIO); }
__device__ __forceinline__ void w4_prio_mfma() { if (SR_W4_PRIO) __builtin_amdgcn_s_setprio(0); }

// ... 804 lines not shown
  (void)hipGetLastError();
  return SR_ERR_UNSUPPORTED;
}

}

extern "C" size_t sr_wino4_packed_weight_floats(int Cout, int Cin) {
  if (Cout <= 0 || Cin <= 0) return 0;
  const size_t S = (size_t)(Cin + 15) / 16, Co_pad = (size_t)((Cout + 63) / 64) * 64;
  return 36 * S * 4 * Co_pad * 4;
}

extern "C" int sr_wino4_pack_weights(const float* weight, int Cout, int Cin, float* packed, void* stream_) {
  if (!weight || !packed || Cout <= 0 || Cin <= 0) return SR_ERR_INVALID_ARGUMENT;
  const int S = (Cin + 15) / 16, Co_pad = ((Cout + 63) / 64) * 64;
  hipLaunchKernelGGL(sr_wino4_pack_kernel, dim3(512), dim3(256), 0, (hipStream_t)stream_, weight, packed, Cout, Cin, S, Co_pad);
  return sr_hip_rc(hipGetLastError());
}

extern "C" int sr_conv_prefers_wino4(int B, int H, int W, int Cin, int Cout, int mode) {
  if (mode == 0 || B <= 0 || H <= 0 || W <= 0 || Cin <= 0 || Cout <= 0 || Cin % 4 != 0 || Cout % 4 != 0) return 0;
  if (mode == 2) return 1;
  const long regions = (long)((H + 15) / 16) * ((W + 15) / 16);
  const double util = (double)H * W / (double)(regions * 256);
  const int co_blocks = (Cout + 63) / 64;
  const double co_util = (double)Cout / (double)(co_blocks * 64);
  const long items = regions * B * co_blocks;
  const long cus = sr_device_cus();
  if (co_util < 0.99 || Cin < 16) return 0;
  if (items >= 2 * cus) {
    const long rounds = (items + cus - 1) / cus;
    const double fill = (double)items / (double)(rounds * cus);
    if (util < 0.9 || fill < 0.8) return 0;
    return 3;
  }
  if (items * 10 >= cus * 6 && items <= cus && util >= 0.75) return 3;
  return 0;
}

#ifdef SR_W4_TRACE
static unsigned long long* w4_trace_buf = nullptr;
static int w4_trace_launches = 0;
static void w4_trace_begin(SrWino4Params& p, hipStream_t stream) {
  const size_t trace_n = (size_t)16 * 2 * W4_TR_N;
  if (!w4_trace_buf) (void)hipMalloc((void**)&w4_trace_buf, trace_n * 8);
  (void)hipMemsetAsync(w4_trace_buf, 0, trace_n * 8, stream);
  p.trace = w4_trace_buf;
}
static void w4_trace_end(int blocks, hipStream_t stream) {
  const size_t trace_n = (size_t)16 * 2 * W4_TR_N;
  const char* at = getenv("SR_W4_TRACE_LAUNCH");
  if (++w4_trace_launches != (at ? atoi(at) : 10)) return;
  (void)hipStreamSynchronize(stream);
  unsigned long long* host = (unsigned long long*)malloc(trace_n * 8);
  (void)hipMemcpy(host, w4_trace_buf, trace_n * 8, hipMemcpyDeviceToHost);
  for (int b = 0; b < 16 && b < blocks; b += 5)
    for (int g = 0; g < 2; ++g) {
      fprintf(stderr, "W4TRACE block %d group %d:", b, g);
      unsigned long long t0 = host[((size_t)b * 2 + 0) * W4_TR_N] & 0xffffffffffffffull, prev = 0;
      for (int i = 0; i < W4_TR_N; ++i) {
        const unsigned long long v = host[((size_t)b * 2 + g) * W4_TR_N + i];
        if (!v) break;
        const unsigned long long t = (v & 0xffffffffffffffull) - t0;
        fprintf(stderr, " %d@%llu(+%llu)", (int)(v >> 56), t, t - prev);
        prev = t;
      }
      fprintf(stderr, "\n");
    }
  {
    const unsigned long long* t = host + (W4_TR_N - 4);
    if (t[3] > t[1]) fprintf(stderr, "W4CLOCK %.3f GHz over %.1f us\n", 0.1 * (double)(t[2] - t[0]) / (double)(t[3] - t[1]),
                             (double)(t[3] - t[1]) * 0.01);
  }
  free(host);
}
#endif

static int w4_run(const float* in, int64_t in_batch_stride, int in_pix_stride, const float* packed_u, const float* bias,
                  const float* residual, int64_t res_batch_stride, int res_pix_stride, float* out, int64_t out_batch_stride,
                  int out_pix_stride, int B, int H, int W, int Cin, int Cout, float leaky_slope, int variant, void* stream_) {
  if (B < 0 || H <= 0 || W <= 0 || Cin <= 0 || Cout <= 0) return SR_ERR_INVALID_ARGUMENT;
  if (B == 0) return SR_OK;
  if (!in || !packed_u || !out) return SR_ERR_INVALID_ARGUMENT;
  if (Cin % 4 != 0 || Cout % 4 != 0 || !sr_rows_aligned(in, in_batch_stride, in_pix_stride, 15, 4) ||
      !sr_rows_aligned(out, out_batch_stride, out_pix_stride, 15, 4) || (bias && !sr_ptr_aligned(bias, 15)) ||
      (residual && !sr_rows_aligned(residual, res_batch_stride, res_pix_stride, 15, 4)))
    return SR_ERR_UNSUPPORTED;
  const int64_t lim = (int64_t)1 << 31;
  const int64_t HW = (int64_t)H * W;
  if (!sr_view_fits32(HW, in_pix_stride, Cin, 4) || !sr_view_fits32(HW, out_pix_stride, Cout, 4) ||
      (residual && !sr_view_fits32(HW, res_pix_stride, Cout, 4)))
    return SR_ERR_UNSUPPORTED;
  SrWino4Params p;
  p.in = in; p.in_sb = in_batch_stride; p.in_sp = in_pix_stride;
  p.wu = packed_u; p.bias = bias;
  p.res = residual; p.res_sb = res_batch_stride; p.res_sp = res_pix_stride;
  p.out = out; p.out_sb = out_batch_stride; p.out_sp = out_pix_stride;
  p.B = B; p.H = H; p.W = W; p.Cin = Cin; p.Cout = Cout;
  p.Co_pad = ((Cout + 63) / 64) * 64;
  p.S = (Cin + 15) / 16;
  if ((int64_t)36 * p.S * 4 * p.Co_pad * 16 >= lim) return SR_ERR_UNSUPPORTED;
  p.regions_x = (W + 15) / 16;
  p.regions_y = (H + 15) / 16;
  p.co_blocks = p.Co_pad / 64;
  const int64_t total = (int64_t)p.regions_x * p.regions_y * p.co_blocks * B;
  if (total >= lim) return SR_ERR_UNSUPPORTED;
  p.total = (int)total;
  p.slope = leaky_slope;
  if (variant == 3) {
    int blocks = sr_device_cus();
    if (blocks > p.total) blocks = p.total;
    const bool generic_act = !((leaky_slope >= 0.0f && leaky_slope <= 1.0f) || (leaky_slope < 0.0f && leaky_slope > -1.5f));
    auto kernel = generic_act ? (residual ? sr_wino4ws_kernel<true, true> : sr_wino4ws_kernel<true, false>)
                              : (residual ? sr_wino4ws_kernel<false, true> : sr_wino4ws_kernel<false, false>);
    if (int rc = w4_allow_lds((const void*)kernel, W4_WS_LDS_BYTES)) return rc;
#ifdef SR_W4_TRACE
    w4_trace_begin(p, (hipStream_t)stream_);
#endif
    hipLaunchKernelGGL(kernel, dim3(blocks), dim3(512), W4_WS_LDS_BYTES, (hipStream_t)stream_, p);
#ifdef SR_W4_TRACE
    w4_trace_end(blocks, (hipStream_t)stream_);
#endif
    return sr_hip_rc(hipGetLastError());
  }
  if (variant != 2) {
    int blocks = 2 * sr_device_cus();
    if (blocks > p.total) blocks = p.total;
    if (int rc = w4_allow_lds((const void*)sr_wino4_kernel, W4_LDS_BYTES)) return rc;
    hipLaunchKernelGGL(sr_wino4_kernel, dim3(blocks), dim3(256), W4_LDS_BYTES, (hipStream_t)stream_, p);
    return sr_hip_rc(hipGetLastError());
  }
  int blocks = sr_device_cus();
  if (blocks > (p.total + 1) / 2) blocks = (p.total + 1) / 2;
#ifdef SR_W4_TRACE
  w4_trace_begin(p, (hipStream_t)stream_);
#endif
  if (int rc = w4_allow_lds((const void*)sr_wino4pp_kernel, 2 * W4_LDS_BYTES)) return rc;
  hipLaunchKernelGGL(sr_wino4pp_kernel, dim3(blocks), dim3(512), 2 * W4_LDS_BYTES, (hipStream_t)stream_, p);
#ifdef SR_W4_TRACE
  w4_trace_end(blocks, (hipStream_t)stream_);
#endif
  return sr_hip_rc(hipGetLastError());
}

extern "C" int sr_conv3x3_wino4_nhwc_fwd(const float* in, int64_t in_batch_stride, int in_pix_stride, const float* packed_u,
                                         const float* bias, const float* residual, int64_t res_batch_stride,
                                         int res_pix_stride, float* out, int64_t out_batch_stride, int out_pix_stride, int B,
                                         int H, int W, int Cin, int Cout, float leaky_slope, void* stream_) {
  return w4_run(in, in_batch_stride, in_pix_stride, packed_u, bias, residual, res_batch_stride, res_pix_stride, out,
                out_batch_stride, out_pix_stride, B, H, W, Cin, Cout, leaky_slope, 0, stream_);
}

extern "C" int sr_conv3x3_wino4_variant_nhwc_fwd(const float* in, int64_t in_batch_stride, int in_pix_stride,
                                                 const float* packed_u, const float* bias, const float* residual,
                                                 int64_t res_batch_stride, int res_pix_stride, float* out,
                                                 int64_t out_batch_stride, int out_pix_stride, int B, int H, int W, int Cin,
                                                 int Cout, float leaky_slope, int variant, void* stream_) {
  if (variant < 0 || variant > 3) return SR_ERR_INVALID_ARGUMENT;
  return w4_run(in, in_batch_stride, in_pix_stride, packed_u, bias, residual, res_batch_stride, res_pix_stride, out,
                out_batch_stride, out_pix_stride, B, H, W, Cin, Cout, leaky_slope, variant, stream_);
}
```

simplerecon_amd/image_encoder.py:

```python
from typing import List

import torch
from torch import nn

from . import ops
from . import train_ops as T


def _tf_pads(x, conv):
    pads = ops.tf_same_pads(x.shape[2], x.shape[3], conv.kernel_size[0], conv.stride[0])
    return None if pads == (1, 1, 1, 1) else pads

BN_EPS = 1e-3
STEM_CHANNELS = 24
STAGES = (("cn", 2, 1, 1, 24, 0.0), ("er", 4, 2, 4, 48, 0.0), ("er", 4, 2, 4, 64, 0.0),
          ("ir", 6, 2, 4, 128, 0.25), ("ir", 9, 1, 6, 160, 0.25), ("ir", 15, 2, 6, 256, 0.25))
FEATURE_STAGES = (0, 1, 2, 4, 5)


def _conv(cin, cout, k, stride=1, groups=1, bias=False):
    return nn.Conv2d(cin, cout, k, stride=stride, padding=k // 2, groups=groups, bias=bias)


def _bn(c):
    return nn.BatchNorm2d(c, eps=BN_EPS)


class ConvBnAct(nn.Module):

    def __init__(self, cin, cout, stride):
        super().__init__()
        self.conv, self.bn1 = _conv(cin, cout, 3, stride), _bn(cout)
        self.has_skip = stride == 1 and cin == cout

    def forward(self, x):
        y = ops.conv2d(x, self.conv, bn=self.bn1, act="silu", tf_same=True)
        return ops.add_(y, x) if self.has_skip else y

    def forward_train(self, x):
        y = T.batch_norm_act(T.conv(x, self.conv, pads=_tf_pads(x, self.conv)), self.bn1, act=T.ACT_SILU)
        return T.add(y, x) if self.has_skip else y


class EdgeResidual(nn.Module):

    def __init__(self, cin, cout, stride, expansion):
        super().__init__()
        mid = cin * expansion
        self.conv_exp, self.bn1 = _conv(cin, mid, 3, stride), _bn(mid)
        self.se = nn.Identity()
        self.conv_pwl, self.bn2 = _conv(mid, cout, 1), _bn(cout)
        self.has_skip = stride == 1 and cin == cout

    def forward(self, x):
        t = ops.conv2d(x, self.conv_exp, bn=self.bn1, act="silu", tf_same=True)
        return ops.conv2d(t, self.conv_pwl, bn=self.bn2, residual=x if self.has_skip else None)

    def forward_train(self, x):
        t = T.batch_norm_act(T.conv(x, self.conv_exp, pads=_tf_pads(x, self.conv_exp)), self.bn1, act=T.ACT_SILU)
        y = T.batch_norm_act(T.conv(t, self.conv_pwl), self.bn2)
        return T.add(y, x) if self.has_skip else y


class SqueezeExcite(nn.Module):
    def __init__(self, channels, reduced):
        super().__init__()
        self.conv_reduce = nn.Conv2d(channels, reduced, 1, bias=True)
        self.conv_expand = nn.Conv2d(reduced, channels, 1, bias=True)


class InvertedResidual(nn.Module):

    def __init__(self, cin, cout, stride, expansion, se_ratio):
        super().__init__()
        mid = cin * expansion
        self.conv_pw, self.bn1 = _conv(cin, mid, 1), _bn(mid)
        self.conv_dw, self.bn2 = _conv(mid, mid, 3, stride, groups=mid), _bn(mid)
        self.se = SqueezeExcite(mid, int(round(cin * se_ratio)))
        self.conv_pwl, self.bn3 = _conv(mid, cout, 1), _bn(cout)
        self.has_skip = stride == 1 and cin == cout

    def forward(self, x):
        t = ops.conv2d(x, self.conv_pw, bn=self.bn1, act="silu")
        d, pool = ops.dwconv3x3(t, self.conv_dw, bn=self.bn2, act="silu", tf_same=True, want_pool=True)
        gate = ops.se_gates(pool, d.shape[2] * d.shape[3], self.se.conv_reduce, self.se.conv_expand)
        return ops.conv2d(d, self.conv_pwl, bn=self.bn3, residual=x if self.has_skip else None, gate=gate)

    def forward_train(self, x):
        t = T.batch_norm_act(T.conv(x, self.conv_pw), self.bn1, act=T.ACT_SILU)
        pads = ops.tf_same_pads(t.shape[2], t.shape[3], 3, self.conv_dw.stride[0])
        d = T.batch_norm_act(T.dwconv3x3(t, self.conv_dw, pads), self.bn2, act=T.ACT_SILU)
        d = T.squeeze_excite(d, self.se.conv_reduce, self.se.conv_expand)
        y = T.batch_norm_act(T.conv(d, self.conv_pwl), self.bn3)
        return T.add(y, x) if self.has_skip else y


class _FeatureInfo:
    def __init__(self, chans, reductions):
        self._chans, self._red = list(chans), list(reductions)

    def channels(self):
        return list(self._chans)

    def reduction(self):
        return list(self._red)


class EfficientNetV2SFeatures(nn.Module):

    def __init__(self):
        super().__init__()
        self.conv_stem, self.bn1 = _conv(3, STEM_CHANNELS, 3, 2), _bn(STEM_CHANNELS)
        stages, cin = [], STEM_CHANNELS
        for kind, repeats, stride, expansion, cout, se_ratio in STAGES:
            blocks = []
            for i in range(repeats):
                s = stride if i == 0 else 1
                if kind == "cn":
                    blocks.append(ConvBnAct(cin, cout, s))
                elif kind == "er":
# ... 35 lines not shown
```

simplerecon_amd/ops.py:

```python
import ctypes as C
import contextlib
import os
import weakref

import torch
from torch import nn

from . import _lib

PROFILE = None

_PACKED = weakref.WeakKeyDictionary()
_NO_ENTRIES = {}
_FORGET_EPOCH = 0


def _cached(mod, tag, key, build, *args):
    e = _PACKED.get(mod, _NO_ENTRIES).get(tag)
    if e is not None and e[0] == key:
        if e[2] is not None:
            _await_pack(e)
        return e[1]
    payload = build(*args)
    fence = None
# ... 136 lines not shown


def _check_conv(conv):
    k = conv.kernel_size[0]
    if conv.kernel_size[0] != conv.kernel_size[1] or k not in (1, 3) or conv.groups != 1 \
            or conv.dilation != (1, 1) or tuple(conv.padding) != (k // 2,) * 2 \
            or conv.padding_mode not in ("zeros", "replicate"):
        raise _lib.HipLibraryError(f"unsupported Conv2d configuration for the HIP path: {conv}")


def _pack_folded(kind, conv, bn):
    _lib.require_device_f32("conv weight", conv.weight)
    _check_conv(conv)
    w, bias = _effective_weight(conv, bn)
    return _pack(kind, w), bias


def packed_weight(conv: nn.Conv2d, bn=None):
    return _cached(conv, "direct", _state_key(conv, bn), _pack_folded, "conv", conv, bn)


USE_PW_1X1 = True
PW_TILED = os.environ.get("SR_PW_TILED", "auto")
PW_TILED_MIN_ROWS = 100000


def _pack_linear(lin):
    return _pack("conv", lin.weight.detach().reshape(lin.out_features, lin.in_features, 1, 1).contiguous())


def linear(x, lin: nn.Linear, leaky=None):
    _lib.require_device_f32("linear input", x)
    _lib.refuse_autograd(x, lin.weight)
    cin, cout = lin.in_features, lin.out_features
    if x.shape[-1] != cin:
        raise ValueError(f"linear expects {cin} input features, got {x.shape[-1]}")
    x2 = x.reshape(-1, cin).contiguous()
    m = x2.shape[0]
    out = torch.empty((m, cout), dtype=torch.float32, device=x.device)
    if m == 0:
        return out.view(*x.shape[:-1], cout)
    wp = _cached(lin, "linear", _state_key(lin, None), _pack_linear, lin)
    bias = lin.bias.detach() if lin.bias is not None else None
    _lib.call("sr_conv2d_nhwc_fwd", x.device, x2, m * cin, cin, wp, bias, None, 0, 0, out, m * cout, cout, 1, 1, m, cin, cout,
              1, 1, -1.0 if leaky is None else float(leaky))
    return out.view(*x.shape[:-1], cout)


def wino_split_mode():
    return _lib.split_mode_name("SR_WINO_SPLIT")


def packed_wino_weight(conv: nn.Conv2d, bn=None):
    key = (_state_key(conv, bn), wino_split_mode())
    return _cached(conv, "wino", key, _pack_folded, "wino", conv, bn)


WINO4_MODE = int(os.environ.get("SR_CONV_WINO4", "1"))
WINO4_VARIANT = int(os.environ.get("SR_WINO4_VARIANT", "0"))


def packed_wino4_weight(conv: nn.Conv2d, bn=None):
    return _cached(conv, "wino4", _state_key(conv, bn), _pack_folded, "wino4", conv, bn)


_SHAPE_QUERIES = {}


def _drop_shape_queries(*_):
    _SHAPE_QUERIES.clear()


_lib.OPTION_LISTENERS.append(_drop_shape_queries)


def _shape_query(lib, name, *shape, dev=None):
    key = (name, shape, dev)
    v = _SHAPE_QUERIES.get(key)
    if v is None:
        v = _SHAPE_QUERIES[key] = getattr(lib, name)(*shape)
    return v


def conv2d(x, conv: nn.Conv2d, residual=None, leaky=None, out=None, bn=None, act=None, tf_same=False, gate=None):
    _lib.refuse_autograd(x, conv.weight)
    x = as_nhwc(x, "conv input")
    b, ci, h, w = x.shape
    if ci != conv.in_channels:
        raise ValueError(f"conv expects {conv.in_channels} input channels, got {ci}")
    k, s = conv.kernel_size[0], conv.stride[0]
    if conv.stride[0] != conv.stride[1] or s not in (1, 2):
        raise _lib.HipLibraryError(f"unsupported stride {conv.stride}")
    pads = tf_same_pads(h, w, k, s) if tf_same else (k // 2,) * 4
    ho, wo = (h + pads[0] + pads[2] - k) // s + 1, (w + pads[1] + pads[3] - k) // s + 1
    co = conv.out_channels
    if out is None:
        out = empty_nhwc(b, co, ho, wo, x.device)
    else:
        if tuple(out.shape) != (b, co, ho, wo) or not _is_nhwc_view(out):
            raise ValueError(f"`out` must be a channels-last view of shape {(b, co, ho, wo)}")
        _lib.require_device_f32("out", out)
    lib = _lib.lib()
    replicate = conv.padding_mode == "replicate"
    padded = pads != (k // 2,) * 4
    if padded and replicate:
        raise _lib.HipLibraryError("explicit padding is implemented for zero padding only")
    use_wino = (not replicate) and (not padded) and bool(_shape_query(lib, "sr_conv_prefers_wino", b, h, w, ci, co, k, s, dev=x.device.index))
    if residual is not None:
        residual = as_nhwc(residual, "residual")
        if tuple(residual.shape) != (b, co, ho, wo):
            raise ValueError(f"residual shape {tuple(residual.shape)} != output shape {(b, co, ho, wo)}")
    if b == 0:
        return out
    isb, isp = _strides(x)
    osb, osp = _strides(out)
    rsb, rsp = _strides(residual) if residual is not None else (0, 0)
    split = use_wino and wino_split_mode()
    if split and not (ci % 4 == 0 and co % 4 == 0 and _aligned16(x, isb, isp) and _aligned16(out, osb, osp)
                      and _aligned16(residual, rsb, rsp)):
        use_wino = split = False
    if gate is not None:
        _lib.require_device_f32("gate", gate)
        if k != 1 or s != 1 or tuple(gate.shape) != (b, ci) or not gate.is_contiguous():
            raise ValueError(f"`gate` needs a 1x1 / stride-1 conv and a contiguous [{b}, {ci}] tensor")
    slope = _act_code(leaky, act)
    strides = (isb, isp, osb, osp, rsb, rsp)
    if k == 1 and s == 1 and not padded and not replicate and (USE_PW_1X1 or gate is not None) and ci % 4 == 0 \
            and _aligned16(x, isb, isp):
        shape = (b, ci, h, w, co, k, s, ho, wo, residual is not None)
        if _conv_pointwise(lib, x, *packed_weight(conv, bn), residual, out, gate, strides, shape, slope) == 0:
            return out
    if gate is not None:
        raise _lib.HipLibraryError("a gated 1x1 convolution needs Cin % 4 == 0 and 16-byte aligned input rows")
    if k == 1 and s == 1 and (w % 32 != 0 or h % 4 != 0) and (isp, isb) == (ci, h * w * ci) \
            and (osp, osb) == (co, h * w * co) and (residual is None or (rsp, rsb) == (co, h * w * co)):
        m = b * h * w
        fw = 32 if m % 32 == 0 else 8 if m % 8 == 0 else 0
        if fw:
            b, h, w, ho, wo = 1, m // fw, fw, m // fw, fw
            strides = (m * ci, isp, m * co, osp, m * co if residual is not None else 0, rsp)
    shape = (b, ci, h, w, co, k, s, ho, wo, residual is not None)
    w4_form = _shape_query(lib, "sr_conv_prefers_wino4", b, h, w, ci, co, WINO4_MODE, dev=x.device.index) \
        if (use_wino and WINO4_MODE and not split) else 0
    if w4_form and _conv_wino4(lib, x, *packed_wino4_weight(conv, bn), residual, out, strides, shape, slope,
                               WINO4_VARIANT or w4_form) == 0:
        return out
    if use_wino:
        _lib.SPLIT_GUARD.acquire()
        try:
            if _conv_wino(lib, x, *packed_wino_weight(conv, bn), residual, out, strides, shape, slope) == 0:
                return out
        finally:
            _lib.SPLIT_GUARD.release()
        wp, bias = packed_weight(conv, bn)
        isb, isp, osb, osp, rsb, rsp = strides
        _lib.call("sr_conv2d_nhwc_fwd", x.device, x, isb, isp, wp, bias, residual, rsb, rsp, out, osb, osp, b, h, w, ci, co,
                  k, s, slope)
        return out
    _conv_direct(lib, x, *packed_weight(conv, bn), residual, out, strides, shape, slope, pads if padded else None, replicate)
    return out


def _aligned16(t, sb, sp):
    return t is None or (t.data_ptr() % 16 == 0 and sp % 4 == 0 and sb % 4 == 0)


def _timed(device, record, fn, *args):
    prof = PROFILE
    with _lib.on_device(device):
        if prof is None:
            return fn(*args)
        ev0, ev1 = torch.cuda.Event(enable_timing=True), torch.cuda.Event(enable_timing=True)
        ev0.record()
        rc = fn(*args)
        ev1.record()
        if rc == 0:
            name, flops, shape, executed = record()
            prof.append((name, flops, ev0, ev1, shape, executed))
    return rc


def _launch(x, shape, entry, fallback, describe, fn, *args):
    if PROFILE is None:
        with _lib.on_device(x.device):
            rc = fn(*args)
    else:
        def record():
            b, ci, h, w, co, k, s, ho, wo, _ = shape
            name, executed = describe()
            return name, 2.0 * b * ho * wo * co * ci * k * k, shape, executed
        rc = _timed(x.device, record, fn, *args)
    if rc != 0 and (rc != _lib.ERR_UNSUPPORTED or not fallback):
        _lib.check(rc, entry)
    return rc


def _conv_pointwise(lib, x, wp, bias, residual, out, gate, strides, shape, slope):
    isb, isp, osb, osp, rsb, rsp = strides
    b, ci, h, w, co = shape[:5]
    m = b * h * w
    dense = b == 1 or (isb == h * w * isp and osb == h * w * osp and (residual is None or rsb == h * w * rsp))
    gflag = "true" if gate is not None else "false"
    if dense and (PW_TILED == "1" or (PW_TILED == "auto" and m >= PW_TILED_MIN_ROWS)):
        nbytes = _shape_query(lib, "sr_pw_conv_tiled_workspace_bytes", m, ci, co, dev=x.device.index)
        ws = _workspace(x.device, "pw_splitk", nbytes) if nbytes else None

        def describe():
            a_, b_ = C.c_int(0), C.c_int(0)
            can_split = ws is not None and ws.data_ptr() % 16 == 0 and co % 4 == 0 and _aligned16(out, 0, osp) and \
                _aligned16(residual, 0, rsp) and (bias is None or bias.data_ptr() % 16 == 0)
            lib.sr_pw_conv_tiled_plan(m, ci, co, int(can_split), C.byref(a_), C.byref(b_))
            if b_.value > 1 and nbytes < b_.value * m * co * 4:
                lib.sr_pw_conv_tiled_plan(m, ci, co, 0, C.byref(a_), C.byref(b_))
            tile_m, tile_n = ((64, 128), (128, 160), (128, 64), (64, 64))[a_.value]
            executed = 2.0 * (-(-m // tile_m) * tile_m) * (-(-co // tile_n) * tile_n) * (-(-ci // 32) * 32)
            return f"sr_pw_tiled_kernel<{tile_m}x{tile_n}, ks {b_.value}, {gflag}>", executed
        return _launch(x, shape, "sr_pw_conv_tiled_nhwc_fwd", gate is None, describe, lib.sr_pw_conv_tiled_nhwc_fwd,
                       _lib.ptr(x), isp, _lib.ptr(wp), _lib.ptr(bias), _lib.ptr(gate), _lib.ptr(residual), rsp, _lib.ptr(out),
                       osp, m, h * w, ci, co, slope, _lib.ptr(ws), nbytes, _lib.stream_ptr(x.device))

    def describe():
        a_, b_ = C.c_int(0), C.c_int(0)
        lib.sr_pw_conv_plan(b, h * w, ci, co, C.byref(a_), C.byref(b_))
        mt = b * ((h * w + 31) // 32)
        executed = 2.0 * mt * 32 * ((co + 32 * a_.value - 1) // (32 * a_.value) * 32 * a_.value) * ((ci + 7) // 8 * 8)
        return f"sr_pw_kernel<{a_.value}, {b_.value}, {gflag}>", executed
    return _launch(x, shape, "sr_pw_conv_nhwc_fwd", gate is None, describe, lib.sr_pw_conv_nhwc_fwd, _lib.ptr(x), isb, isp,
                   _lib.ptr(wp), _lib.ptr(bias), _lib.ptr(gate), _lib.ptr(residual), rsb, rsp, _lib.ptr(out), osb, osp, b,
                   h * w, ci, co, slope, _lib.stream_ptr(x.device))


def _conv_wino4(lib, x, wp, bias, residual, out, strides, shape, slope, variant):
    isb, isp, osb, osp, rsb, rsp = strides
    b, ci, h, w, co = shape[:5]
    if not (_aligned16(x, isb, isp) and _aligned16(out, osb, osp) and _aligned16(residual, rsb, rsp)
            and (bias is None or bias.data_ptr() % 16 == 0)):
        return _lib.ERR_UNSUPPORTED

    def describe():
        regions = ((h + 15) // 16) * ((w + 15) // 16)
        executed = 2.0 * b * regions * 16 * 36 * ((ci + 15) // 16 * 16) * ((co + 63) // 64 * 64)
        return "sr_wino4ws_kernel" if variant == 3 else "sr_wino4_kernel", executed
    return _launch(x, shape, "sr_conv3x3_wino4_nhwc_fwd", True, describe, lib.sr_conv3x3_wino4_variant_nhwc_fwd, _lib.ptr(x),
                   isb, isp, _lib.ptr(wp), _lib.ptr(bias), _lib.ptr(residual), rsb, rsp, _lib.ptr(out), osb, osp, b, h, w, ci,
                   co, slope, variant, _lib.stream_ptr(x.device))
# ... 412 lines not shown
```

Measured before the change: 327.0.

## Fuse post-activation residual add into 3x3 conv epilogues and add blocked depthwise kernel

```diff
diff --git a/include/simplerecon_hip.h b/include/simplerecon_hip.h
--- a/include/simplerecon_hip.h
+++ b/include/simplerecon_hip.h
@@ -18,7 +18,7 @@
   SR_OPT_MLP_SPLIT = 0, SR_OPT_WINO_SPLIT, SR_OPT_WINO_XCD, SR_OPT_WINO_NT, SR_OPT_WINO_KSPLIT, SR_OPT_CONV_WINO,
   SR_OPT_CONV_TILE, SR_OPT_CONV_KSPLIT, SR_OPT_PW_NT, SR_OPT_PW_KS, SR_OPT_PT_CFG, SR_OPT_PT_KS, SR_OPT_DOT_LDS,
   SR_OPT_DOT_LDS_G, SR_OPT_DOT_LDS_CULL, SR_OPT_DOT_LDS_CAP, SR_OPT_UPSAMPLE_QUAD, SR_OPT_POOL_STREAM,
-  SR_OPT_MLP_TILE,
+  SR_OPT_MLP_TILE, SR_OPT_DW_FORM,
   SR_OPT_COUNT
 };
 int sr_option_count(void);
@@ -140,6 +140,8 @@
 
 #define SR_ACT_NONE (-1.0f)
 #define SR_ACT_SILU (-2.0f)
+#define SR_ACT_SILU_RES (-4.0f)
+int sr_conv_fuses_res_after_act(int ksize, int stride, int route, int aligned16);
 int sr_conv2d_padded_nhwc_fwd(const float* in, int64_t in_batch_stride, int in_pix_stride,
                               const float* packed_weight, const float* bias, const float* residual,
                               int64_t res_batch_stride, int res_pix_stride, float* out,
diff --git a/simplerecon_amd/_lib.py b/simplerecon_amd/_lib.py
--- a/simplerecon_amd/_lib.py
+++ b/simplerecon_amd/_lib.py
@@ -50,6 +50,7 @@
     "sr_pw_conv_tiled_plan": (_i, [_i, _i, _i, _i, _p, _p]),
     "sr_pw_conv_tiled_nhwc_fwd": (_i, [_p, _i, _p, _p, _p, _p, _i, _p, _i, _i, _i, _i, _i, _f, _p, _sz, _p]),
     "sr_pw_conv_supported": (_i, [_i, _i]),
+    "sr_conv_fuses_res_after_act": (_i, [_i, _i, _i, _i]),
     "sr_pw_conv_plan": (_i, [_i, _i, _i, _i, _p, _p]),
     "sr_pw_conv_nhwc_fwd": (_i, [_p, _i64, _i, _p, _p, _p, _p, _i64, _i, _p, _i64, _i, _i, _i, _i, _i, _f, _p]),
     "sr_backproject_fwd": (_i, [_p, _p, _p, _i, _i, _i, _p]),
@@ -263,7 +264,9 @@
 _SPLIT_NAMES = {0: "", 1: "bf16", 2: "f16"}
 SPLIT_OPTION_NAMES = ("SR_MLP_SPLIT", "SR_WINO_SPLIT")
 TILE_MODES = {"auto": 0, "flat": 1, "2x32": 2, "4x16": 3, "8x8": 4}
-_NAMED_VALUES = {"SR_MLP_SPLIT": SPLIT_MODES, "SR_WINO_SPLIT": SPLIT_MODES, "SR_MLP_TILE": TILE_MODES}
+DW_FORMS = {"auto": 0, "taps": 1, "block": 2}
+_NAMED_VALUES = {"SR_MLP_SPLIT": SPLIT_MODES, "SR_WINO_SPLIT": SPLIT_MODES, "SR_MLP_TILE": TILE_MODES,
+                 "SR_DW_FORM": DW_FORMS}
 import threading
 SPLIT_GUARD = threading.RLock()
 
diff --git a/simplerecon_amd/csrc/sr_common.h b/simplerecon_amd/csrc/sr_common.h
--- a/simplerecon_amd/csrc/sr_common.h
+++ b/simplerecon_amd/csrc/sr_common.h
@@ -143,6 +143,10 @@
   if (slope < -1.5f) return v / (1.0f + __expf(-v));
   return v;
 }
+__device__ __forceinline__ float sr_add_rounded(float a, float b) {
+#pragma clang fp contract(off)
+  return a + b;
+}
 __device__ __forceinline__ float sr_uniform(float x) {
   return __builtin_bit_cast(float, __builtin_amdgcn_readfirstlane(__builtin_bit_cast(int, x)));
 }
@@ -163,6 +167,8 @@
 }
 #endif
 
+static inline bool sr_act_is_res_after(float code) { return code < -3.5f; }
+
 struct SrDotParams {
   const float* cur;
   const float* src_nhwc;
diff --git a/simplerecon_amd/csrc/sr_conv.hip b/simplerecon_amd/csrc/sr_conv.hip
--- a/simplerecon_amd/csrc/sr_conv.hip
+++ b/simplerecon_amd/csrc/sr_conv.hip
@@ -121,7 +121,7 @@
   return t;
 }
 
-template <int KS, int S, int MT, int NT, int CM, bool VEC4>
+template <int KS, int S, int MT, int NT, int CM, bool VEC4, bool AFTER = false>
 __global__ __launch_bounds__(256) void sr_conv_kernel(SrConvParams p) {
   using G = SrConvGeom<KS, S, MT, CM>;
   constexpr int TH = G::TH, HW = G::HW, RM = G::RM;
@@ -281,9 +281,17 @@
               for (int r = 0; r < 16; ++r) rv[r] = 0.0f;
             }
             float o16[16];
-#pragma unroll
-            for (int r = 0; r < 16; ++r) o16[r] = acc[m][n][r] + bv + rv[r];
-            sr_activate_group(o16, slope);
+            if (AFTER) {
+#pragma unroll
+              for (int r = 0; r < 16; ++r) o16[r] = acc[m][n][r] + bv + 0.0f;
+              sr_activate_group(o16, SR_ACT_SILU);
+#pragma unroll
+              for (int r = 0; r < 16; ++r) o16[r] = sr_add_rounded(o16[r], rv[r]);
+            } else {
+#pragma unroll
+              for (int r = 0; r < 16; ++r) o16[r] = acc[m][n][r] + bv + rv[r];
+              sr_activate_group(o16, slope);
+            }
 #pragma unroll
             for (int r = 0; r < 16; ++r) {
               const int row = (8 * (r >> 2)) / CM, colc = (8 * (r >> 2)) % CM + (r & 3);
@@ -298,9 +306,17 @@
               if (!RES_PF) rv[r] = (!no_res && ok[r]) ? resp[rb + (unsigned)((row * p.Wo + colc) * rsp)] : 0.0f;
             }
             float o16[16];
-#pragma unroll
-            for (int r = 0; r < 16; ++r) o16[r] = acc[m][n][r] + bv + rv[r];
-            sr_activate_group(o16, slope);
+            if (AFTER) {
+#pragma unroll
+              for (int r = 0; r < 16; ++r) o16[r] = acc[m][n][r] + bv + 0.0f;
+              sr_activate_group(o16, SR_ACT_SILU);
+#pragma unroll
+              for (int r = 0; r < 16; ++r) o16[r] = sr_add_rounded(o16[r], rv[r]);
+            } else {
+#pragma unroll
+              for (int r = 0; r < 16; ++r) o16[r] = acc[m][n][r] + bv + rv[r];
+              sr_activate_group(o16, slope);
+            }
 #pragma unroll
             for (int r = 0; r < 16; ++r) {
               const int row = (8 * (r >> 2)) / CM, colc = (8 * (r >> 2)) % CM + (r & 3);
@@ -469,6 +485,17 @@
   if (blocks > p.total_tiles) blocks = p.total_tiles;
   dim3 grid(blocks), block(256);
   const bool v4 = p.vec4 && (p.Cin % 4 == 0);
+  if (sr_act_is_res_after(p.slope) && p.res) {
+    if constexpr (KS == 3 && S == 1) {
+      if (nt == 2 && v4) hipLaunchKernelGGL((sr_conv_kernel<3, 1, MT, 2, CM, true, true>), grid, block, 0, stream, p);
+      else if (nt == 2) hipLaunchKernelGGL((sr_conv_kernel<3, 1, MT, 2, CM, false, true>), grid, block, 0, stream, p);
+      else if (v4) hipLaunchKernelGGL((sr_conv_kernel<3, 1, MT, 1, CM, true, true>), grid, block, 0, stream, p);
+      else hipLaunchKernelGGL((sr_conv_kernel<3, 1, MT, 1, CM, false, true>), grid, block, 0, stream, p);
+      return sr_hip_rc(hipGetLastError());
+    } else {
+      return SR_ERR_UNSUPPORTED;
+    }
+  }
   if (nt == 2 && v4) hipLaunchKernelGGL((sr_conv_kernel<KS, S, MT, 2, CM, true>), grid, block, 0, stream, p);
   else if (nt == 2) hipLaunchKernelGGL((sr_conv_kernel<KS, S, MT, 2, CM, false>), grid, block, 0, stream, p);
   else if (v4) hipLaunchKernelGGL((sr_conv_kernel<KS, S, MT, 1, CM, true>), grid, block, 0, stream, p);
@@ -550,8 +577,9 @@
   p.slope = leaky_slope;
   p.replicate = replicate;
   p.ksplit = 1; p.part = nullptr; p.part_stride = 0;
-  if (workspace && sr_conv_splitk_eligible(out, out_batch_stride, out_pix_stride, bias, residual, res_batch_stride,
-                                           res_pix_stride, Cin, Cout, ksize, stride)) {
+  if (workspace && !sr_act_is_res_after(leaky_slope) &&
+      sr_conv_splitk_eligible(out, out_batch_stride, out_pix_stride, bias, residual, res_batch_stride, res_pix_stride, Cin, Cout,
+                              ksize, stride)) {
     p.part_stride = (int64_t)B * p.Ho * p.Wo * Cout;
     const size_t fit = workspace_bytes / ((size_t)p.part_stride * sizeof(float));
     p.ksplit = fit < 2 ? 1 : (fit < SR_CONV_KSPLIT_MAX ? (int)fit : SR_CONV_KSPLIT_MAX);
@@ -616,6 +644,11 @@
                             leaky_slope, 0, stream_, pads);
 }
 
+extern "C" int sr_conv_fuses_res_after_act(int ksize, int stride, int route, int aligned16) {
+  if (ksize != 3 || stride != 1) return 0;
+  return (route == 0 || (route == 1 && aligned16)) ? 1 : 0;
+}
+
 extern "C" size_t sr_conv_splitk_workspace_bytes(int B, int H, int W, int Cin, int Cout, int ksize, int stride) {
   if (B <= 0 || H <= 0 || W <= 0 || Cout % 4 != 0) return 0;
   const bool pw = ksize == 1 && stride == 1 && Cin >= 4 * SR_CK1;
diff --git a/simplerecon_amd/csrc/sr_mbconv.hip b/simplerecon_amd/csrc/sr_mbconv.hip
--- a/simplerecon_amd/csrc/sr_mbconv.hip
+++ b/simplerecon_amd/csrc/sr_mbconv.hip
@@ -69,6 +69,75 @@
         }
         *reinterpret_cast<float4*>(outb + (int64_t)opix[u] * p.out_sp) = acc;
         sum.x += acc.x; sum.y += acc.y; sum.z += acc.z; sum.w += acc.w;
+      }
+    }
+  }
+  if (p.pool) {
+    red[xl][c4] = sum;
+    __syncthreads();
+    for (int s = DW_XL / 2; s > 0; s >>= 1) {
+      if (xl < s) {
+        const float4 a = red[xl][c4], o = red[xl + s][c4];
+        red[xl][c4] = make_float4(a.x + o.x, a.y + o.y, a.z + o.z, a.w + o.w);
+      }
+      __syncthreads();
+    }
+    if (xl == 0 && live)
+      *reinterpret_cast<float4*>(p.pool + ((int64_t)b * p.bands + band) * p.C + c) = red[0][c4];
+  }
+}
+
+template <int S>
+__global__ __launch_bounds__(256) void sr_dwconv3x3_block_kernel(SrDwParams p) {
+  constexpr int WIN = S + 3;
+  __shared__ float4 red[DW_XL][DW_CH / 4];
+  const int c4 = threadIdx.x & 15, xl = threadIdx.x >> 4;
+  const int c = blockIdx.x * DW_CH + 4 * c4;
+  const int band = blockIdx.y, b = blockIdx.z;
+  const bool live = c < p.C;
+  float4 wt[9], bv = make_float4(0.f, 0.f, 0.f, 0.f), sum = make_float4(0.f, 0.f, 0.f, 0.f);
+#pragma unroll
+  for (int t = 0; t < 9; ++t)
+    wt[t] = live ? *reinterpret_cast<const float4*>(p.w + (int64_t)t * p.C + c) : make_float4(0.f, 0.f, 0.f, 0.f);
+  if (live && p.bias) bv = *reinterpret_cast<const float4*>(p.bias + c);
+  const float* __restrict__ inb = p.in + (int64_t)b * p.in_sb + c;
+  float* __restrict__ outb = p.out + (int64_t)b * p.out_sb + c;
+  const int oy0 = band * p.rows, oy1 = min(p.Ho, oy0 + p.rows);
+  const int bw = (p.Wo + 1) >> 1;
+  const int nblk = ((oy1 - oy0 + 1) >> 1) * bw;
+  if (live) {
+    for (int q = xl; q < nblk; q += DW_XL) {
+      const int by = q / bw, bx = q - by * bw;
+      const int oy = oy0 + 2 * by, ox = 2 * bx;
+      const bool row1 = oy + 1 < oy1, col1 = ox + 1 < p.Wo;
+      const int iy0 = oy * S - p.pad_y, ix0 = ox * S - p.pad_x;
+      float4 v[WIN][WIN];
+#pragma unroll
+      for (int r = 0; r < WIN; ++r) {
+#pragma unroll
+        for (int k = 0; k < WIN; ++k) {
+          const int iy = iy0 + r, ix = ix0 + k;
+          const bool ok = (r < 3 || row1) && (k < 3 || col1) && (iy >= 0) && (iy < p.H) && (ix >= 0) && (ix < p.W);
+          const float4 t = *reinterpret_cast<const float4*>(inb + (ok ? (iy * p.W + ix) * p.in_sp : 0));
+          v[r][k] = ok ? t : make_float4(0.f, 0.f, 0.f, 0.f);
+        }
+      }
+#pragma unroll
+      for (int dy = 0; dy < 2; ++dy) {
+#pragma unroll
+        for (int dx = 0; dx < 2; ++dx) {
+          if ((dy && !row1) || (dx && !col1)) continue;
+          float4 acc = bv;
+#pragma unroll
+          for (int t = 0; t < 9; ++t) acc = f4fma(v[dy * S + t / 3][dx * S + t % 3], wt[t], acc);
+          {
+            float a4[4] = {acc.x, acc.y, acc.z, acc.w};
+            sr_activate_group(a4, sr_uniform(p.slope));
+            acc = make_float4(a4[0], a4[1], a4[2], a4[3]);
+          }
+          *reinterpret_cast<float4*>(outb + (int64_t)((oy + dy) * p.Wo + ox + dx) * p.out_sp) = acc;
+          sum.x += acc.x; sum.y += acc.y; sum.z += acc.z; sum.w += acc.w;
+        }
       }
     }
   }
@@ -278,6 +347,8 @@
 }
 
 inline bool aligned16(const void* ptr) { return (((uintptr_t)ptr) & 15) == 0; }
+
+inline int sr_dwconv3x3_auto_form(int stride) { return stride == 1 ? 2 : 1; }
 
 }
 
@@ -315,8 +386,13 @@
   p.slope = leaky_slope;
   if ((int64_t)H * W * in_pix_stride >= (1ll << 31) || (int64_t)p.Ho * p.Wo * out_pix_stride >= (1ll << 31))
     return SR_ERR_UNSUPPORTED;
+  int form = sr_opt(SR_OPT_DW_FORM);
+  if (form < 0 || form > 2) return SR_ERR_INVALID_ARGUMENT;
+  if (form == 0) form = sr_dwconv3x3_auto_form(stride);
   dim3 grid((C + DW_CH - 1) / DW_CH, p.bands, B);
-  hipLaunchKernelGGL(sr_dwconv3x3_kernel, grid, dim3(256), 0, (hipStream_t)stream_, p);
+  if (form == 1) hipLaunchKernelGGL(sr_dwconv3x3_kernel, grid, dim3(256), 0, (hipStream_t)stream_, p);
+  else if (stride == 1) hipLaunchKernelGGL(sr_dwconv3x3_block_kernel<1>, grid, dim3(256), 0, (hipStream_t)stream_, p);
+  else hipLaunchKernelGGL(sr_dwconv3x3_block_kernel<2>, grid, dim3(256), 0, (hipStream_t)stream_, p);
   return sr_hip_rc(hipGetLastError());
 }
 
diff --git a/simplerecon_amd/csrc/sr_options.hip b/simplerecon_amd/csrc/sr_options.hip
--- a/simplerecon_amd/csrc/sr_options.hip
+++ b/simplerecon_amd/csrc/sr_options.hip
@@ -16,6 +16,7 @@
     {"SR_PW_NT", 0, 0},           {"SR_PW_KS", 0, 0},          {"SR_PT_CFG", -1, 0},         {"SR_PT_KS", 0, 0},
     {"SR_DOT_LDS", 1, 0},         {"SR_DOT_LDS_G", 0, 0},      {"SR_DOT_LDS_CULL", 1, 0},    {"SR_DOT_LDS_CAP", 634, 0},
     {"SR_UPSAMPLE_QUAD", 1, 0},   {"SR_POOL_STREAM", 1, 0},    {"SR_MLP_TILE", 0, 2},
+    {"SR_DW_FORM", 0, 3},
 };
 std::atomic<int> g_val[SR_OPT_COUNT];
 std::once_flag g_once;
@@ -31,6 +32,13 @@
     static const char* const names[] = {"auto", "flat", "2x32", "4x16", "8x8"};
     if (!e || !*e) return d.dflt;
     for (int i = 0; i < 5; ++i)
+      if (!strcmp(e, names[i])) return i;
+    return -1;
+  }
+  if (d.kind == 3) {
+    static const char* const names[] = {"auto", "taps", "block"};
+    if (!e || !*e) return d.dflt;
+    for (int i = 0; i < 3; ++i)
       if (!strcmp(e, names[i])) return i;
     return -1;
   }
diff --git a/simplerecon_amd/csrc/sr_pw.hip b/simplerecon_amd/csrc/sr_pw.hip
--- a/simplerecon_amd/csrc/sr_pw.hip
+++ b/simplerecon_amd/csrc/sr_pw.hip
@@ -221,6 +221,7 @@
   if (B == 0) return SR_OK;
   if (!in || !packed_w || !out) return SR_ERR_INVALID_ARGUMENT;
   if (io && gate) return SR_ERR_UNSUPPORTED;
+  if (sr_act_is_res_after(act_code)) return SR_ERR_UNSUPPORTED;
   if (Cin % 4 != 0 || !sr_rows_aligned(in, in_batch_stride, in_pix_stride, io ? 7 : 15, 4) || (gate && !sr_ptr_aligned(gate, 15)))
     return SR_ERR_UNSUPPORTED;
   if (!sr_view_fits32(HW, in_pix_stride, Cin, 4) || !sr_view_fits32(HW, out_pix_stride, Cout, 4) ||
diff --git a/simplerecon_amd/csrc/sr_pw_tiled.hip b/simplerecon_amd/csrc/sr_pw_tiled.hip
--- a/simplerecon_amd/csrc/sr_pw_tiled.hip
+++ b/simplerecon_amd/csrc/sr_pw_tiled.hip
@@ -205,6 +205,7 @@
   if (M < 0 || HW <= 0 || Cin <= 0 || Cout <= 0) return SR_ERR_INVALID_ARGUMENT;
   if (M == 0) return SR_OK;
   if (!in || !packed_w || !out) return SR_ERR_INVALID_ARGUMENT;
+  if (sr_act_is_res_after(act_code)) return SR_ERR_UNSUPPORTED;
   if (Cin % 4 != 0 || !sr_rows_aligned(in, 0, in_pix_stride, 15, 4) || (gate && !sr_ptr_aligned(gate, 15)))
     return SR_ERR_UNSUPPORTED;
   const bool can_split = workspace && sr_ptr_aligned(workspace, 15) && Cout % 4 == 0 &&
diff --git a/simplerecon_amd/csrc/sr_wino.hip b/simplerecon_amd/csrc/sr_wino.hip
--- a/simplerecon_amd/csrc/sr_wino.hip
+++ b/simplerecon_amd/csrc/sr_wino.hip
@@ -32,9 +32,10 @@
   }
 }
 
-template <int NT, bool VEC4, bool VOUT, int IO = 0>
+template <int NT, bool VEC4, bool VOUT, int IO = 0, bool AFTER = false>
 __global__ __launch_bounds__(256, NT == 1 ? SR_WINO_NT1_WAVES : SR_WINO_WAVES) void sr_wino_kernel(SrWinoParams p) {
   static_assert(IO == 0 || (VEC4 && VOUT), "16-bit I/O exists for the vector staging / epilogue instantiation only");
+  static_assert(!AFTER || (VEC4 && VOUT && IO == 0), "the residual-after-activation epilogue exists for fp32 vector I/O only");
   constexpr unsigned ES = SR_IO_ES(IO);
   extern __shared__ __attribute__((aligned(16))) float lds[];
   float* O = lds;
@@ -387,14 +388,27 @@
 #pragma unroll
           for (int q = 0; q < 4; ++q) {
             float4 v = f4add(y[q], bv);
-            if (RES) v = f4add(v, rv[it][q]);
-            if (fast_leaky) {
+            if (RES && !AFTER) v = f4add(v, rv[it][q]);
+            if (!AFTER && fast_leaky) {
               const wn_f2 lo = wn_f2{v.x, v.y} * slope2, hi = wn_f2{v.z, v.w} * slope2;
               v = make_float4(sr_vmax(v.x, lo.x), sr_vmax(v.y, lo.y), sr_vmax(v.z, hi.x), sr_vmax(v.w, hi.y));
             }
             o16[4 * q + 0] = v.x; o16[4 * q + 1] = v.y; o16[4 * q + 2] = v.z; o16[4 * q + 3] = v.w;
           }
-          if (!fast_leaky) sr_activate_group(o16, slope);
+          if (AFTER) {
+            sr_activate_group(o16, SR_ACT_SILU);
+            if (RES) {
+#pragma unroll
+              for (int q = 0; q < 4; ++q) {
+                o16[4 * q + 0] = sr_add_rounded(o16[4 * q + 0], rv[it][q].x);
+                o16[4 * q + 1] = sr_add_rounded(o16[4 * q + 1], rv[it][q].y);
+                o16[4 * q + 2] = sr_add_rounded(o16[4 * q + 2], rv[it][q].z);
+                o16[4 * q + 3] = sr_add_rounded(o16[4 * q + 3], rv[it][q].w);
+              }
+            }
+          } else if (!fast_leaky) {
+            sr_activate_group(o16, slope);
+          }
 #pragma unroll
           for (int q = 0; q < 4; ++q) {
             sr_io_store<IO>(sr_f4{o16[4 * q], o16[4 * q + 1], o16[4 * q + 2], o16[4 * q + 3]}, rs_out,
@@ -603,7 +617,9 @@
   if (p.vec4 && !sr_view_fits32(HW, in_pix_stride, Cin, 4)) return SR_ERR_UNSUPPORTED;
   if (vout && (!sr_view_fits32(HW, out_pix_stride, Cout, 4) || (residual && !sr_view_fits32(HW, res_pix_stride, Cout, 4))))
     return SR_ERR_UNSUPPORTED;
-  const bool can_split = !io && vout && workspace && sr_ptr_aligned(workspace, 15);
+  const bool res_after = sr_act_is_res_after(leaky_slope) && residual;
+  if (res_after && (split || io || !vout)) return SR_ERR_UNSUPPORTED;
+  const bool can_split = !io && vout && workspace && sr_ptr_aligned(workspace, 15) && !res_after;
   SrWinoPlan plan = sr_wino_plan(B, H, W, Cin, Cout, can_split);
   if (plan.ks > 1 && workspace_bytes < (size_t)plan.ks * B * H * W * Cout * sizeof(float))
     plan = sr_wino_plan(B, H, W, Cin, Cout, false);
@@ -636,7 +652,14 @@
     if (hipError_t e = sr_allow_lds((const void*)sr_wino_kernel<NTV, V4, VO>, lds)) return sr_hip_rc(e);          \
     hipLaunchKernelGGL((sr_wino_kernel<NTV, V4, VO>), dim3(blocks), dim3(256), lds, stream, p);                   \
   }
+#define SR_WINO_LAUNCH_AFTER(NTV)                                                                                      \
+  {                                                                                                                    \
+    if (hipError_t e = sr_allow_lds((const void*)sr_wino_kernel<NTV, true, true, 0, true>, lds)) return sr_hip_rc(e);  \
+    hipLaunchKernelGGL((sr_wino_kernel<NTV, true, true, 0, true>), dim3(blocks), dim3(256), lds, stream, p);           \
+  }
   if (split) { const int rc = sr_wino_split_launch(p, nt, blocks, split, stream); if (rc) return rc; }
+  else if (res_after && nt == 2) SR_WINO_LAUNCH_AFTER(2)
+  else if (res_after) SR_WINO_LAUNCH_AFTER(1)
   else if (io == 1 && nt == 2) SR_WINO_LAUNCH_IO(2, 1)
   else if (io == 1) SR_WINO_LAUNCH_IO(1, 1)
   else if (io == 2 && nt == 2) SR_WINO_LAUNCH_IO(2, 2)
@@ -648,6 +671,7 @@
   else if (p.vec4) SR_WINO_LAUNCH(1, true, false)
   else SR_WINO_LAUNCH(1, false, false)
 #undef SR_WINO_LAUNCH
+#undef SR_WINO_LAUNCH_AFTER
 #undef SR_WINO_LAUNCH_IO
 #ifdef SR_WINO_TRACE
   {
diff --git a/simplerecon_amd/csrc/sr_wino4.hip b/simplerecon_amd/csrc/sr_wino4.hip
--- a/simplerecon_amd/csrc/sr_wino4.hip
+++ b/simplerecon_amd/csrc/sr_wino4.hip
@@ -910,6 +910,7 @@
   if (B < 0 || H <= 0 || W <= 0 || Cin <= 0 || Cout <= 0) return SR_ERR_INVALID_ARGUMENT;
   if (B == 0) return SR_OK;
   if (!in || !packed_u || !out) return SR_ERR_INVALID_ARGUMENT;
+  if (sr_act_is_res_after(leaky_slope)) return SR_ERR_UNSUPPORTED;
   if (Cin % 4 != 0 || Cout % 4 != 0 || !sr_rows_aligned(in, in_batch_stride, in_pix_stride, 15, 4) ||
       !sr_rows_aligned(out, out_batch_stride, out_pix_stride, 15, 4) || (bias && !sr_ptr_aligned(bias, 15)) ||
       (residual && !sr_rows_aligned(residual, res_batch_stride, res_pix_stride, 15, 4)))
diff --git a/simplerecon_amd/image_encoder.py b/simplerecon_amd/image_encoder.py
--- a/simplerecon_amd/image_encoder.py
+++ b/simplerecon_amd/image_encoder.py
@@ -34,8 +34,9 @@
         self.has_skip = stride == 1 and cin == cout
 
     def forward(self, x):
-        y = ops.conv2d(x, self.conv, bn=self.bn1, act="silu", tf_same=True)
-        return ops.add_(y, x) if self.has_skip else y
+        if self.has_skip:
+            return ops.conv2d(x, self.conv, bn=self.bn1, act="silu", tf_same=True, residual=x, residual_after_act=True)
+        return ops.conv2d(x, self.conv, bn=self.bn1, act="silu", tf_same=True)
 
     def forward_train(self, x):
         y = T.batch_norm_act(T.conv(x, self.conv, pads=_tf_pads(x, self.conv)), self.bn1, act=T.ACT_SILU)
diff --git a/simplerecon_amd/ops.py b/simplerecon_amd/ops.py
--- a/simplerecon_amd/ops.py
+++ b/simplerecon_amd/ops.py
@@ -242,7 +242,11 @@
     return v
 
 
-def conv2d(x, conv: nn.Conv2d, residual=None, leaky=None, out=None, bn=None, act=None, tf_same=False, gate=None):
+ACT_SILU_RES = -4.0
+
+
+def conv2d(x, conv: nn.Conv2d, residual=None, leaky=None, out=None, bn=None, act=None, tf_same=False, gate=None,
+           residual_after_act=False):
     _lib.refuse_autograd(x, conv.weight)
     x = as_nhwc(x, "conv input")
     b, ci, h, w = x.shape
@@ -270,12 +274,21 @@
         residual = as_nhwc(residual, "residual")
         if tuple(residual.shape) != (b, co, ho, wo):
             raise ValueError(f"residual shape {tuple(residual.shape)} != output shape {(b, co, ho, wo)}")
+    if residual_after_act:
+        if residual is None:
+            raise ValueError("residual_after_act needs a residual")
+        if act != "silu":
+            raise ValueError("residual_after_act is implemented for act=\"silu\" only")
     if b == 0:
         return out
     isb, isp = _strides(x)
     osb, osp = _strides(out)
     rsb, rsp = _strides(residual) if residual is not None else (0, 0)
     split = use_wino and wino_split_mode()
+    if residual_after_act and not _fuses_residual_after_act(lib, x, residual, out, (isb, isp, osb, osp, rsb, rsp),
+                                                            (b, ci, h, w, co, k, s), use_wino, split, padded, replicate):
+        y = conv2d(x, conv, leaky=leaky, out=out, bn=bn, act=act, tf_same=tf_same, gate=gate)
+        return add_(y, residual)
     if split and not (ci % 4 == 0 and co % 4 == 0 and _aligned16(x, isb, isp) and _aligned16(out, osb, osp)
                       and _aligned16(residual, rsb, rsp)):
         use_wino = split = False
@@ -283,7 +296,7 @@
         _lib.require_device_f32("gate", gate)
         if k != 1 or s != 1 or tuple(gate.shape) != (b, ci) or not gate.is_contiguous():
             raise ValueError(f"`gate` needs a 1x1 / stride-1 conv and a contiguous [{b}, {ci}] tensor")
-    slope = _act_code(leaky, act)
+    slope = ACT_SILU_RES if residual_after_act else _act_code(leaky, act)
     strides = (isb, isp, osb, osp, rsb, rsp)
     if k == 1 and s == 1 and not padded and not replicate and (USE_PW_1X1 or gate is not None) and ci % 4 == 0 \
             and _aligned16(x, isb, isp):
@@ -321,6 +334,24 @@
     return out
 
 
+def _fuses_residual_after_act(lib, x, residual, out, strides, shape, use_wino, split, padded, replicate):
+    isb, isp, osb, osp, rsb, rsp = strides
+    b, ci, h, w, co, k, s = shape
+    if k == 1:
+        route = 4
+    elif not use_wino:
+        route = 0
+    elif split:
+        route = 3
+    elif WINO4_MODE and _shape_query(lib, "sr_conv_prefers_wino4", b, h, w, ci, co, WINO4_MODE, dev=x.device.index):
+        route = 2
+    else:
+        route = 1
+    aligned = ci % 4 == 0 and co % 4 == 0 and bool(_aligned16(x, isb, isp) and _aligned16(out, osb, osp)
+                                                   and _aligned16(residual, rsb, rsp))
+    return bool(_shape_query(lib, "sr_conv_fuses_res_after_act", k, s, route, int(aligned)))
+
+
 def _aligned16(t, sb, sp):
     return t is None or (t.data_ptr() % 16 == 0 and sp % 4 == 0 and sb % 4 == 0)
 
```

New measurement: 330.9 (median of 6 runs). 1.2% higher.
